# EpicDuckPotato/stereo_vo

Measured on AMD Instinct MI355X. Metric: stereo frames/sec on 1241x376 KITTI pairs, higher is better.
Workload: dtype u8/f32/f64; 1 GPU; kitti_1241x376_1500corners_5kf_window (BASELINE configs[1]); streams_per_gpu=96, max_corners=1500, window=5, pipeline_groups=3, hardware_queues=4

## Files before the change

include/svo.h:

```cpp
#ifndef SVO_H_
#define SVO_H_

#include <stddef.h>
#include <stdint.h>

#ifdef __cplusplus
extern "C" {
#endif

typedef enum svo_status {
  SVO_OK = 0,
  SVO_ERR_INVALID = -1,
  SVO_ERR_HIP = -2,
  SVO_ERR_CAPACITY = -3,
  SVO_ERR_NO_DEVICE = -4,
  SVO_ERR_NUMERIC = -5
} svo_status;

typedef struct svo_camera_info {
  double focal, cx, cy;
  double k1, k2, p1, p2;
  double baseline;
} svo_camera_info;

// ... 224 lines not shown

typedef struct svo_ba_options {
  int max_iterations;
  double max_time_s;
  double function_tolerance, gradient_tolerance, parameter_tolerance;
  double initial_radius;
  int max_features;
  int accumulation;
} svo_ba_options;

enum { SVO_BA_ACC_AUTO = 0, SVO_BA_ACC_DETERMINISTIC = 1, SVO_BA_ACC_ATOMICS = 2, SVO_BA_ACC_MFMA = 3 };

typedef struct svo_ba_summary {
  int iterations, successful_steps, termination;
  double initial_cost, final_cost;
  double solve_ms;
} svo_ba_summary;

typedef int (*svo_allreduce_fn)(void* dev_ptr, size_t n_doubles, void* user);

typedef struct svo_lm_step_ctl {
  double cost, mcc, decrease_factor;
  double spec_radius;
  int chain;
} svo_lm_step_ctl;
typedef struct svo_lm_ops {
  void* user;
  int (*linearize)(void* user, double radius, int first, double* payload1);
  int (*step)(void* user, const double* dc, const double* cand_poses7, double radius, const svo_lm_step_ctl* ctl,
              double* payload2, double* payload1_next, double* next_radius, int* next_at_candidate);
  int (*accept)(void* user);
} svo_lm_ops;
typedef struct svo_lm_stats {
  int linearize_calls;
  int step_calls;
  int speculations;
  int speculation_hits;
  int single_exchange;
  int collectives;
  int device_control;
  int fallbacks;
  double host_us;
} svo_lm_stats;

void svo_ba_default_options(svo_ba_options* o);
int svo_lm_solve(int n_poses, double* poses7, const svo_lm_ops* ops, const svo_ba_options* opt,
                 svo_ba_summary* summary, svo_lm_stats* stats);
int svo_lm_decide_step(double cost, double mcc, double radius, double decrease_factor, double cost_new,
                       double model_change_points, int* accept, double* next_radius);
int svo_ba_create(svo_ctx* ctx, svo_ba** out, int window_size, const svo_camera_info* cam,
                  const svo_ba_options* opt, int max_landmarks, int max_observations);
void svo_ba_destroy(svo_ba* ba);
int svo_ba_reset(svo_ba* ba);
int svo_ba_add_keyframe(svo_ba* ba, const double* pose7, const int64_t* tracked_ids,
                        const float* tracked_xy, int n_tracked, const float* new_xy,
                        const float* new_xyz, int n_new, int64_t* new_ids, int* n_new_out);
int svo_ba_solve(svo_ba* ba, svo_ba_summary* summary);
int svo_cholesky_solve(double* A, double* b, int n);
int svo_cholesky_solve_dev(svo_ctx* ctx, double* A, double* b, int n);
int svo_ba_get_pose(svo_ba* ba, int k, double* pose7);
int svo_ba_window_count(svo_ba* ba);
int svo_ba_get_points(svo_ba* ba, const int64_t* ids, int n, float* xyz);

int svo_ba_load_problem(svo_ba* ba, int n_poses, const double* poses7, int n_points,
                        const double* points3, int n_obs, const int32_t* obs_pose,
                        const int32_t* obs_point, const double* obs_uv);
int svo_ba_set_allreduce(svo_ba* ba, svo_allreduce_fn fn, void* user);
int svo_ba_set_comm(svo_ba* ba, void* nccl_comm);
int svo_rccl_unique_id(void* id128);
int svo_rccl_comm_create(void** nccl_comm, int n_ranks, int rank, const void* id128, int device);
int svo_rccl_comm_destroy(void* nccl_comm);
int svo_ba_set_device_lm(svo_ba* ba, int mode);
int svo_ba_set_solve_form(svo_ba* ba, int form);
int svo_ba_set_bulk_control(svo_ba* ba, int mode);
int svo_ba_last_stats(svo_ba* ba, svo_lm_stats* stats);
int svo_ba_wave_chunks_limit(void);
int svo_ba_set_wave_chunks(svo_ba* ba, int k);
int svo_ba_solve_forms(svo_ba* ba, long* counts, int n, long* gave_up);
int svo_ba_set_yield_iterations(svo_ba* ba, int n);
int svo_ba_solve_problem(svo_ba* ba, svo_ba_summary* summary);
int svo_ba_solve_problems(svo_ba** bas, int n, svo_ba_summary* summaries);
int svo_ba_read_problem(svo_ba* ba, double* poses7, double* points3);

typedef struct svo_pipeline svo_pipeline;
typedef struct svo_pipeline_params {
  svo_camera_info cam;
  int width, height;
  int max_corners;
  double quality;
  float min_feature_distance;
  float parallax_thresh;
  int window_size;
  int max_features;
  int ba_max_iterations;
  double ba_max_time_s;
} svo_pipeline_params;

typedef struct svo_frame_result {
  int n_detected, n_tracked, n_inliers, n_new;
  int is_keyframe;
  float av_parallax, percent_lost;
  double pose7[7];
  int ba_iterations;
} svo_frame_result;

void svo_pipeline_default_params(svo_pipeline_params* p);
int svo_pipeline_create(svo_ctx* ctx, svo_pipeline** out, const svo_pipeline_params* p);
void svo_pipeline_destroy(svo_pipeline* p);
int svo_pipeline_reset(svo_pipeline* p);
int svo_pipeline_process_batch_dev(svo_pipeline* p, const uint8_t* left, const uint8_t* right,
                                   int batch, svo_frame_result* results);
int svo_pipeline_process_batch(svo_pipeline* p, const uint8_t* left, const uint8_t* right,
                               int batch, svo_frame_result* results);
int svo_pipeline_set_rectification(svo_pipeline* p, const svo_rectify_eye* left, const svo_rectify_eye* right);
int svo_pipeline_set_keyframe_clouds(svo_pipeline* p, const svo_cloud_params* params, int max_keyframes_per_call);
int svo_pipeline_set_keyframe_speckle_filter(svo_pipeline* p, const svo_speckle_params* params);
int svo_pipeline_set_keyframe_lr_check(svo_pipeline* p, const svo_lr_check_params* params);
int svo_pipeline_set_keyframe_sgm(svo_pipeline* p, const svo_sgm_params* params);
typedef struct svo_keyframe_cloud {
  int frame;
  int lane;
  int n_total, n_stored;
  const svo_cloud_point* dev;
} svo_keyframe_cloud;
int svo_pipeline_keyframe_clouds(svo_pipeline* p, int* n, const svo_keyframe_cloud** table);
int svo_pipeline_copy_keyframe_cloud(svo_pipeline* p, int i, svo_cloud_point* host, int capacity);
int svo_pipeline_keyframe_disparity(svo_pipeline* p, int i, const int16_t** dev);
int svo_pipeline_copy_keyframe_disparity(svo_pipeline* p, int i, int16_t* host);
int svo_pipeline_get_tracked(svo_pipeline* p, int64_t* ids, float* xy, int capacity, int* n);

typedef struct svo_pipeline_group svo_pipeline_group;
int svo_pipeline_group_create(svo_ctx* ctx, svo_pipeline_group** out, const svo_pipeline_params* p, int n_lanes);
void svo_pipeline_group_destroy(svo_pipeline_group* g);
int svo_pipeline_group_reset(svo_pipeline_group* g);
int svo_pipeline_group_lanes(const svo_pipeline_group* g);
int svo_pipeline_group_process_batch_dev(svo_pipeline_group* g, const uint8_t* left, const uint8_t* right, size_t lane_stride,
                                         int batch, svo_frame_result* results);
int svo_pipeline_group_staging(svo_pipeline_group* g, int slot, uint8_t** left, uint8_t** right, size_t* lane_stride);
int svo_pipeline_group_upload(svo_pipeline_group* g, int slot, int batch);
int svo_pipeline_group_process_uploaded(svo_pipeline_group* g, int slot, svo_frame_result* results);
int svo_pipeline_group_process_batch(svo_pipeline_group* g, const uint8_t* left, const uint8_t* right, size_t lane_stride,
                                     int batch, svo_frame_result* results);
int svo_pipeline_group_set_rectification(svo_pipeline_group* g, int lane, const svo_rectify_eye* left, const svo_rectify_eye* right);
int svo_pipeline_group_set_keyframe_clouds(svo_pipeline_group* g, int lane, const svo_cloud_params* params, int max_keyframes_per_call);
int svo_pipeline_group_set_keyframe_speckle_filter(svo_pipeline_group* g, const svo_speckle_params* params);
int svo_pipeline_group_set_keyframe_lr_check(svo_pipeline_group* g, const svo_lr_check_params* params);
int svo_pipeline_group_set_keyframe_sgm(svo_pipeline_group* g, const svo_sgm_params* params);
int svo_pipeline_group_keyframe_clouds(svo_pipeline_group* g, int* n, const svo_keyframe_cloud** table);
int svo_pipeline_group_copy_keyframe_cloud(svo_pipeline_group* g, int i, svo_cloud_point* host, int capacity);
int svo_pipeline_group_keyframe_disparity(svo_pipeline_group* g, int i, const int16_t** dev);
int svo_pipeline_group_copy_keyframe_disparity(svo_pipeline_group* g, int i, int16_t* host);
int svo_pipeline_group_get_tracked(svo_pipeline_group* g, int lane, int64_t* ids, float* xy, int capacity, int* n);
int svo_pipeline_group_last_stats(const svo_pipeline_group* g, long* launches6, long* lanes6);
int svo_pipeline_group_solve_work(svo_pipeline_group* g, double* out4, int reset);
int svo_pipeline_group_solve_forms(svo_pipeline_group* g, long* counts, int n, long* gave_up);
int svo_pipeline_group_set_solve_yield(svo_pipeline_group* g, int n);

int svo_draw_track(const uint8_t* gray, int width, int height, int row_stride, const float* from_xy,
                   const float* to_xy, int n, uint8_t* rgb);
int svo_pipeline_draw_track(svo_pipeline* p, const uint8_t* keyframe_gray, int row_stride, uint8_t* rgb);

typedef struct svo_synth_params {
  uint64_t seed;
  int width, height;
  double focal, cx, cy, baseline;
  double step_z, step_x, yaw_per_frame;
  int n_billboards;
} svo_synth_params;
void svo_synth_default_params(svo_synth_params* p, int width, int height);
int svo_synth_render(const svo_synth_params* p, int frame, uint8_t* left, uint8_t* right);
int svo_synth_pose(const svo_synth_params* p, int frame, double* rt12);

int svo_image_read_gray(const char* path, uint8_t* buf, size_t capacity, int* width, int* height);
int svo_kitti_read_poses(const char* poses_file, double* rt12, int capacity_frames, int* n_frames);
int svo_ate_rmse(const double* est_xyz, const double* gt_xyz, int n, int with_scale, double* rmse);
typedef struct svo_run_stats {
  int frames, keyframes;
  double ate_rmse;
  double seconds;
} svo_run_stats;
int svo_kitti_run(svo_ctx* ctx, const svo_pipeline_params* params, const char* data_path, int sequence,
                  int max_frames, double* traj_rt12, svo_run_stats* stats);

#ifdef __cplusplus
}
#endif
#endif
```

stereo_vo_amd/api.py:

```python
import ctypes as C
import os

import numpy as np

_HERE = os.path.dirname(os.path.abspath(__file__))
_LIB = None


class SvoError(RuntimeError):
    pass


def lib_path():
    return os.path.join(_HERE, "libsvo_hip.so")


class Limits(C.Structure):
    _fields_ = [("max_width", C.c_int), ("max_height", C.c_int), ("max_batch", C.c_int),
                ("max_corners", C.c_int), ("max_candidates", C.c_int), ("max_features", C.c_int)]


class CameraInfo(C.Structure):
    _fields_ = [(n, C.c_double) for n in ("focal", "cx", "cy", "k1", "k2", "p1", "p2", "baseline")]

# ... 199 lines not shown
SPECKLE_TILE = (64, 16)


def speckle_workspace_bytes(width, height, batch=1):
    return int(lib().svo_speckle_workspace_bytes(width, height, batch))


CLOUD_POINT_DTYPE = np.dtype([("x", np.float32), ("y", np.float32), ("z", np.float32), ("tag", np.uint32)])


class KeyframeCloud(C.Structure):
    _fields_ = [("frame", C.c_int), ("lane", C.c_int), ("n_total", C.c_int), ("n_stored", C.c_int), ("dev", C.c_void_p)]


def cloud_default_params(width, height):
    p = CloudParams()
    if lib().svo_cloud_default_params(C.byref(p), width, height) != 0:
        raise SvoError("svo_cloud_default_params failed")
    return p


def _cloud_params(width, height, step, min_disparity, max_points):
    return CloudParams(int(step), float(min_disparity), int(width * height if max_points is None else max_points))


def _keyframe_disparity(ctx, h, fn, i):
    dev = C.c_void_p()
    ctx._chk(fn(h, int(i), C.byref(dev)), fn.__name__)
    return dev.value


def _keyframe_disparity_host(ctx, h, fn, i, width, height):
    d = np.empty((height, width), np.int16)
    ctx._chk(fn(h, int(i), _p(d)), fn.__name__)
    return d


def _keyframe_clouds(ctx, L, h, table_fn, copy_fn):
    n, tab = C.c_int(0), C.POINTER(KeyframeCloud)()
    ctx._chk(table_fn(h, C.byref(n), C.byref(tab)), table_fn.__name__)
    out = []
    for i in range(n.value):
        e = tab[i]
        pts = np.empty(e.n_stored, CLOUD_POINT_DTYPE)
        ctx._chk(copy_fn(h, i, _p(pts), e.n_stored), copy_fn.__name__)
        out.append({"frame": e.frame, "lane": e.lane, "n_total": e.n_total, "n_stored": e.n_stored, "dev": e.dev, "points": pts})
    return out


class SynthParams(C.Structure):
    _fields_ = [("seed", C.c_uint64), ("width", C.c_int), ("height", C.c_int), ("focal", C.c_double),
                ("cx", C.c_double), ("cy", C.c_double), ("baseline", C.c_double), ("step_z", C.c_double),
                ("step_x", C.c_double), ("yaw_per_frame", C.c_double), ("n_billboards", C.c_int)]


REFERENCE_CONSTANT_NAMES = (
    "gftt_max_corners", "gftt_quality", "min_detected", "keyframe_percent_lost", "pnp_iterations", "pnp_reproj_error",
    "pnp_confidence", "stereo_num_disparities", "stereo_block_size", "stereo_disparity_scale",
    "triangulate_min_disparity_exclusive", "lk_win_w", "lk_win_h", "lk_max_level", "lk_max_iterations", "lk_epsilon",
    "lk_min_eig_threshold", "fb_max_distance", "max_parallax", "draw_thickness", "parallax_thresh", "min_feature_distance",
    "sliding_window_size", "max_features", "ba_max_solver_time_s", "ba_num_threads")


class ReferenceConstants(C.Structure):
    _fields_ = [(n, C.c_double) for n in REFERENCE_CONSTANT_NAMES]


def reference_constants():
    c = ReferenceConstants()
    if lib().svo_reference_constants(C.byref(c)) != 0:
        raise SvoError("svo_reference_constants failed")
    return {n: getattr(c, n) for n in REFERENCE_CONSTANT_NAMES}


class LmStats(C.Structure):
    _fields_ = [("linearize_calls", C.c_int), ("step_calls", C.c_int), ("speculations", C.c_int), ("speculation_hits", C.c_int),
                ("single_exchange", C.c_int), ("collectives", C.c_int), ("device_control", C.c_int), ("fallbacks", C.c_int),
                ("host_us", C.c_double)]


class LmStepCtl(C.Structure):
    _fields_ = [("cost", C.c_double), ("mcc", C.c_double), ("decrease_factor", C.c_double), ("spec_radius", C.c_double),
                ("chain", C.c_int)]


LM_LINEARIZE_FN = C.CFUNCTYPE(C.c_int, C.c_void_p, C.c_double, C.c_int, C.POINTER(C.c_double))
LM_STEP_FN = C.CFUNCTYPE(C.c_int, C.c_void_p, C.POINTER(C.c_double), C.POINTER(C.c_double), C.c_double, C.POINTER(LmStepCtl),
                         C.POINTER(C.c_double), C.POINTER(C.c_double), C.POINTER(C.c_double), C.POINTER(C.c_int))
LM_ACCEPT_FN = C.CFUNCTYPE(C.c_int, C.c_void_p)


class LmOps(C.Structure):
    _fields_ = [("user", C.c_void_p), ("linearize", LM_LINEARIZE_FN), ("step", LM_STEP_FN), ("accept", LM_ACCEPT_FN)]


def lm_decide_step(cost, mcc, radius, decrease_factor, cost_new, model_change_points):
    acc, rad = C.c_int(0), C.c_double(0.0)
    lib().svo_lm_decide_step(C.c_double(cost), C.c_double(mcc), C.c_double(radius), C.c_double(decrease_factor), C.c_double(cost_new),
                             C.c_double(model_change_points), C.byref(acc), C.byref(rad))
    return bool(acc.value), rad.value


def lm_solve(poses7, linearize, step, accept, max_iterations=50, max_time_s=0.0):
    poses = np.ascontiguousarray(poses7, np.float64).copy()
    K = poses.shape[0]
    n = 6 * (K - 1)
    pay1 = n * n + 3 * n + 2

    def _lin(user, radius, first, out):
        np.ctypeslib.as_array(out, shape=(pay1,))[:] = linearize(radius, first)
        return 0

    def _step(user, dc, cand, radius, ctl, out2, out1, out_radius, out_at_cand):
        d = np.ctypeslib.as_array(dc, shape=(max(n, 1),))[:n].copy()
        c = np.ctypeslib.as_array(cand, shape=(K, 7)).copy()
        p2, p1, nr, at_cand = step(d, c, radius, ctl.contents)
        np.ctypeslib.as_array(out2, shape=(4,))[:] = p2
        if p1 is not None:
            np.ctypeslib.as_array(out1, shape=(pay1,))[:] = p1
        out_radius[0] = nr if p1 is not None else 0.0
        out_at_cand[0] = int(bool(at_cand))
        return 0

    def _acc(user):
        accept()
        return 0
    ops = LmOps(None, LM_LINEARIZE_FN(_lin), LM_STEP_FN(_step), LM_ACCEPT_FN(_acc))
    opt = ba_default_options()
    opt.max_iterations, opt.max_time_s = max_iterations, max_time_s
    s, st = BASummary(), LmStats()
    rc = lib().svo_lm_solve(K, _p(poses), C.byref(ops), C.byref(opt), C.byref(s), C.byref(st))
    if rc:
        raise SvoError(f"svo_lm_solve failed ({rc})")
    return poses, s, st


ALLREDUCE_FN = C.CFUNCTYPE(C.c_int, C.c_void_p, C.c_size_t, C.c_void_p)

SYMBOLS = [
    "svo_create", "svo_destroy", "svo_last_error", "svo_stream", "svo_sync", "svo_version", "svo_reference_constants",
    "svo_profile_select", "svo_profile_read", "svo_measure_peak",
    "svo_reproj_eval", "svo_reproj_eval_dev",
    "svo_corner_detect", "svo_corner_detect_batch_dev", "svo_corner_response",
    "svo_stereo_bm", "svo_stereo_disparity_at", "svo_stereo_disparity_at_dev",
    "svo_triangulate", "svo_lk_track", "svo_build_pyramid", "svo_track_features", "svo_dedup",
    "svo_pnp_ransac",
    "svo_ba_default_options", "svo_ba_create", "svo_ba_destroy", "svo_ba_reset", "svo_ba_add_keyframe", "svo_ba_solve",
    "svo_ba_get_pose", "svo_ba_window_count", "svo_ba_get_points", "svo_ba_load_problem",
    "svo_ba_set_allreduce", "svo_ba_set_device_lm", "svo_ba_set_bulk_control", "svo_ba_set_solve_form", "svo_ba_wave_chunks_limit", "svo_ba_set_wave_chunks", "svo_ba_set_yield_iterations", "svo_ba_solve_forms", "svo_ba_solve_problem", "svo_ba_solve_problems", "svo_ba_read_problem", "svo_ba_set_comm", "svo_ba_last_stats", "svo_lm_solve", "svo_lm_decide_step",
    "svo_rccl_unique_id", "svo_rccl_comm_create", "svo_rccl_comm_destroy",
    "svo_pipeline_default_params", "svo_pipeline_create", "svo_pipeline_destroy", "svo_pipeline_reset",
    "svo_pipeline_process_batch_dev", "svo_pipeline_process_batch", "svo_pipeline_get_tracked",
    "svo_pipeline_group_create", "svo_pipeline_group_destroy", "svo_pipeline_group_reset", "svo_pipeline_group_lanes",
    "svo_pipeline_group_process_batch_dev", "svo_pipeline_group_get_tracked", "svo_pipeline_group_last_stats",
    "svo_pipeline_group_solve_work", "svo_pipeline_group_solve_forms", "svo_pipeline_group_set_solve_yield", "svo_pipeline_group_staging", "svo_pipeline_group_upload", "svo_pipeline_group_process_uploaded", "svo_pipeline_group_process_batch",
    "svo_synth_default_params", "svo_synth_render", "svo_synth_pose",
    "svo_image_read_gray", "svo_kitti_read_poses", "svo_ate_rmse", "svo_kitti_run", "svo_cholesky_solve", "svo_cholesky_solve_dev", "svo_draw_track", "svo_pipeline_draw_track",
    "svo_rectify_eye_from_camera_info", "svo_rectify_build_map", "svo_rectify_remap", "svo_rectify_remap_batch_dev",
    "svo_pipeline_set_rectification", "svo_pipeline_group_set_rectification",
    "svo_stereo_bm_batch_dev", "svo_cloud_default_params", "svo_disparity_cloud_batch_dev", "svo_stereo_cloud",
    "svo_pipeline_set_keyframe_clouds", "svo_pipeline_keyframe_clouds", "svo_pipeline_copy_keyframe_cloud",
    "svo_pipeline_group_set_keyframe_clouds", "svo_pipeline_group_keyframe_clouds", "svo_pipeline_group_copy_keyframe_cloud",
    "svo_speckle_workspace_bytes", "svo_disparity_speckle_filter_batch_dev", "svo_disparity_speckle_filter",
    "svo_pipeline_set_keyframe_speckle_filter", "svo_pipeline_group_set_keyframe_speckle_filter",
    "svo_stereo_bm_cost_batch_dev", "svo_disparity_lr_check_batch_dev", "svo_disparity_lr_check",
    "svo_pipeline_set_keyframe_lr_check", "svo_pipeline_group_set_keyframe_lr_check",
    "svo_sgm_default_params", "svo_sgm_workspace_bytes", "svo_stereo_sgm_batch_dev", "svo_stereo_sgm",
    "svo_pipeline_set_keyframe_sgm", "svo_pipeline_group_set_keyframe_sgm",
    "svo_voxel_map_default_params", "svo_voxel_map_bytes", "svo_voxel_map_create", "svo_voxel_map_destroy", "svo_voxel_map_clear",
    "svo_voxel_map_insert_dev", "svo_pose7_to_cam_to_world", "svo_voxel_map_insert_pose7_dev", "svo_voxel_map_stats",
    "svo_voxel_map_extract_dev", "svo_voxel_map_extract", "svo_voxel_map_download",
    "svo_voxel_carve_default_params", "svo_voxel_map_carve_dev", "svo_pose7_to_world_to_cam", "svo_voxel_map_carve_pose7_dev",
    "svo_voxel_map_carve", "svo_voxel_map_copy_live_dev", "svo_pipeline_keyframe_disparity", "svo_pipeline_group_keyframe_disparity",
    "svo_pipeline_copy_keyframe_disparity", "svo_pipeline_group_copy_keyframe_disparity",
    "svo_voxel_render_default_params", "svo_voxel_render_workspace_bytes", "svo_voxel_map_render_dev", "svo_voxel_map_render_pose7_dev",
    "svo_voxel_map_render", "svo_voxel_render_set_mode",
    "svo_voxel_map_remove_dev", "svo_voxel_map_remove_pose7_dev", "svo_voxel_map_remove_sync", "svo_voxel_map_move_dev", "svo_voxel_map_move_pose7_dev",
    "svo_voxel_ledger_bytes", "svo_voxel_ledger_create", "svo_voxel_ledger_destroy", "svo_voxel_ledger_insert_pose7_dev",
    "svo_voxel_ledger_update_pose7", "svo_voxel_ledger_retire", "svo_voxel_ledger_remove", "svo_voxel_ledger_ids", "svo_voxel_ledger_get",
]


def lib():
    global _LIB
    if _LIB is None:
        p = lib_path()
        if not os.path.exists(p):
            raise SvoError(f"{p} not built — run `python -c 'import __graft_entry__ as g; g.build()'`")
        L = C.CDLL(p)
        L.svo_version.restype = C.c_char_p
        L.svo_last_error.restype = C.c_char_p
        L.svo_last_error.argtypes = [C.c_void_p]
        L.svo_stream.restype = C.c_void_p
        L.svo_stream.argtypes = [C.c_void_p]
        L.svo_destroy.argtypes = [C.c_void_p]
        L.svo_destroy.restype = None
        vp, ci, sz = C.c_void_p, C.c_int, C.c_size_t
        L.svo_cloud_default_params.argtypes = [vp, ci, ci]
        L.svo_stereo_bm_batch_dev.argtypes = [vp, vp, vp, ci, ci, ci, ci, sz, ci, ci, vp]
        L.svo_disparity_cloud_batch_dev.argtypes = [vp, vp, vp, ci, ci, ci, ci, sz, vp, vp, vp, vp, vp]
        L.svo_stereo_cloud.argtypes = [vp, vp, vp, ci, ci, ci, ci, ci, vp, vp, vp, vp, vp, vp]
        L.svo_pipeline_set_keyframe_clouds.argtypes = [vp, vp, ci]
        L.svo_pipeline_keyframe_clouds.argtypes = [vp, vp, vp]
        L.svo_pipeline_copy_keyframe_cloud.argtypes = [vp, ci, vp, ci]
        L.svo_pipeline_group_set_keyframe_clouds.argtypes = [vp, ci, vp, ci]
        L.svo_pipeline_group_keyframe_clouds.argtypes = [vp, vp, vp]
        L.svo_pipeline_group_copy_keyframe_cloud.argtypes = [vp, ci, vp, ci]
        for f in ("svo_cloud_default_params", "svo_stereo_bm_batch_dev", "svo_disparity_cloud_batch_dev", "svo_stereo_cloud",
                  "svo_pipeline_set_keyframe_clouds", "svo_pipeline_keyframe_clouds", "svo_pipeline_copy_keyframe_cloud",
                  "svo_pipeline_group_set_keyframe_clouds", "svo_pipeline_group_keyframe_clouds", "svo_pipeline_group_copy_keyframe_cloud"):
            getattr(L, f).restype = ci
        L.svo_speckle_workspace_bytes.argtypes = [ci, ci, ci]
        L.svo_speckle_workspace_bytes.restype = sz
        L.svo_disparity_speckle_filter_batch_dev.argtypes = [vp, vp, ci, ci, ci, vp, vp, sz, vp]
        L.svo_disparity_speckle_filter.argtypes = [vp, vp, ci, ci, vp, vp]
        L.svo_pipeline_set_keyframe_speckle_filter.argtypes = [vp, vp]
        L.svo_pipeline_group_set_keyframe_speckle_filter.argtypes = [vp, vp]
        for f in ("svo_disparity_speckle_filter_batch_dev", "svo_disparity_speckle_filter", "svo_pipeline_set_keyframe_speckle_filter",
                  "svo_pipeline_group_set_keyframe_speckle_filter"):
            getattr(L, f).restype = ci
        L.svo_stereo_bm_cost_batch_dev.argtypes = [vp, vp, vp, ci, ci, ci, ci, sz, ci, ci, vp, vp]
        L.svo_disparity_lr_check_batch_dev.argtypes = [vp, vp, vp, ci, ci, ci, vp, vp]
        L.svo_disparity_lr_check.argtypes = [vp, vp, vp, ci, ci, vp, vp]
        L.svo_pipeline_set_keyframe_lr_check.argtypes = [vp, vp]
        L.svo_pipeline_group_set_keyframe_lr_check.argtypes = [vp, vp]
        for f in ("svo_stereo_bm_cost_batch_dev", "svo_disparity_lr_check_batch_dev", "svo_disparity_lr_check",
                  "svo_pipeline_set_keyframe_lr_check", "svo_pipeline_group_set_keyframe_lr_check"):
            getattr(L, f).restype = ci
        L.svo_sgm_default_params.argtypes = [vp, ci]
        L.svo_sgm_workspace_bytes.argtypes = [ci, ci, ci, ci, ci]
        L.svo_sgm_workspace_bytes.restype = sz
        L.svo_stereo_sgm_batch_dev.argtypes = [vp, vp, vp, ci, ci, ci, ci, sz, ci, ci, vp, vp, sz, vp, vp]
        L.svo_stereo_sgm.argtypes = [vp, vp, vp, ci, ci, ci, ci, ci, vp, vp, vp]
        L.svo_pipeline_set_keyframe_sgm.argtypes = [vp, vp]
        L.svo_pipeline_group_set_keyframe_sgm.argtypes = [vp, vp]
        for f in ("svo_sgm_default_params", "svo_stereo_sgm_batch_dev", "svo_stereo_sgm", "svo_pipeline_set_keyframe_sgm",
                  "svo_pipeline_group_set_keyframe_sgm"):
            getattr(L, f).restype = ci
        L.svo_voxel_map_default_params.argtypes = [vp]
        L.svo_voxel_map_bytes.argtypes = [vp, vp]
        L.svo_voxel_map_create.argtypes = [vp, vp, vp]
        L.svo_voxel_map_destroy.argtypes = [vp]
        L.svo_voxel_map_destroy.restype = None
        L.svo_voxel_map_clear.argtypes = [vp]
        L.svo_voxel_map_insert_dev.argtypes = [vp, vp, ci, vp]
        L.svo_pose7_to_cam_to_world.argtypes = [vp, vp]
        L.svo_voxel_map_insert_pose7_dev.argtypes = [vp, vp, ci, vp]
        L.svo_voxel_map_stats.argtypes = [vp, vp]
        L.svo_voxel_map_extract_dev.argtypes = [vp, ci, vp, ci, vp]
        L.svo_voxel_map_extract.argtypes = [vp, ci, vp, ci, vp, vp]
        L.svo_voxel_map_download.argtypes = [vp, vp, sz]
        for f in ("svo_voxel_map_default_params", "svo_voxel_map_bytes", "svo_voxel_map_create", "svo_voxel_map_clear",
                  "svo_voxel_map_insert_dev", "svo_pose7_to_cam_to_world", "svo_voxel_map_insert_pose7_dev", "svo_voxel_map_stats",
                  "svo_voxel_map_extract_dev", "svo_voxel_map_extract", "svo_voxel_map_download"):
            getattr(L, f).restype = ci
        L.svo_voxel_carve_default_params.argtypes = [vp]
        L.svo_voxel_map_carve_dev.argtypes = [vp, vp, ci, ci, vp, vp, vp, vp]
        L.svo_pose7_to_world_to_cam.argtypes = [vp, vp]
        L.svo_voxel_map_carve_pose7_dev.argtypes = [vp, vp, ci, ci, vp, vp, vp, vp]
        L.svo_voxel_map_carve.argtypes = [vp, vp, ci, ci, vp, vp, vp, vp]
        L.svo_voxel_map_copy_live_dev.argtypes = [vp, vp, ci, vp]
        L.svo_pipeline_keyframe_disparity.argtypes = [vp, ci, vp]
        L.svo_pipeline_group_keyframe_disparity.argtypes = [vp, ci, vp]
        L.svo_pipeline_copy_keyframe_disparity.argtypes = [vp, ci, vp]
        L.svo_pipeline_group_copy_keyframe_disparity.argtypes = [vp, ci, vp]
        for f in ("svo_voxel_carve_default_params", "svo_voxel_map_carve_dev", "svo_pose7_to_world_to_cam", "svo_voxel_map_carve_pose7_dev",
                  "svo_voxel_map_carve", "svo_voxel_map_copy_live_dev", "svo_pipeline_keyframe_disparity",
                  "svo_pipeline_group_keyframe_disparity", "svo_pipeline_copy_keyframe_disparity",
                  "svo_pipeline_group_copy_keyframe_disparity"):
            getattr(L, f).restype = ci
        L.svo_voxel_render_default_params.argtypes = [vp]
        L.svo_voxel_render_workspace_bytes.argtypes = [ci, ci]
        L.svo_voxel_render_workspace_bytes.restype = sz
        L.svo_voxel_map_render_dev.argtypes = [vp, ci, ci, vp, vp, vp, vp, vp, vp, vp]
        L.svo_voxel_map_render_pose7_dev.argtypes = [vp, ci, ci, vp, vp, vp, vp, vp, vp, vp]
        L.svo_voxel_map_render.argtypes = [vp, ci, ci, vp, vp, vp, vp, vp, vp]
        L.svo_voxel_render_set_mode.argtypes = [vp, ci, ci]
        for f in ("svo_voxel_render_default_params", "svo_voxel_map_render_dev", "svo_voxel_map_render_pose7_dev", "svo_voxel_map_render",
                  "svo_voxel_render_set_mode"):
            getattr(L, f).restype = ci
        i64 = C.c_int64
        L.svo_voxel_map_remove_dev.argtypes = [vp, vp, ci, vp, vp]
        L.svo_voxel_map_remove_pose7_dev.argtypes = [vp, vp, ci, vp, vp]
        L.svo_voxel_map_remove_sync.argtypes = [vp, vp, ci, vp, vp]
        L.svo_voxel_map_move_dev.argtypes = [vp, vp, ci, vp, vp, vp]
        L.svo_voxel_map_move_pose7_dev.argtypes = [vp, vp, ci, vp, vp, vp]
        L.svo_voxel_ledger_bytes.argtypes = [vp, vp]
        L.svo_voxel_ledger_create.argtypes = [vp, vp, vp]
        L.svo_voxel_ledger_destroy.argtypes = [vp]
        L.svo_voxel_ledger_destroy.restype = None
        L.svo_voxel_ledger_insert_pose7_dev.argtypes = [vp, i64, vp, ci, vp]
        L.svo_voxel_ledger_update_pose7.argtypes = [vp, i64, vp, vp]
        L.svo_voxel_ledger_retire.argtypes = [vp, i64]
        L.svo_voxel_ledger_remove.argtypes = [vp, i64, vp]
        L.svo_voxel_ledger_ids.argtypes = [vp, vp, ci, vp]
        L.svo_voxel_ledger_get.argtypes = [vp, i64, vp, vp, vp]
        for f in ("svo_voxel_map_remove_dev", "svo_voxel_map_remove_pose7_dev", "svo_voxel_map_remove_sync", "svo_voxel_map_move_dev", "svo_voxel_map_move_pose7_dev",
                  "svo_voxel_ledger_bytes", "svo_voxel_ledger_create", "svo_voxel_ledger_insert_pose7_dev", "svo_voxel_ledger_update_pose7",
                  "svo_voxel_ledger_retire", "svo_voxel_ledger_remove", "svo_voxel_ledger_ids", "svo_voxel_ledger_get"):
            getattr(L, f).restype = ci
        _LIB = L
    return _LIB


def _p(a, t=None):
    if a is None:
        return None
# ... 685 lines not shown

    def close(self):
        if self.h:
            self.L.svo_pipeline_destroy(self.h)
            self.h = C.c_void_p()

    def __del__(self):
        try:
            self.close()
        except Exception:
            pass

    def reset(self):
        self.ctx._chk(self.L.svo_pipeline_reset(self.h), "svo_pipeline_reset")

    def set_rectification(self, left=None, right=None):
        self.L.svo_pipeline_set_rectification.argtypes = [C.c_void_p, C.c_void_p, C.c_void_p]
        self.ctx._chk(self.L.svo_pipeline_set_rectification(self.h, _ref(left), _ref(right)), "svo_pipeline_set_rectification")

    def set_keyframe_clouds(self, params=None, max_keyframes_per_call=0):
        if params is True:
            params = cloud_default_params(self.prm.width, self.prm.height)
        self.ctx._chk(self.L.svo_pipeline_set_keyframe_clouds(self.h, _ref(params), max_keyframes_per_call),
                      "svo_pipeline_set_keyframe_clouds")

    def process_batch(self, left, right):
        left, right = _u8(left), _u8(right)
        b = left.shape[0]
        res = (FrameResult * b)()
        self.ctx._chk(self.L.svo_pipeline_process_batch(self.h, _p(left), _p(right), b, res), "svo_pipeline_process_batch")
        return list(res)

    def process_batch_dev(self, left_ptr, right_ptr, batch):
        res = (FrameResult * batch)()
        self.ctx._chk(self.L.svo_pipeline_process_batch_dev(self.h, C.c_void_p(left_ptr), C.c_void_p(right_ptr), batch, res),
                      "svo_pipeline_process_batch_dev")
        return list(res)

    def draw_track(self, keyframe_gray):
        g = np.ascontiguousarray(keyframe_gray, np.uint8)
        out = np.empty(g.shape + (3,), np.uint8)
        self.ctx._chk(self.L.svo_pipeline_draw_track(self.h, _p(g), g.shape[1], _p(out)), "svo_pipeline_draw_track")
        return out

    def tracked(self, capacity=8192):
        ids = np.empty(capacity, np.int64)
        xy = np.empty((capacity, 2), np.float32)
        n = C.c_int(0)
        self.ctx._chk(self.L.svo_pipeline_get_tracked(self.h, _p(ids), _p(xy), capacity, C.byref(n)), "svo_pipeline_get_tracked")
        return ids[:n.value].copy(), xy[:n.value].copy()


class PipelineGroup(_KeyframeCloudMethods):

    _ENTRY = "svo_pipeline_group"
    STAGES = ("track", "pnp_ransac", "host_thread_busy_us_of_call_us", "dedup_stereo_triangulate", "bundle_adjust", "corners_pyramids")

    def __init__(self, ctx, params, n_lanes):
        self.ctx, self.L, self.prm, self.n_lanes = ctx, ctx.L, params, n_lanes
        self.h = C.c_void_p()
        self.L.svo_pipeline_group_destroy.argtypes = [C.c_void_p]
        self.L.svo_pipeline_group_destroy.restype = None
        self.L.svo_pipeline_group_process_batch_dev.argtypes = [C.c_void_p, C.c_void_p, C.c_void_p, C.c_size_t, C.c_int, C.c_void_p]
        ctx._chk(self.L.svo_pipeline_group_create(ctx.h, C.byref(self.h), C.byref(params), n_lanes), "svo_pipeline_group_create")

    def close(self):
        if self.h:
            self.L.svo_pipeline_group_destroy(self.h)
            self.h = C.c_void_p()

    def __del__(self):
        try:
            self.close()
        except Exception:
            pass

    def reset(self):
        self.ctx._chk(self.L.svo_pipeline_group_reset(self.h), "svo_pipeline_group_reset")

    def set_rectification(self, lane, left=None, right=None):
        self.L.svo_pipeline_group_set_rectification.argtypes = [C.c_void_p, C.c_int, C.c_void_p, C.c_void_p]
        self.ctx._chk(self.L.svo_pipeline_group_set_rectification(self.h, lane, _ref(left), _ref(right)), "svo_pipeline_group_set_rectification")

    def set_keyframe_clouds(self, lane=-1, params=None, max_keyframes_per_call=0):
        if params is True:
            params = cloud_default_params(self.prm.width, self.prm.height)
        self.ctx._chk(self.L.svo_pipeline_group_set_keyframe_clouds(self.h, lane, _ref(params), max_keyframes_per_call),
                      "svo_pipeline_group_set_keyframe_clouds")

    def process_batch_dev(self, left_ptr, right_ptr, lane_stride, batch):
        res = (FrameResult * (self.n_lanes * batch))()
        self.ctx._chk(self.L.svo_pipeline_group_process_batch_dev(self.h, C.c_void_p(left_ptr), C.c_void_p(right_ptr), C.c_size_t(lane_stride),
                                                                  batch, res), "svo_pipeline_group_process_batch_dev")
        self.last_raw = bytes(res)
        return [list(res[l * batch:(l + 1) * batch]) for l in range(self.n_lanes)]

    def staging(self, slot):
        lp, rp, stride = C.POINTER(C.c_uint8)(), C.POINTER(C.c_uint8)(), C.c_size_t(0)
        self.L.svo_pipeline_group_staging.argtypes = [C.c_void_p, C.c_int, C.c_void_p, C.c_void_p, C.c_void_p]
        self.ctx._chk(self.L.svo_pipeline_group_staging(self.h, slot, C.byref(lp), C.byref(rp), C.byref(stride)), "svo_pipeline_group_staging")
        h, w = self.prm.height, self.prm.width
        mb = stride.value // (h * w)
        shape = (self.n_lanes, mb, h, w)
        n = self.n_lanes * mb * h * w
        return (np.ctypeslib.as_array(lp, shape=(n,)).reshape(shape), np.ctypeslib.as_array(rp, shape=(n,)).reshape(shape))

    def upload(self, slot, batch):
        self.ctx._chk(self.L.svo_pipeline_group_upload(self.h, slot, batch), "svo_pipeline_group_upload")

    def process_uploaded(self, slot, batch):
        res = (FrameResult * (self.n_lanes * batch))()
        self.L.svo_pipeline_group_process_uploaded.argtypes = [C.c_void_p, C.c_int, C.c_void_p]
        self.ctx._chk(self.L.svo_pipeline_group_process_uploaded(self.h, slot, res), "svo_pipeline_group_process_uploaded")
        self.last_raw = bytes(res)
        return [list(res[l * batch:(l + 1) * batch]) for l in range(self.n_lanes)]

    def process_batch(self, left, right):
        left, right = _u8(left), _u8(right)
        batch = left.shape[1]
        res = (FrameResult * (self.n_lanes * batch))()
        self.L.svo_pipeline_group_process_batch.argtypes = [C.c_void_p, C.c_void_p, C.c_void_p, C.c_size_t, C.c_int, C.c_void_p]
        self.ctx._chk(self.L.svo_pipeline_group_process_batch(self.h, _p(left), _p(right), C.c_size_t(batch * left.shape[2] * left.shape[3]), batch, res),
                      "svo_pipeline_group_process_batch")
        self.last_raw = bytes(res)
        return [list(res[l * batch:(l + 1) * batch]) for l in range(self.n_lanes)]

    def get_tracked(self, lane, capacity=8192):
        ids = np.empty(capacity, np.int64)
        xy = np.empty((capacity, 2), np.float32)
        n = C.c_int(0)
        self.ctx._chk(self.L.svo_pipeline_group_get_tracked(self.h, lane, _p(ids), _p(xy), capacity, C.byref(n)), "svo_pipeline_group_get_tracked")
        return ids[:n.value].copy(), xy[:n.value].copy()

    def solve_work(self, reset=False):
        out = (C.c_double * 4)()
        self.ctx._chk(self.L.svo_pipeline_group_solve_work(self.h, out, int(reset)), "svo_pipeline_group_solve_work")
        return list(out)

    def solve_forms(self):
        n = self.L.svo_ba_wave_chunks_limit() + 1
        out, gu = (C.c_long * n)(), C.c_long(0)
        self.ctx._chk(self.L.svo_pipeline_group_solve_forms(self.h, out, n, C.byref(gu)), "svo_pipeline_group_solve_forms")
        return list(out), gu.value

    def set_solve_yield(self, n):
        self.ctx._chk(self.L.svo_pipeline_group_set_solve_yield(self.h, int(n)), "svo_pipeline_group_set_solve_yield")

    def solve_resumes(self):
        n = self.L.svo_ba_wave_chunks_limit() + 2
        out = (C.c_long * n)()
        self.ctx._chk(self.L.svo_pipeline_group_solve_forms(self.h, out, n, None), "svo_pipeline_group_solve_forms")
        return out[n - 1]

    def last_stats(self):
        a, b = (C.c_long * 6)(), (C.c_long * 6)()
        self.ctx._chk(self.L.svo_pipeline_group_last_stats(self.h, a, b), "svo_pipeline_group_last_stats")
        return {s: (a[i], b[i]) for i, s in enumerate(self.STAGES) if s != "unused"}


class RunStats(C.Structure):
    _fields_ = [("frames", C.c_int), ("keyframes", C.c_int), ("ate_rmse", C.c_double), ("seconds", C.c_double)]


def image_read_gray(path, max_pixels=1 << 24):
    buf = np.empty(max_pixels, np.uint8)
    w, h = C.c_int(0), C.c_int(0)
    rc = lib().svo_image_read_gray(path.encode(), _p(buf), C.c_size_t(max_pixels), C.byref(w), C.byref(h))
    if rc:
        raise SvoError(f"svo_image_read_gray({path}) rc={rc}")
    return buf[:w.value * h.value].reshape(h.value, w.value).copy()


def kitti_read_poses(path, max_frames=100000):
    rt = np.empty((max_frames, 12))
    n = C.c_int(0)
    rc = lib().svo_kitti_read_poses(path.encode(), _p(rt), max_frames, C.byref(n))
    if rc:
        raise SvoError(f"svo_kitti_read_poses({path}) rc={rc}")
    return rt[:n.value].reshape(-1, 3, 4).copy()


def ate_rmse(est_xyz, gt_xyz, with_scale=False):
    est_xyz, gt_xyz = _f64(est_xyz), _f64(gt_xyz)
    out = C.c_double(0)
    rc = lib().svo_ate_rmse(_p(est_xyz), _p(gt_xyz), est_xyz.shape[0], int(with_scale), C.byref(out))
    if rc:
        raise SvoError(f"svo_ate_rmse rc={rc}")
    return out.value


def kitti_run(ctx, params, data_path, sequence, max_frames):
    traj = np.zeros((max_frames, 12))
    st = RunStats()
    ctx._chk(lib().svo_kitti_run(ctx.h, C.byref(params), data_path.encode(), sequence, max_frames, _p(traj), C.byref(st)),
             "svo_kitti_run")
    return traj[:st.frames].reshape(-1, 3, 4).copy(), st


def cholesky_solve(A, b):
    A = np.array(A, np.float64, order="C")
    b = np.array(b, np.float64)
    rc = lib().svo_cholesky_solve(_p(A), _p(b), b.shape[0])
    if rc != 0:
        raise SvoError(f"svo_cholesky_solve rc={rc}")
    return b


def draw_track(gray, from_xy, to_xy):
    g = np.ascontiguousarray(gray, np.uint8)
    a = np.ascontiguousarray(from_xy, np.float32).reshape(-1, 2)
    b = np.ascontiguousarray(to_xy, np.float32).reshape(-1, 2)
    out = np.empty(g.shape + (3,), np.uint8)
    rc = lib().svo_draw_track(_p(g), g.shape[1], g.shape[0], g.shape[1], _p(a), _p(b), a.shape[0], _p(out))
    if rc:
        raise SvoError(f"svo_draw_track rc={rc}")
    return out
```

stereo_vo_amd/csrc/ba.hip:

```cpp
#include <math.h>
#include <stdlib.h>

#include <algorithm>
#include <atomic>
#include <mutex>
#include <sched.h>
#include <chrono>
#include <memory>
#include <vector>

#include "ba_admission.h"
#include "ba_graph.h"
#include "ba_layout.h"
#include "ba_plan.h"
#include "kernels.h"
#include "group_kernels.h"
#include "lm_decide.h"
#include "lm_device.h"
#include "lm_lds.h"
#include "lm_turns.h"
#include "ref_constants.h"
#include "reproj_device.h"

int svo_rccl_allreduce_f64(void* buf, size_t count, void* comm, hipStream_t stream, const char** err);
bool svo_throughput_mode();

namespace {
int g_ba_cu_share = 32;
constexpr int SVO_MAX_DEVICES = 16;
int ba_fused_budget(int device);
BaLedger& ba_ledger(int dev) {
  static std::mutex mu;
  static BaLedger* ledger[SVO_MAX_DEVICES];
  dev = dev >= 0 && dev < SVO_MAX_DEVICES ? dev : 0;
  std::lock_guard<std::mutex> g(mu);
  if (ledger[dev]) return *ledger[dev];
  char bus[64] = {0}, path[128] = {0};
  const char* e = getenv("SVO_BA_XPROC");
  if (!(e && *e && atoi(e) == 0) && hipDeviceGetPCIBusId(bus, sizeof(bus) - 1, dev) == hipSuccess) {
    for (char* c = bus; *c; ++c) if (*c == ':' || *c == '.') *c = '_';
    snprintf(path, sizeof(path), "/dev/shm/svo_admit_%s", bus);
  }
  return *(ledger[dev] = new BaLedger(path[0] ? path : nullptr, dev));
}
constexpr double MIN_DIAG = 1e-6, MAX_DIAG = 1e32, LM_MIN_RADIUS_BULK = 1e-32;
constexpr int BULK_RING = 8;
constexpr int PAY2_SLOTS = 8;

struct BaDev {
  int K = 0, n = 0, M = 0, L = 0, C = 0;
  const double* poses = nullptr;
  double* cand_poses = nullptr;
  const double* points = nullptr;
  double* cand_points = nullptr;
  const int4* rec = nullptr;
  const double* obs_uv = nullptr;
  double* sp = nullptr;
  double* pay1 = nullptr;
  double* pay2 = nullptr;
  double f = 0, cx = 0, cy = 0;
  int det = 0;
  int G = 1, NG = 0, Epad = 0, E = 0;
  int CPW = 1, GS = 1;
  const uint16_t* tab = nullptr;
  const uint32_t* tab_off = nullptr;
  int tab_lds_words = 0;
  const unsigned* lm_key = nullptr;
  double* part1 = nullptr;
  double* part2 = nullptr;
  double* pay1_out = nullptr;
  double* pay2_out = nullptr;
  const double* step_in = nullptr;
  int* flag = nullptr;
  unsigned* arrive = nullptr;
  unsigned arrive_target = 0;
  int seq = 0;
  double* ctl_dev = nullptr;
  unsigned long long pay_tag = 0;
  int pay_parity = 0;
};

struct LmCtl { double cost, mcc, radius, decrease_factor; int chain; };

typedef double svo_d2 __attribute__((ext_vector_type(2)));
template <bool WT>
__device__ __forceinline__ void slot_store2(double* p, double x, double y) {
  if constexpr (WT) {
    const svo_d2 v = {x, y};
    asm volatile("global_store_dwordx4 %0, %1, off sc1\n\ts_nop 1" : : "v"(p), "v"(v) : "memory");
  } else {
    p[0] = x; p[1] = y;
  }
}
__device__ __forceinline__ double slot_load(const double* p) { return __hip_atomic_load(p, __ATOMIC_RELAXED, __HIP_MEMORY_SCOPE_AGENT); }

__device__ __forceinline__ void pay_store(double* p, double v) { __hip_atomic_store(p, v, __ATOMIC_RELAXED, __HIP_MEMORY_SCOPE_SYSTEM); }
__device__ __forceinline__ void granule_store(double* g, double v, unsigned long long tag) { slot_store2<true>(g, v, __longlong_as_double((long long)tag)); }
__device__ __forceinline__ unsigned granule_load8(const double* base, const int (&idx)[8], unsigned long long tag, double (&out)[8]) {
  svo_d2 v0, v1, v2, v3, v4, v5, v6, v7;
  const double* p0 = base + 2 * (idx[0] < 0 ? 0 : idx[0]); const double* p1 = base + 2 * (idx[1] < 0 ? 0 : idx[1]);
  const double* p2 = base + 2 * (idx[2] < 0 ? 0 : idx[2]); const double* p3 = base + 2 * (idx[3] < 0 ? 0 : idx[3]);
  const double* p4 = base + 2 * (idx[4] < 0 ? 0 : idx[4]); const double* p5 = base + 2 * (idx[5] < 0 ? 0 : idx[5]);
  const double* p6 = base + 2 * (idx[6] < 0 ? 0 : idx[6]); const double* p7 = base + 2 * (idx[7] < 0 ? 0 : idx[7]);
  asm volatile(
      "global_load_dwordx4 %0, %8, off sc1\n\tglobal_load_dwordx4 %1, %9, off sc1\n\tglobal_load_dwordx4 %2, %10, off sc1\n\t"
      "global_load_dwordx4 %3, %11, off sc1\n\tglobal_load_dwordx4 %4, %12, off sc1\n\tglobal_load_dwordx4 %5, %13, off sc1\n\t"
      "global_load_dwordx4 %6, %14, off sc1\n\tglobal_load_dwordx4 %7, %15, off sc1\n\ts_waitcnt vmcnt(0)"
      : "=&v"(v0), "=&v"(v1), "=&v"(v2), "=&v"(v3), "=&v"(v4), "=&v"(v5), "=&v"(v6), "=&v"(v7)
      : "v"(p0), "v"(p1), "v"(p2), "v"(p3), "v"(p4), "v"(p5), "v"(p6), "v"(p7)
      : "memory");
  const svo_d2 v[8] = {v0, v1, v2, v3, v4, v5, v6, v7};
  unsigned ok = 0;
#pragma unroll
  for (int u = 0; u < 8; ++u) {
    out[u] = v[u].x;
    if (idx[u] < 0 || (unsigned long long)__double_as_longlong(v[u].y) == tag) ok |= 1u << u;
  }
  return ok;
}
__device__ __forceinline__ bool granule_wait(const double* base, int idx, unsigned long long tag, double& out) {
  const int only[8] = {idx, -1, -1, -1, -1, -1, -1, -1};
  double v[8];
  long long t0 = 0;
  for (unsigned spins = 0;; ++spins) {
    if (granule_load8(base, only, tag, v) & 1u) { out = v[0]; return true; }
    __builtin_amdgcn_s_sleep(2);
    if ((spins & 255u) == 255u) {
      const long long tn = (long long)wall_clock64();
      if (!t0) t0 = tn;
      else if (tn - t0 > 300000000ll) return false;
    }
  }
}

__device__ __forceinline__ bool wait_sentinels(const double* base, int first, int stride, int count, unsigned long long tag, int* s_flag) {
  if (threadIdx.x == 0) *s_flag = 1;
  __syncthreads();
  for (int i = threadIdx.x; i < count; i += (int)blockDim.x) {
    const double* p = base + 2 * ((size_t)first + (size_t)i * stride);
    long long t0 = 0;
    for (unsigned spins = 0;; ++spins) {
      svo_d2 v;
      asm volatile("global_load_dwordx4 %0, %1, off sc1\n\ts_waitcnt vmcnt(0)" : "=&v"(v) : "v"(p) : "memory");
      if ((unsigned long long)__double_as_longlong(v.y) == tag) break;
      __builtin_amdgcn_s_sleep(4);
      if ((spins & 255u) == 255u) {
        const long long tn = (long long)wall_clock64();
        if (!t0) t0 = tn;
        else if (tn - t0 > 300000000ll) { *s_flag = 0; break; }
      }
    }
  }
  __syncthreads();
  return *s_flag != 0;
}

__device__ __forceinline__ void decide_device(const LmCtl& c, double cost_new, double mc_points, double* ctl_dev, double* pay2buf) {
  const SvoLmDecision d = svo_lm_decide(c.cost, c.mcc, c.radius, c.decrease_factor, cost_new, mc_points);
  ctl_dev[0] = (double)d.accept; ctl_dev[1] = d.next_radius;
  pay_store(&pay2buf[4], (double)d.accept); pay_store(&pay2buf[5], d.next_radius);
}

__device__ __forceinline__ void apply_ctl(BaDev& P, double& radius, const double* __restrict__ ctl) {
  if (!ctl) return;
  const double acc = __hip_atomic_load(&ctl[0], __ATOMIC_RELAXED, __HIP_MEMORY_SCOPE_AGENT);
  radius = __hip_atomic_load(&ctl[1], __ATOMIC_RELAXED, __HIP_MEMORY_SCOPE_AGENT);
  if (acc != 0.0) { P.points = P.cand_points; P.poses = P.cand_poses; }
}

enum { BC_DONE = 0, BC_MODE, BC_SEL, BC_RADIUS, BC_DF, BC_COST, BC_INITIAL_COST, BC_MCC, BC_ITER, BC_SUCC, BC_TERM, BC_NEED_LIN,
       BC_LIN_CALLS, BC_STEP_CALLS, BC_NEXT_USED, BC_T0, BC_WORDS = 24 };
enum { BCM_FIRST = 0, BCM_STEP, BCM_RELIN };
struct BulkSel { const double* bctl; double* pts[2]; double* pos[2]; };

__device__ __forceinline__ void bulk_select(BaDev& P, const BulkSel& bs) {
  const int sel = (int)bs.bctl[BC_SEL] & 1;
  P.points = bs.pts[sel]; P.cand_points = bs.pts[sel ^ 1]; P.poses = bs.pos[sel]; P.cand_poses = bs.pos[sel ^ 1];
}
__device__ __forceinline__ bool bulk_apply(BaDev& P, double& radius, int& first_pass, const BulkSel& bs) {
  if (!bs.bctl) return true;
  const double* c = bs.bctl;
  if (c[BC_DONE] != 0.0) return false;
  const int mode = (int)c[BC_MODE];
  bulk_select(P, bs);
  first_pass = mode == BCM_FIRST;
  radius = c[BC_RADIUS];
  if (mode == BCM_STEP) {
    const SvoLmDecision d = svo_lm_decide(c[BC_COST], c[BC_MCC], c[BC_RADIUS], c[BC_DF], P.pay2[0], P.pay2[1]);
    radius = d.next_radius;
    if (d.accept) { P.points = P.cand_points; P.poses = P.cand_poses; }
  }
  return true;
}

__device__ __forceinline__ bool inv3_sym(const double* V, double* Vi) {
  const double a = V[0], b = V[1], c = V[2], d = V[4], e = V[5], f = V[8];
  const double c00 = d * f - e * e, c01 = c * e - b * f, c02 = b * e - c * d;
  const double det = a * c00 + b * c01 + c * c02;
  if (!(fabs(det) > 0)) { for (int i = 0; i < 9; ++i) Vi[i] = 0.0; return false; }
  const double id = 1.0 / det;
  Vi[0] = c00 * id; Vi[1] = c01 * id; Vi[2] = c02 * id;
  Vi[3] = Vi[1]; Vi[4] = (a * f - c * c) * id; Vi[5] = (b * c - a * e) * id;
  Vi[6] = Vi[2]; Vi[7] = Vi[5]; Vi[8] = (a * d - b * b) * id;
  return true;
}

__device__ __forceinline__ double shfl_d(double v, int src) { return __shfl(v, src); }

template <int NV>
__device__ __forceinline__ void segment_totals(double (&v)[NV], int lane, int first, int last, int maxlen) {
  for (int off = 1; off < maxlen; off <<= 1) {
    const bool take = lane - off >= first;
#pragma unroll
    for (int i = 0; i < NV; ++i) {
      const double u = __shfl_up(v[i], off);
      v[i] += take ? u : 0.0;
    }
  }
#pragma unroll
  for (int i = 0; i < NV; ++i) v[i] = shfl_d(v[i], last);
}

__device__ __forceinline__ void eval_obs(const double* __restrict__ pose, D3 p, double u, double v, double f, double cx,
                                         double cy, bool want_jc, double* r, double* Jc, double* Jp) {
  double Jq[14];
  reproj_full(pose, p, u, v, f, cx, cy, r, want_jc ? Jq : nullptr, Jp);
  if (want_jc) {
    const double w = pose[0], x = pose[1], y = pose[2], z = pose[3];
    const double T[4][3] = {{-x, -y, -z}, {w, z, -y}, {-z, w, x}, {y, -x, w}};
#pragma unroll
    for (int row = 0; row < 2; ++row) {
#pragma unroll
      for (int c = 0; c < 3; ++c) {
        double s = 0;
#pragma unroll
        for (int k = 0; k < 4; ++k) s += Jq[7 * row + k] * T[k][c];
        Jc[6 * row + c] = s;
      }
#pragma unroll
      for (int c = 0; c < 3; ++c) Jc[6 * row + 3 + c] = Jq[7 * row + 4 + c];
    }
  }
}
#pragma clang fp contract(fast)
__device__ __forceinline__ void eval_obs_contract(const double* __restrict__ pose, D3 p, double u, double v, double f, double cx,
                                         double cy, bool want_jc, double* r, double* Jc, double* Jp) {
  double Jq[14];
  reproj_full_c(pose, p, u, v, f, cx, cy, r, want_jc ? Jq : nullptr, Jp);
  if (want_jc) {
    const double w = pose[0], x = pose[1], y = pose[2], z = pose[3];
    const double T[4][3] = {{-x, -y, -z}, {w, z, -y}, {-z, w, x}, {y, -x, w}};
#pragma unroll
    for (int row = 0; row < 2; ++row) {
#pragma unroll
      for (int c = 0; c < 3; ++c) {
        double s = 0;
#pragma unroll
        for (int k = 0; k < 4; ++k) s += Jq[7 * row + k] * T[k][c];
        Jc[6 * row + c] = s;
      }
#pragma unroll
      for (int c = 0; c < 3; ++c) Jc[6 * row + 3 + c] = Jq[7 * row + 4 + c];
    }
  }
}
#pragma clang fp contract(off)
}

struct ObsRec { bool active; int o, k, j, first, len; D3 p; double u, v; };

__device__ __forceinline__ ObsRec load_obs(const BaDev& P, int chunk, int lane, const double* __restrict__ points) {
  ObsRec R{false, 0, 0, 0, lane, 0, D3{0, 0, 1}, 0.0, 0.0};
  R.o = chunk * 64 + lane;
  const int4 rc = P.rec[R.o];
  R.u = P.obs_uv[2 * R.o]; R.v = P.obs_uv[2 * R.o + 1];
  R.active = rc.x >= 0;
  if (R.active) {
    R.k = rc.x; R.j = rc.y; R.first = rc.z; R.len = rc.w;
    R.p = D3{points[3 * R.j], points[3 * R.j + 1], points[3 * R.j + 2]};
  }
  return R;
}

struct ObsNext { int4 rc; double u, v; };
__device__ __forceinline__ ObsNext obs_request(const BaDev& P, int chunk, int lane) {
  const int o = chunk * 64 + lane;
  return ObsNext{P.rec[o], P.obs_uv[2 * o], P.obs_uv[2 * o + 1]};
}

struct LinPre { double r[2], Jc[12], Jp[6], V[9], gp[3], cost_l; int maxlen; };
struct ChunkRegs { double s[3]; };

__device__ __forceinline__ ObsRec obs_complete(const ObsNext& x, int chunk, int lane, const double* __restrict__ points, const double* sp, ChunkRegs& c) {
  ObsRec R{false, 0, 0, 0, lane, 0, D3{0, 0, 1}, 0.0, 0.0};
  R.o = chunk * 64 + lane;
  R.u = x.u; R.v = x.v;
// ... 3824 lines not shown
```

stereo_vo_amd/csrc/group_kernels.h:

```cpp
#ifndef SVO_GROUP_KERNELS_H_
#define SVO_GROUP_KERNELS_H_
#include "kernels.h"

#include "chain_math.h"
#include "xcd_map.h"

struct SvoLkLane {
  const uint8_t* pyr_prev; const uint8_t* pyr_next;
  const uint8_t* l0_prev; const uint8_t* l0_next;
  const float* xy; const float* init_xy; const long long* ids;
  int n;
  float* fwd; uint8_t* keep; float* parallax;
  float* kept_xy; float* init_dst; long long* ids_dst;
  float* host_xy; long long* host_ids; int* host_n; float* host_av;
  unsigned* arrive; unsigned arrive_target;
  int* word; int seq;
};
struct SvoLkLanes { int w, h; SvoXcdMap map; SvoLkLane lane[SVO_MAX_LANES]; };
int svo_kg_track(svo_ctx* ctx, hipStream_t st, const SvoLkLanes& lanes, int n_lanes, int grid_x);

struct SvoPnpLane {
  const long long* ids; const float4* store; unsigned store_mask;
  const float* xy; int n; double f, cx, cy; double q0[4], t0[3]; double thr2, confidence; int iterations;
  int launched;
  double* hyp_pose; int* hyp_count; unsigned long long* hyp_mask; int mask_words;
  double* out_pose; int* inliers; int* n_inliers; float* inlier_xy;
  double* host_pose; int* host_inliers; int* host_nin; int* host_best; int* host_bad;
  unsigned* arrive; unsigned arrive_target;
  int* word; int seq;
  SvoChainRec* chain; float prev_rvec[3], prev_tvec[3]; float cam_f, cam_cx, cam_cy, cam_b;
};
struct SvoPnpLanes { SvoPnpLane lane[SVO_MAX_LANES]; };
int svo_kg_pnp(svo_ctx* ctx, hipStream_t st, const SvoPnpLanes& lanes, int n_lanes);
int svo_kg_pnp_workgroups(int launched);
int svo_kg_pnp_first(int iterations);
int svo_pnp_update_num_iters(double p, double ep, int model_points, int max_iters);
int svo_pnp_model_points();

struct SvoStereoTriLane {
  const uint8_t* left; const uint8_t* right; const float* xy; const int* n_dev; int n_max; float* disp; SvoMat4 M;
  const float* trk; int n_trk; float min_d;
  float* kept_xy; float* xyz; int* n_kept; SvoPublish pub;
  const SvoChainRec* chain;
};
struct SvoStereoTriLanes { int w, h, stride, ndisp, block; SvoXcdMap map; SvoStereoTriLane lane[SVO_MAX_LANES]; };
int svo_kg_stereo_triangulate(svo_ctx* ctx, hipStream_t st, const SvoStereoTriLanes& lanes, int n_lanes, int grid_x);

int svo_ba_solve_prepare(svo_ba* ba);
int svo_ba_solve_launch(svo_ba** bas, int n, void* stream, unsigned long long* launched_mask);
int svo_ba_solve_poll(svo_ba* ba);
int svo_ba_solve_continues(svo_ba* ba);
int svo_ba_solve_yielded(svo_ba* ba);
int svo_ba_solve_holds_budget(svo_ba* ba);
int svo_ba_solve_finish(svo_ba* ba, svo_ba_summary* summary);
void svo_ba_work(svo_ba* ba, double* out4, int reset);
int svo_ba_use_stream(svo_ba* ba, void* stream);
int svo_ba_attach_store(svo_ba* ba, float4* store, unsigned mask);

#endif
```

stereo_vo_amd/csrc/lk.hip:

```cpp
#include "kernels.h"
#include "group_kernels.h"
#include "tail_device.h"

namespace {
#include "ref_constants.h"
#ifndef SVO_LK_MAX_ITER
#define SVO_LK_MAX_ITER svo_ref::LK_MAX_ITERATIONS
#endif
constexpr int WIN = svo_ref::LK_WIN, HALF = WIN / 2, LEVELS = svo_ref::LK_MAX_LEVEL + 1, MAX_ITER = SVO_LK_MAX_ITER;
static_assert(WIN == 21 && LEVELS == 4, "the LDS layout and the exact-sum bounds below are derived for a 21x21 window, 4 levels");
constexpr int G = WIN + 1;
constexpr int RP = WIN + 3;
constexpr float MIN_EIG = svo_ref::LK_MIN_EIG_THRESHOLD;
constexpr double LK_EPS = svo_ref::LK_EPSILON;
constexpr float FLT_SCALE = 1.0f / (float)(1 << 20);
constexpr float FLT_EPS = 1.1920928955078125e-7f;

struct Pyr {
  const uint8_t* base;
  const uint8_t* l0;
  int w0, h0;
};

__device__ __forceinline__ Pyr make_pyr(const uint8_t* base, int w, int h, const uint8_t* l0 = nullptr) { return Pyr{base, l0 ? l0 : base, w, h}; }

__device__ __forceinline__ void pyr_level(const Pyr& P, int level, const uint8_t*& p, int& w, int& h) {
  if (level == 0) { p = P.l0; w = P.w0; h = P.h0; return; }
  size_t off = 0;
  w = P.w0; h = P.h0;
  for (int l = 0; l < level; ++l) {
    off += (size_t)w * h;
    w = (w + 1) / 2; h = (h + 1) / 2;
  }
  p = P.base + off;
}

__device__ __forceinline__ int descale(int v, int n) { return (v + (1 << (n - 1))) >> n; }

__device__ __forceinline__ long long wave_sum_i64(int v) {
  v += __builtin_amdgcn_mov_dpp(v, 0xB1, 0xf, 0xf, true);
  v += __builtin_amdgcn_mov_dpp(v, 0x4E, 0xf, 0xf, true);
  v += __builtin_amdgcn_mov_dpp(v, 0x141, 0xf, 0xf, true);
  int lo = v & 0xFFFF, hi = v >> 16;
  lo += __builtin_amdgcn_mov_dpp(lo, 0x140, 0xf, 0xf, true);
  hi += __builtin_amdgcn_mov_dpp(hi, 0x140, 0xf, 0xf, true);
  lo += __builtin_amdgcn_update_dpp(0, lo, 0x142, 0xa, 0xf, false);
  hi += __builtin_amdgcn_update_dpp(0, hi, 0x142, 0xa, 0xf, false);
  lo += __builtin_amdgcn_update_dpp(0, lo, 0x143, 0xc, 0xf, false);
  hi += __builtin_amdgcn_update_dpp(0, hi, 0x143, 0xc, 0xf, false);
  const long long l = __builtin_amdgcn_readlane(lo, 63), h = __builtin_amdgcn_readlane(hi, 63);
  return h * 65536 + l;
}

__device__ __forceinline__ float wave_sum_f32(int v) {
  v += __builtin_amdgcn_mov_dpp(v, 0xB1, 0xf, 0xf, true);
  v += __builtin_amdgcn_mov_dpp(v, 0x4E, 0xf, 0xf, true);
  v += __builtin_amdgcn_mov_dpp(v, 0x141, 0xf, 0xf, true);
  int lo = v & 0xFFFF, hi = v >> 16;
  lo += __builtin_amdgcn_mov_dpp(lo, 0x140, 0xf, 0xf, true);
  hi += __builtin_amdgcn_mov_dpp(hi, 0x140, 0xf, 0xf, true);
  lo += __builtin_amdgcn_update_dpp(0, lo, 0x142, 0xa, 0xf, false);
  hi += __builtin_amdgcn_update_dpp(0, hi, 0x142, 0xa, 0xf, false);
  lo += __builtin_amdgcn_update_dpp(0, lo, 0x143, 0xc, 0xf, false);
  hi += __builtin_amdgcn_update_dpp(0, hi, 0x143, 0xc, 0xf, false);
  const int l = __builtin_amdgcn_readlane(lo, 63), h = __builtin_amdgcn_readlane(hi, 63);
  return (float)h * 65536.0f + (float)l;
}

#ifndef SVO_LK_THREADS
#define SVO_LK_THREADS 64
#endif
typedef short lk_s2 __attribute__((ext_vector_type(2)));
__device__ __forceinline__ lk_s2 pack_s2(int lo, int hi) { return __builtin_bit_cast(lk_s2, __builtin_amdgcn_perm((unsigned)hi, (unsigned)lo, 0x05040100u)); }

constexpr int LKT = SVO_LK_THREADS;
constexpr int NW = LKT / 64;
constexpr int FPB = LKT == 64 ? 1 : 256 / LKT;
constexpr int PPT = (21 * 21 + LKT - 1) / LKT;
static_assert(LKT == 64 || LKT == 128 || LKT == 256, "threads per feature");
static_assert(PPT * 8 * 33292800ll < 2147483647ll, "half-row sums must stay exact in int32");
constexpr int RM = 5;
constexpr int RS = G + 2 * RM;

struct LkShared {
  alignas(4) uint8_t raw[RP * RP];
  alignas(4) uint8_t jreg[RS * RS + 8];
  short Iw[LKT == 64 ? 2 : WIN * WIN], dIx[LKT == 64 ? 2 : WIN * WIN], dIy[LKT == 64 ? 2 : WIN * WIN];
  short gx[LKT == 64 ? 2 : G * G], gy[LKT == 64 ? 2 : G * G];
  long long red[2][3][NW];
};

__device__ __forceinline__ void lk_sync() {
  if (NW == 1) {
    __builtin_amdgcn_fence(__ATOMIC_RELEASE, "workgroup");
    __builtin_amdgcn_wave_barrier();
    __builtin_amdgcn_fence(__ATOMIC_ACQUIRE, "workgroup");
  } else {
    __syncthreads();
  }
}

template <int NV>
__device__ __forceinline__ void block_sum_split(const int* v, long long* out, LkShared& S, int& phase) {
  if (NW == 1) {
#pragma unroll
    for (int k = 0; k < NV; ++k) out[k] = wave_sum_i64(v[k]);
    lk_sync();
    return;
  }
  const int wave = (threadIdx.x % LKT) >> 6, lane = threadIdx.x & 63;
#pragma unroll
  for (int k = 0; k < NV; ++k) {
    const long long t = wave_sum_i64(v[k]);
    if (lane == 0) S.red[phase][k][wave] = t;
  }
  __syncthreads();
#pragma unroll
  for (int k = 0; k < NV; ++k) {
    long long t = S.red[phase][k][0];
#pragma unroll
    for (int w = 1; w < NW; ++w) t += S.red[phase][k][w];
    out[k] = t;
  }
  phase ^= 1;
}

__device__ uint8_t lk_point_wave(const Pyr& A, const Pyr& B, float px0, float py0, float* ox, float* oy, LkShared& S);

__device__ uint8_t lk_point(const Pyr& A, const Pyr& B, float px0, float py0, float* ox, float* oy, LkShared& S) {
  if (NW == 1) return lk_point_wave(A, B, px0, py0, ox, oy, S);
  const int lane = threadIdx.x % LKT;
  int phase = 0;
  uint8_t status = 1;
  float nx = 0.f, ny = 0.f;
  for (int level = LEVELS - 1; level >= 0; --level) {
    const uint8_t *Ip, *Jp;
    int Iw_, Ih_, Jw_, Jh_;
    pyr_level(A, level, Ip, Iw_, Ih_);
    pyr_level(B, level, Jp, Jw_, Jh_);
    const float sc = (float)(1.0 / (double)(1 << level));
    float pxl = px0 * sc, pyl = py0 * sc;
    if (level == LEVELS - 1) { nx = pxl; ny = pyl; } else { nx = nx * 2.0f; ny = ny * 2.0f; }
    pxl -= (float)HALF; pyl -= (float)HALF;
    const int ipx = (int)floorf(pxl), ipy = (int)floorf(pyl);
    if (ipx < -WIN || ipx >= Iw_ || ipy < -WIN || ipy >= Ih_) {
      if (level == 0) status = 0;
      continue;
    }
    float a = pxl - (float)ipx, b = pyl - (float)ipy;
    int iw00 = __float2int_rn((1.f - a) * (1.f - b) * (float)(1 << 14));
    int iw01 = __float2int_rn(a * (1.f - b) * (float)(1 << 14));
    int iw10 = __float2int_rn((1.f - a) * b * (float)(1 << 14));
    int iw11 = (1 << 14) - iw00 - iw01 - iw10;
    lk_sync();
    for (int i = lane; i < RP * RP; i += LKT) {
      const int r = i / RP, c = i % RP;
      S.raw[i] = Ip[__mul24(reflect101(ipy - 1 + r, Ih_), Iw_) + reflect101(ipx - 1 + c, Iw_)];
    }
    lk_sync();
    for (int i = lane; i < G * G; i += LKT) {
      const int r = i / G, c = i % G;
      const int X = ipx + c, Y = ipy + r;
      int vx = 0, vy = 0;
      if (X >= 0 && X < Iw_ && Y >= 0 && Y < Ih_) {
        const uint8_t* t = &S.raw[r * RP + c];
        const int t00 = t[0], t01 = t[1], t02 = t[2];
        const int t10 = t[RP], t11 = t[RP + 1], t12 = t[RP + 2];
        const int t20 = t[2 * RP], t21 = t[2 * RP + 1], t22 = t[2 * RP + 2];
        const int s0 = (t00 + t20) * 3 + t10 * 10, s2 = (t02 + t22) * 3 + t12 * 10;
        const int d0 = t20 - t00, d1 = t21 - t01, d2 = t22 - t02;
        vx = (short)(s2 - s0);
        vy = (short)((d2 + d0) * 3 + d1 * 10);
        (void)t11;
      }
      S.gx[i] = (short)vx; S.gy[i] = (short)vy;
    }
    lk_sync();
    int pA[3] = {0, 0, 0};
    for (int i = lane; i < WIN * WIN; i += LKT) {
      const int r = i / WIN, c = i % WIN;
      const int o = r * G + c, o1 = o + G;
      const int rr = (r + 1) * RP + (c + 1);
      const int ival = descale(__mul24(S.raw[rr], iw00) + __mul24(S.raw[rr + 1], iw01) + __mul24(S.raw[rr + RP], iw10) + __mul24(S.raw[rr + RP + 1], iw11), 9);
      const int ixv = descale(__mul24(S.gx[o], iw00) + __mul24(S.gx[o + 1], iw01) + __mul24(S.gx[o1], iw10) + __mul24(S.gx[o1 + 1], iw11), 14);
      const int iyv = descale(__mul24(S.gy[o], iw00) + __mul24(S.gy[o + 1], iw01) + __mul24(S.gy[o1], iw10) + __mul24(S.gy[o1 + 1], iw11), 14);
      S.Iw[i] = (short)ival; S.dIx[i] = (short)ixv; S.dIy[i] = (short)iyv;
      pA[0] += __mul24(ixv, ixv);
      pA[1] += __mul24(ixv, iyv);
      pA[2] += __mul24(iyv, iyv);
    }
    long long sA[3];
    block_sum_split<3>(pA, sA, S, phase);
    const long long sA11 = sA[0], sA12 = sA[1], sA22 = sA[2];
    const float A11 = (float)(double)sA11 * FLT_SCALE;
    const float A12 = (float)(double)sA12 * FLT_SCALE;
    const float A22 = (float)(double)sA22 * FLT_SCALE;
    float D = A11 * A22 - A12 * A12;
    const float dif = A11 - A22;
    const float minEig = (A22 + A11 - sqrtf(dif * dif + 4.f * A12 * A12)) / (float)(2 * WIN * WIN);
    if (minEig < MIN_EIG || D < FLT_EPS) {
      if (level == 0) status = 0;
      continue;
    }
    D = 1.f / D;
    float outx = nx, outy = ny;
    nx -= (float)HALF; ny -= (float)HALF;
    float pdx = 0.f, pdy = 0.f;
    int woff[PPT], wi[PPT];
#pragma unroll
    for (int u = 0; u < PPT; ++u) {
      const int i = lane + LKT * u;
      wi[u] = i < WIN * WIN ? i : -1;
      woff[u] = i < WIN * WIN ? (i / WIN) * RS + (i % WIN) : 0;
    }
    int rx0 = 0, ry0 = 0;
    bool staged = false;
    for (int j = 0; j < MAX_ITER; ++j) {
      const int inx = (int)floorf(nx), iny = (int)floorf(ny);
      if (inx < -WIN || inx >= Jw_ || iny < -WIN || iny >= Jh_) {
        if (level == 0) status = 0;
        break;
      }
      a = nx - (float)inx; b = ny - (float)iny;
      iw00 = __float2int_rn((1.f - a) * (1.f - b) * (float)(1 << 14));
      iw01 = __float2int_rn(a * (1.f - b) * (float)(1 << 14));
      iw10 = __float2int_rn((1.f - a) * b * (float)(1 << 14));
      iw11 = (1 << 14) - iw00 - iw01 - iw10;
      if (!staged || inx < rx0 || inx > rx0 + 2 * RM || iny < ry0 || iny > ry0 + 2 * RM) {
        rx0 = inx - RM; ry0 = iny - RM;
        lk_sync();
        if (rx0 >= 0 && ry0 >= 0 && rx0 + RS <= Jw_ && ry0 + RS <= Jh_) {
          for (int i = lane; i < RS * RS; i += LKT) S.jreg[i] = Jp[__mul24(ry0 + i / RS, Jw_) + rx0 + i % RS];
        } else {
          for (int i = lane; i < RS * RS; i += LKT)
            S.jreg[i] = Jp[__mul24(reflect101(ry0 + i / RS, Jh_), Jw_) + reflect101(rx0 + i % RS, Jw_)];
        }
        lk_sync();
        staged = true;
      }
      const int ob = (iny - ry0) * RS + (inx - rx0);
      int pb[2] = {0, 0};
#pragma unroll
      for (int u = 0; u < PPT; ++u) {
        if (wi[u] >= 0) {
          const int o = ob + woff[u];
          const int diff = descale(__mul24(S.jreg[o], iw00) + __mul24(S.jreg[o + 1], iw01) + __mul24(S.jreg[o + RS], iw10) + __mul24(S.jreg[o + RS + 1], iw11), 9) - S.Iw[wi[u]];
          pb[0] += __mul24(diff, S.dIx[wi[u]]);
          pb[1] += __mul24(diff, S.dIy[wi[u]]);
        }
      }
      long long sb[2];
      block_sum_split<2>(pb, sb, S, phase);
      const long long sb1 = sb[0], sb2 = sb[1];
      const float b1 = (float)(double)sb1 * FLT_SCALE;
      const float b2 = (float)(double)sb2 * FLT_SCALE;
      const float dx = (A12 * b2 - A22 * b1) * D;
      const float dy = (A12 * b1 - A11 * b2) * D;
      nx += dx; ny += dy;
      outx = nx + (float)HALF; outy = ny + (float)HALF;
      if ((double)dx * (double)dx + (double)dy * (double)dy <= LK_EPS * LK_EPS) break;
      if (j > 0 && (double)fabsf(dx + pdx) < LK_EPS && (double)fabsf(dy + pdy) < LK_EPS) {
        outx -= dx * 0.5f; outy -= dy * 0.5f;
        break;
      }
      pdx = dx; pdy = dy;
    }
    nx = outx; ny = outy;
    if (status && level == 0) {
      const float fx = nx - (float)HALF, fy = ny - (float)HALF;
      const int ix = (int)floorf(fx), iy = (int)floorf(fy);
      if (ix < -WIN || ix >= Jw_ || iy < -WIN || iy >= Jh_) status = 0;
    }
  }
  *ox = nx; *oy = ny;
  return status;
}

__device__ __forceinline__ bool below_eps(float x) {
  static_assert(LK_EPS == 0.01, "the float threshold below is derived for epsilon = 0.01");
  return fabsf(x) <= 0.01f;
}
__device__ __forceinline__ bool step_below_eps(float dx, float dy) {
  const float s = dx * dx + dy * dy;
  if (s < 0.9999e-4f) return true;
  if (s > 1.0001e-4f) return false;
  return (double)dx * (double)dx + (double)dy * (double)dy <= LK_EPS * LK_EPS;
}

template <int N, int CAP>
__device__ __forceinline__ void stage_tile(uint8_t* dst, const uint8_t* __restrict__ img, int w, int h, int x0, int y0, int lane) {
  static_assert(N % 4 == 0 && N * N <= CAP, "tile rows are whole dwords");
  constexpr int DW = N / 4, NDW = DW * N, PER = (NDW + 63) / 64;
  if (x0 >= 0 && y0 >= 0 && x0 + N <= w && y0 + N <= h) {
    uint32_t v[PER];
#pragma unroll
    for (int k = 0; k < PER; ++k) {
      const int i = lane + 64 * k;
      v[k] = 0;
      if (NDW % 64 == 0 || i < NDW) __builtin_memcpy(&v[k], img + __mul24(y0 + i / DW, w) + x0 + 4 * (i % DW), 4);
    }
    uint32_t* d32 = reinterpret_cast<uint32_t*>(dst);
#pragma unroll
    for (int k = 0; k < PER; ++k) {
      const int i = lane + 64 * k;
      if (NDW % 64 == 0 || i < NDW) d32[i] = v[k];
    }
  } else {
    constexpr int NB = N * N, PERB = (NB + 63) / 64;
    uint8_t v[PERB];
#pragma unroll
    for (int k = 0; k < PERB; ++k) {
      const int i = lane + 64 * k;
      v[k] = 0;
      if (NB % 64 == 0 || i < NB) v[k] = img[__mul24(reflect101(y0 + i / N, h), w) + reflect101(x0 + i % N, w)];
    }
#pragma unroll
    for (int k = 0; k < PERB; ++k) {
      const int i = lane + 64 * k;
      if (NB % 64 == 0 || i < NB) dst[i] = v[k];
    }
  }
}

__device__ uint8_t lk_point_wave(const Pyr& A, const Pyr& B, float px0, float py0, float* ox, float* oy, LkShared& S) {
  const int lane = threadIdx.x & 63;
  const bool act = lane < 63;
  const int r = act ? lane / 3 : 0, c0 = act ? 7 * (lane - 3 * (lane / 3)) : 0;
  int phase = 0;
  uint8_t status = 1;
  float nx = 0.f, ny = 0.f;
  for (int level = LEVELS - 1; level >= 0; --level) {
    const uint8_t *Ip, *Jp;
    int Iw_, Ih_, Jw_, Jh_;
    pyr_level(A, level, Ip, Iw_, Ih_);
    pyr_level(B, level, Jp, Jw_, Jh_);
    const float sc = (float)(1.0 / (double)(1 << level));
    float pxl = px0 * sc, pyl = py0 * sc;
    if (level == LEVELS - 1) { nx = pxl; ny = pyl; } else { nx = nx * 2.0f; ny = ny * 2.0f; }
    pxl -= (float)HALF; pyl -= (float)HALF;
    const int ipx = (int)floorf(pxl), ipy = (int)floorf(pyl);
    if (ipx < -WIN || ipx >= Iw_ || ipy < -WIN || ipy >= Ih_) {
      if (level == 0) status = 0;
      continue;
    }
    float a = pxl - (float)ipx, b = pyl - (float)ipy;
    int iw00 = __float2int_rn((1.f - a) * (1.f - b) * (float)(1 << 14));
    int iw01 = __float2int_rn(a * (1.f - b) * (float)(1 << 14));
    int iw10 = __float2int_rn((1.f - a) * b * (float)(1 << 14));
    int iw11 = (1 << 14) - iw00 - iw01 - iw10;
    lk_sync();
    stage_tile<RP, sizeof(S.raw)>(S.raw, Ip, Iw_, Ih_, ipx - 1, ipy - 1, lane);
    lk_sync();
    int tI[7], tX[7], tY[7];
    int pA[3] = {0, 0, 0};
    {
      int t[4][10];
#pragma unroll
      for (int j = 0; j < 4; ++j)
#pragma unroll
        for (int i = 0; i < 10; ++i) t[j][i] = S.raw[(r + j) * RP + c0 + i];
      int gx[2][8], gy[2][8];
#pragma unroll
      for (int j = 0; j < 2; ++j)
#pragma unroll
        for (int i = 0; i < 8; ++i) {
          const int X = ipx + c0 + i, Y = ipy + r + j;
          const int s0 = (t[j][i] + t[j + 2][i]) * 3 + t[j + 1][i] * 10, s2 = (t[j][i + 2] + t[j + 2][i + 2]) * 3 + t[j + 1][i + 2] * 10;
          const int d0 = t[j + 2][i] - t[j][i], d1 = t[j + 2][i + 1] - t[j][i + 1], d2 = t[j + 2][i + 2] - t[j][i + 2];
          const bool in = X >= 0 && X < Iw_ && Y >= 0 && Y < Ih_;
          gx[j][i] = in ? (int)(short)(s2 - s0) : 0;
          gy[j][i] = in ? (int)(short)((d2 + d0) * 3 + d1 * 10) : 0;
        }
#pragma unroll
      for (int p = 0; p < 7; ++p) {
        const int ival = descale(__mul24(t[1][p + 1], iw00) + __mul24(t[1][p + 2], iw01) + __mul24(t[2][p + 1], iw10) + __mul24(t[2][p + 2], iw11), 9);
        const int ixv = descale(__mul24(gx[0][p], iw00) + __mul24(gx[0][p + 1], iw01) + __mul24(gx[1][p], iw10) + __mul24(gx[1][p + 1], iw11), 14);
        const int iyv = descale(__mul24(gy[0][p], iw00) + __mul24(gy[0][p + 1], iw01) + __mul24(gy[1][p], iw10) + __mul24(gy[1][p + 1], iw11), 14);
        tI[p] = (1 << 8) - ((int)(short)ival << 9); tX[p] = (int)(short)ixv; tY[p] = (int)(short)iyv;
        if (act) {
          pA[0] += __mul24(tX[p], tX[p]);
          pA[1] += __mul24(tX[p], tY[p]);
          pA[2] += __mul24(tY[p], tY[p]);
        }
      }
    }
    lk_s2 tXp[4], tYp[4];
#pragma unroll
    for (int q = 0; q < 4; ++q) {
      tXp[q] = pack_s2(act ? tX[2 * q] : 0, act && 2 * q + 1 < 7 ? tX[2 * q + 1] : 0);
      tYp[q] = pack_s2(act ? tY[2 * q] : 0, act && 2 * q + 1 < 7 ? tY[2 * q + 1] : 0);
    }
    long long sA[3];
    block_sum_split<3>(pA, sA, S, phase);
    const float A11 = (float)(double)sA[0] * FLT_SCALE;
    const float A12 = (float)(double)sA[1] * FLT_SCALE;
    const float A22 = (float)(double)sA[2] * FLT_SCALE;
    float D = A11 * A22 - A12 * A12;
    const float dif = A11 - A22;
    const float minEig = (A22 + A11 - sqrtf(dif * dif + 4.f * A12 * A12)) / (float)(2 * WIN * WIN);
    if (minEig < MIN_EIG || D < FLT_EPS) {
      if (level == 0) status = 0;
      continue;
    }
    D = 1.f / D;
    float outx = nx, outy = ny;
    nx -= (float)HALF; ny -= (float)HALF;
    float pdx = 0.f, pdy = 0.f;
    int rx0 = 0, ry0 = 0;
    bool staged = false;
    const uint32_t* jw = reinterpret_cast<const uint32_t*>(S.jreg);
    for (int j = 0; j < MAX_ITER; ++j) {
      const int inx = __builtin_amdgcn_readfirstlane((int)floorf(nx)), iny = __builtin_amdgcn_readfirstlane((int)floorf(ny));
      if (inx < -WIN || inx >= Jw_ || iny < -WIN || iny >= Jh_) {
        if (level == 0) status = 0;
        break;
      }
      a = nx - (float)inx; b = ny - (float)iny;
      iw00 = __float2int_rn((1.f - a) * (1.f - b) * (float)(1 << 14));
      iw01 = __float2int_rn(a * (1.f - b) * (float)(1 << 14));
      iw10 = __float2int_rn((1.f - a) * b * (float)(1 << 14));
      iw11 = (1 << 14) - iw00 - iw01 - iw10;
      if (!staged || inx < rx0 || inx > rx0 + 2 * RM || iny < ry0 || iny > ry0 + 2 * RM) {
        rx0 = inx - RM; ry0 = iny - RM;
        lk_sync();
        stage_tile<RS, RS * RS>(S.jreg, Jp, Jw_, Jh_, rx0, ry0, lane);
        lk_sync();
        staged = true;
      }
      const int base = (iny - ry0 + r) * RS + (inx - rx0) + c0;
      const int wi = base >> 2, sh = base & 3;
      const uint32_t u0 = jw[wi], u1 = jw[wi + 1], u2 = jw[wi + 2];
      const uint32_t v0 = jw[wi + RS / 4], v1 = jw[wi + RS / 4 + 1], v2 = jw[wi + RS / 4 + 2];
      const uint32_t tl = __builtin_amdgcn_alignbyte(u1, u0, sh), th = __builtin_amdgcn_alignbyte(u2, u1, sh);
      const uint32_t bl = __builtin_amdgcn_alignbyte(v1, v0, sh), bh = __builtin_amdgcn_alignbyte(v2, v1, sh);
      const lk_s2 wtop = pack_s2(iw00, iw01), wbot = pack_s2(iw10, iw11);
      int diff[8];
#pragma unroll
      for (int p = 0; p < 7; ++p) {
        const uint32_t sel = 0x0c000c00u | ((uint32_t)(p + 1) << 16) | (uint32_t)p;
        const lk_s2 tp = __builtin_bit_cast(lk_s2, __builtin_amdgcn_perm(th, tl, sel)), bp = __builtin_bit_cast(lk_s2, __builtin_amdgcn_perm(bh, bl, sel));
        diff[p] = __builtin_amdgcn_sdot2(tp, wtop, __builtin_amdgcn_sdot2(bp, wbot, tI[p], false), false) >> 9;
      }
      diff[7] = 0;
      int pb[2] = {0, 0};
#pragma unroll
      for (int q = 3; q >= 0; --q) {
        const lk_s2 d = pack_s2(diff[2 * q], diff[2 * q + 1]);
        pb[0] = __builtin_amdgcn_sdot2(d, tXp[q], pb[0], false);
        pb[1] = __builtin_amdgcn_sdot2(d, tYp[q], pb[1], false);
      }
      const float b1 = wave_sum_f32(pb[0]) * FLT_SCALE;
      const float b2 = wave_sum_f32(pb[1]) * FLT_SCALE;
      const float dx = (A12 * b2 - A22 * b1) * D;
      const float dy = (A12 * b1 - A11 * b2) * D;
      nx += dx; ny += dy;
      outx = nx + (float)HALF; outy = ny + (float)HALF;
      if (step_below_eps(dx, dy)) break;
      if (j > 0 && ((int)below_eps(dx + pdx) & (int)below_eps(dy + pdy))) {
        outx -= dx * 0.5f; outy -= dy * 0.5f;
        break;
      }
      pdx = dx; pdy = dy;
    }
    nx = outx; ny = outy;
    if (status && level == 0) {
      const float fx = nx - (float)HALF, fy = ny - (float)HALF;
      const int ix = (int)floorf(fx), iy = (int)floorf(fy);
      if (ix < -WIN || ix >= Jw_ || iy < -WIN || iy >= Jh_) status = 0;
    }
  }
  *ox = nx; *oy = ny;
  return status;
}
}

__global__ __launch_bounds__(256) void pyr_copy_kernel(const uint8_t* __restrict__ imgs, int w, int h, int row_stride,
                                                       size_t image_stride, uint8_t* __restrict__ pyr, size_t pyr_stride) {
  const int x = blockIdx.x * 64 + (threadIdx.x & 63), y = blockIdx.y * 4 + (threadIdx.x >> 6);
  if (x >= w || y >= h) return;
  pyr[(size_t)blockIdx.z * pyr_stride + (size_t)y * w + x] = imgs[(size_t)blockIdx.z * image_stride + (size_t)y * row_stride + x];
}

__global__ __launch_bounds__(256) void pyr_down_kernel(uint8_t* __restrict__ pyr, size_t pyr_stride, size_t src_off, int sw,
                                                       int sh, size_t dst_off, int dw, int dh, const uint8_t* __restrict__ src_imgs,
                                                       size_t src_image_stride, int src_row_stride) {
  const int x = blockIdx.x * 64 + (threadIdx.x & 63), y = blockIdx.y * 4 + (threadIdx.x >> 6);
  if (x >= dw || y >= dh) return;
  const uint8_t* src = src_imgs ? src_imgs + (size_t)blockIdx.z * src_image_stride : pyr + (size_t)blockIdx.z * pyr_stride + src_off;
  const int k[5] = {1, 4, 6, 4, 1};
  int s = 0;
#pragma unroll
  for (int j = 0; j < 5; ++j) {
    const uint8_t* row = src + (size_t)reflect101(2 * y + j - 2, sh) * (src_imgs ? src_row_stride : sw);
    int r = 0;
#pragma unroll
    for (int i = 0; i < 5; ++i) r += k[i] * row[reflect101(2 * x + i - 2, sw)];
    s += k[j] * r;
  }
  pyr[(size_t)blockIdx.z * pyr_stride + dst_off + (size_t)y * dw + x] = (uint8_t)((s + 128) >> 8);
}

constexpr int PB_T1W = 128, PB_T1H = 64;
constexpr int PB_R0W = 2 * PB_T1W + 21, PB_R0H = 2 * PB_T1H + 21;
constexpr int PB_R1W = PB_T1W + 9, PB_R1H = PB_T1H + 9;
constexpr int PB_R2W = PB_T1W / 2 + 3, PB_R2H = PB_T1H / 2 + 3;
constexpr int PB_P0 = 280, PB_P1 = 140, PB_P2 = 68;
__global__ __launch_bounds__(256) void pyr_build_kernel(const uint8_t* __restrict__ imgs, size_t image_stride, int row_stride, int w0, int h0,
                                                        uint8_t* __restrict__ pyr, size_t pyr_stride, int tiles_x, int tiles_y, int n_images) {
  __shared__ __align__(16) uint8_t s0[PB_R0H * PB_P0];
  __shared__ __align__(16) uint8_t s1[PB_R1H * PB_P1];
  __shared__ __align__(16) uint8_t s2[PB_R2H * PB_P2];
  const int per_img = tiles_x * tiles_y, total = per_img * n_images;
  const int per_xcd = (total + 7) >> 3, v = ((int)blockIdx.x & 7) * per_xcd + ((int)blockIdx.x >> 3);
  if (v >= total) return;
  const int img = v / per_img, t = v - img * per_img, ty = t / tiles_x, tx = t - ty * tiles_x;
  const int w1 = (w0 + 1) >> 1, h1 = (h0 + 1) >> 1, w2 = (w1 + 1) >> 1, h2 = (h1 + 1) >> 1, w3 = (w2 + 1) >> 1, h3 = (h2 + 1) >> 1;
  const int x0lo = max(0, 2 * PB_T1W * tx - 14), x0hi = min(w0 - 1, 2 * PB_T1W * tx + 2 * PB_T1W + 6);
  const int y0lo = max(0, 2 * PB_T1H * ty - 14), y0hi = min(h0 - 1, 2 * PB_T1H * ty + 2 * PB_T1H + 6);
  const int x1lo = max(0, PB_T1W * tx - 6), x1hi = min(w1 - 1, PB_T1W * tx + PB_T1W + 2);
  const int y1lo = max(0, PB_T1H * ty - 6), y1hi = min(h1 - 1, PB_T1H * ty + PB_T1H + 2);
  const int x2lo = max(0, PB_T1W / 2 * tx - 2), x2hi = min(w2 - 1, PB_T1W / 2 * tx + PB_T1W / 2);
  const int y2lo = max(0, PB_T1H / 2 * ty - 2), y2hi = min(h2 - 1, PB_T1H / 2 * ty + PB_T1H / 2);
  const uint8_t* src = imgs + (size_t)img * image_stride;
  uint8_t* dst = pyr + (size_t)img * pyr_stride;
  const size_t off1 = (size_t)w0 * h0, off2 = off1 + (size_t)w1 * h1, off3 = off2 + (size_t)w2 * h2;
  {
    const int rw = x0hi - x0lo + 1, rh = y0hi - y0lo + 1, dw = rw >> 2;
    for (int i = threadIdx.x; i < rh * dw; i += 256) {
      const int r = i / dw, c = i - r * dw;
      uint32_t val;
      __builtin_memcpy(&val, src + (size_t)(y0lo + r) * row_stride + x0lo + 4 * c, 4);
      *reinterpret_cast<uint32_t*>(&s0[r * PB_P0 + 4 * c]) = val;
    }
    const int tail = rw - 4 * dw;
    for (int i = threadIdx.x; i < rh * tail; i += 256) {
      const int r = i / tail, c = 4 * dw + (i - r * tail);
      s0[r * PB_P0 + c] = src[(size_t)(y0lo + r) * row_stride + x0lo + c];
    }
  }
  __syncthreads();
  const int k5[5] = {1, 4, 6, 4, 1};
  {
    const int rw = x1hi - x1lo + 1, rh = y1hi - y1lo + 1;
    for (int i = threadIdx.x; i < rw * rh; i += 256) {
      const int ry = i / rw, rx = i - ry * rw, x = x1lo + rx, y = y1lo + ry;
      int sum = 0;
#pragma unroll
      for (int j = 0; j < 5; ++j) {
        const uint8_t* row = &s0[(reflect101(2 * y + j - 2, h0) - y0lo) * PB_P0];
        int r = 0;
#pragma unroll
        for (int q = 0; q < 5; ++q) r += k5[q] * row[reflect101(2 * x + q - 2, w0) - x0lo];
        sum += k5[j] * r;
      }
      const uint8_t o = (uint8_t)((sum + 128) >> 8);
      s1[ry * PB_P1 + rx] = o;
      if (x >= PB_T1W * tx && x < PB_T1W * tx + PB_T1W && y >= PB_T1H * ty && y < PB_T1H * ty + PB_T1H) dst[off1 + (size_t)y * w1 + x] = o;
    }
  }
  __syncthreads();
  {
    const int rw = x2hi - x2lo + 1, rh = y2hi - y2lo + 1;
    for (int i = threadIdx.x; i < rw * rh; i += 256) {
      const int ry = i / rw, rx = i - ry * rw, x = x2lo + rx, y = y2lo + ry;
      int sum = 0;
#pragma unroll
      for (int j = 0; j < 5; ++j) {
        const uint8_t* row = &s1[(reflect101(2 * y + j - 2, h1) - y1lo) * PB_P1];
        int r = 0;
#pragma unroll
        for (int q = 0; q < 5; ++q) r += k5[q] * row[reflect101(2 * x + q - 2, w1) - x1lo];
        sum += k5[j] * r;
      }
      const uint8_t o = (uint8_t)((sum + 128) >> 8);
      s2[ry * PB_P2 + rx] = o;
      if (x >= PB_T1W / 2 * tx && x < PB_T1W / 2 * tx + PB_T1W / 2 && y >= PB_T1H / 2 * ty && y < PB_T1H / 2 * ty + PB_T1H / 2) dst[off2 + (size_t)y * w2 + x] = o;
    }
  }
  __syncthreads();
  {
    const int x3lo = PB_T1W / 4 * tx, y3lo = PB_T1H / 4 * ty, rw = min(w3, x3lo + PB_T1W / 4) - x3lo, rh = min(h3, y3lo + PB_T1H / 4) - y3lo;
    for (int i = threadIdx.x; i < rw * rh; i += 256) {
      const int ry = i / rw, rx = i - ry * rw, x = x3lo + rx, y = y3lo + ry;
      int sum = 0;
#pragma unroll
      for (int j = 0; j < 5; ++j) {
        const uint8_t* row = &s2[(reflect101(2 * y + j - 2, h2) - y2lo) * PB_P2];
        int r = 0;
#pragma unroll
        for (int q = 0; q < 5; ++q) r += k5[q] * row[reflect101(2 * x + q - 2, w2) - x2lo];
        sum += k5[j] * r;
      }
      dst[off3 + (size_t)y * w3 + x] = (uint8_t)((sum + 128) >> 8);
    }
  }
}

__global__ __launch_bounds__(LKT * FPB) void lk_kernel(const uint8_t* __restrict__ pyrA, const uint8_t* __restrict__ pyrB, int w,
                                                      int h, const float* __restrict__ xy, int n, float* __restrict__ out,
                                                      uint8_t* __restrict__ status) {
  __shared__ LkShared SS[FPB];
  LkShared& S = SS[threadIdx.x / LKT];
  const int f = blockIdx.x * FPB + threadIdx.x / LKT;
  if (f >= n) return;
  const Pyr A = make_pyr(pyrA, w, h), B = make_pyr(pyrB, w, h);
  float ox, oy;
  const uint8_t s = lk_point(A, B, xy[2 * f], xy[2 * f + 1], &ox, &oy, S);
  if (threadIdx.x % LKT == 0) { out[2 * f] = ox; out[2 * f + 1] = oy; status[f] = s; }
}

__global__ __launch_bounds__(LKT * FPB) void lk_fb_kernel(const uint8_t* __restrict__ pyrA, const uint8_t* __restrict__ pyrB, int w,
                                                         int h, const float* __restrict__ xy, const float* __restrict__ init_xy,
                                                         const int* __restrict__ n_dev, int n_host, float* __restrict__ fwd,
                                                         uint8_t* __restrict__ keep, float* __restrict__ parallax) {
  __shared__ LkShared SS[FPB];
  LkShared& S = SS[threadIdx.x / LKT];
  const int n = n_dev ? *n_dev : n_host;
  const int f = blockIdx.x * FPB + threadIdx.x / LKT;
  if (f >= n) return;
  const Pyr A = make_pyr(pyrA, w, h), B = make_pyr(pyrB, w, h);
  const float x0 = xy[2 * f], y0 = xy[2 * f + 1];
  float fx, fy, bx = 0.f, by = 0.f;
  const uint8_t s1 = lk_point(A, B, x0, y0, &fx, &fy, S);
  uint8_t s2 = 0;
  if (s1) s2 = lk_point(B, A, fx, fy, &bx, &by, S);
  if (threadIdx.x % LKT == 0) {
    uint8_t k = 0;
    float par = 0.f;
    if (s1 && s2) {
      const float ex = x0 - bx, ey = y0 - by;
      if ((double)ex * (double)ex + (double)ey * (double)ey < svo_ref::FB_MAX_DISTANCE * svo_ref::FB_MAX_DISTANCE) {
        const float dx = fx - init_xy[2 * f], dy = fy - init_xy[2 * f + 1];
        par = sqrtf(dx * dx + dy * dy);
        k = !(par > svo_ref::MAX_PARALLAX);
      }
    }
    fwd[2 * f] = fx; fwd[2 * f + 1] = fy; keep[f] = k; parallax[f] = par;
  }
}

__global__ __launch_bounds__(64) __attribute__((amdgpu_waves_per_eu(4))) void lk_fb_group_kernel(SvoLkLanes g) {
  static_assert(LKT == 64 && FPB == 1, "the stream-batched tracker is written for one wavefront per feature");
  __shared__ LkShared S;
  __shared__ int sLast;
  int li, f;
  if (!svo_xcd_map_item(g.map, li, f)) return;
  const SvoLkLane& a = g.lane[li];
  const int n = a.n, lane = threadIdx.x;
  if (f < n) {
    const Pyr A = make_pyr(a.pyr_prev, g.w, g.h, a.l0_prev), B = make_pyr(a.pyr_next, g.w, g.h, a.l0_next);
    const float x0 = a.xy[2 * f], y0 = a.xy[2 * f + 1];
    float fx = 0.f, fy = 0.f, bx = 0.f, by = 0.f, px = x0, py = y0;
    uint8_t s1 = 0, s2 = 0;
#pragma nounroll
    for (int dir = 0; dir < 2; ++dir) {
      const Pyr P0 = dir ? B : A, P1 = dir ? A : B;
      float ox, oy;
      const uint8_t st = lk_point(P0, P1, px, py, &ox, &oy, S);
      if (dir == 0) { s1 = st; fx = ox; fy = oy; px = ox; py = oy; if (!st) break; }
      else { s2 = st; bx = ox; by = oy; }
    }
    if (lane == 0) {
      uint8_t k = 0;
      float par = 0.f;
      if (s1 && s2) {
        const float ex = x0 - bx, ey = y0 - by;
        if ((double)ex * (double)ex + (double)ey * (double)ey < svo_ref::FB_MAX_DISTANCE * svo_ref::FB_MAX_DISTANCE) {
          const float dx = fx - a.init_xy[2 * f], dy = fy - a.init_xy[2 * f + 1];
          par = sqrtf(dx * dx + dy * dy);
          k = !(par > svo_ref::MAX_PARALLAX);
        }
      }
      svo_wt_store(&a.fwd[2 * f], fx); svo_wt_store(&a.fwd[2 * f + 1], fy);
      svo_wt_store(&a.keep[f], k); svo_wt_store(&a.parallax[f], par);
    }
  }
  if (!svo_last_arrival(a.arrive, a.arrive_target, &sLast)) return;
  svo_latency_critical();
  int base = 0;
  float sum = 0.f;
  for (int c0 = 0; c0 < n; c0 += 64) {
    const int i = c0 + lane;
    const bool k = i < n && svo_coherent_load(&a.keep[i]) != 0;
    const float par = k ? svo_coherent_load(&a.parallax[i]) : 0.0f;
    const unsigned long long mask = __ballot(k);
    if (k) {
      const int slot = base + __popcll(mask & ((1ull << lane) - 1ull));
      const float fx = svo_coherent_load(&a.fwd[2 * i]), fy = svo_coherent_load(&a.fwd[2 * i + 1]);
      a.kept_xy[2 * slot] = fx; a.kept_xy[2 * slot + 1] = fy;
      a.init_dst[2 * slot] = a.init_xy[2 * i]; a.init_dst[2 * slot + 1] = a.init_xy[2 * i + 1];
      const long long id = a.ids[i];
      a.ids_dst[slot] = id;
      a.host_xy[2 * slot] = fx; a.host_xy[2 * slot + 1] = fy;
      a.host_ids[slot] = id;
    }
    base += __popcll(mask);
#pragma unroll
    for (int t = 0; t < 64; ++t) sum += __int_as_float(__builtin_amdgcn_readlane(__float_as_int(par), t));
  }
  if (lane == 0) {
    *a.host_n = base;
    *a.host_av = n > 0 ? sum / (float)n : 0.f;
  }
  __builtin_amdgcn_fence(__ATOMIC_RELEASE, "");
  if (lane == 0) __hip_atomic_store(a.word, a.seq, __ATOMIC_RELAXED, __HIP_MEMORY_SCOPE_SYSTEM);
}

__global__ __launch_bounds__(1024) void track_compact_kernel(const float* __restrict__ fwd, const uint8_t* __restrict__ keep,
                                                             const float* __restrict__ parallax, const int* __restrict__ n_dev,
                                                             int n_host, float* __restrict__ kept_xy, int* __restrict__ kept_index,
                                                             int* __restrict__ n_kept, float* __restrict__ av_parallax,
                                                             SvoTrackCarry carry) {
  svo_latency_critical();
  __shared__ int sWave[16];
  __shared__ __align__(16) float sPar[4096];
  const int n = n_dev ? *n_dev : n_host;
  const int lane = threadIdx.x & 63, wave = threadIdx.x >> 6;
  int base = 0;
  for (int c0 = 0; c0 < n; c0 += 1024) {
    const int i = c0 + threadIdx.x;
    const bool k = i < n && keep[i];
    if (i < 4096) sPar[i] = k ? parallax[i] : 0.0f;
    const unsigned long long mask = __ballot(k);
    if (lane == 0) sWave[wave] = __popcll(mask);
    __syncthreads();
    int off = 0, total = 0;
    for (int w = 0; w < 16; ++w) { const int c = sWave[w]; if (w < wave) off += c; total += c; }
    if (k) {
      const int slot = base + off + __popcll(mask & ((1ull << lane) - 1ull));
      kept_xy[2 * slot] = fwd[2 * i]; kept_xy[2 * slot + 1] = fwd[2 * i + 1];
      kept_index[slot] = i;
      if (carry.init_src) {
        carry.init_dst[2 * slot] = carry.init_src[2 * i]; carry.init_dst[2 * slot + 1] = carry.init_src[2 * i + 1];
        const long long id = carry.ids_src[i];
        carry.ids_dst[slot] = id;
        if (carry.host_xy) { carry.host_xy[2 * slot] = fwd[2 * i]; carry.host_xy[2 * slot + 1] = fwd[2 * i + 1]; carry.host_ids[slot] = id; }
      }
    }
    base += total;
    __syncthreads();
  }
  float sum = 0.f;
  for (int c0 = 0; c0 < n; c0 += 4096) {
    if (c0 > 0) {
      __syncthreads();
      for (int i = threadIdx.x; i < 4096 && c0 + i < n; i += 1024) sPar[i] = keep[c0 + i] ? parallax[c0 + i] : 0.0f;
      __syncthreads();
    }
    if (threadIdx.x == 0) {
      const int m = n - c0 < 4096 ? n - c0 : 4096;
      int i = 0;
      for (; i + 32 <= m; i += 32) {
        float4 q[8];
#pragma unroll
        for (int u = 0; u < 8; ++u) q[u] = *reinterpret_cast<const float4*>(&sPar[i + 4 * u]);
#pragma unroll
        for (int u = 0; u < 8; ++u) { sum += q[u].x; sum += q[u].y; sum += q[u].z; sum += q[u].w; }
      }
      for (; i < m; ++i) sum += sPar[i];
    }
  }
  if (threadIdx.x == 0) {
    const float av = n > 0 ? sum / (float)n : 0.f;
    *n_kept = base;
    *av_parallax = av;
    if (carry.host_n) {
      *carry.host_n = base;
      *carry.host_av = av;
    }
  }
  svo_publish_block(carry.pub);
}

size_t svo_k_pyramid_bytes(int w, int h) {
  size_t s = 0;
  for (int l = 0; l < LEVELS; ++l) { s += (size_t)w * h; w = (w + 1) / 2; h = (h + 1) / 2; }
  return s;
}

int svo_k_build_pyramid(svo_ctx* ctx, const uint8_t* imgs, int batch, int w, int h, int row_stride, size_t image_stride,
                        uint8_t* pyr, size_t pyr_stride, bool level0_in_place) {
  hipStream_t st = ctx->stream;
  if (!level0_in_place)
    hipLaunchKernelGGL(pyr_copy_kernel, dim3(svo_div_up(w, 64), svo_div_up(h, 4), batch), dim3(256), 0, st, imgs, w, h,
                       row_stride, image_stride, pyr, pyr_stride);
  static const bool per_level = [] { const char* e = getenv("SVO_PYR_PER_LEVEL"); return e && *e && atoi(e) != 0; }();
  if (LEVELS == 4 && !per_level && w >= 64 && h >= 64) {
    const int w1 = (w + 1) / 2, h1 = (h + 1) / 2, tiles_x = svo_div_up(w1, PB_T1W), tiles_y = svo_div_up(h1, PB_T1H);
    const long long total = (long long)tiles_x * tiles_y * batch;
    if (total > 0 && total < (1ll << 30)) {
      SvoProfScope prof(ctx, SVO_PROF_PYR_DOWN);
      hipLaunchKernelGGL(pyr_build_kernel, dim3((unsigned)(8 * ((total + 7) / 8))), dim3(256), 0, st, imgs, image_stride, row_stride, w, h, pyr, pyr_stride,
                         tiles_x, tiles_y, batch);
      SVO_HIP_CHECK(ctx, hipGetLastError());
      return SVO_OK;
    }
  }
  size_t src_off = 0;
  int sw = w, sh = h;
  for (int l = 1; l < LEVELS; ++l) {
    const size_t dst_off = src_off + (size_t)sw * sh;
    const int dw = (sw + 1) / 2, dh = (sh + 1) / 2;
    SvoProfScope prof(ctx, SVO_PROF_PYR_DOWN);
    const bool from_images = level0_in_place && l == 1;
    hipLaunchKernelGGL(pyr_down_kernel, dim3(svo_div_up(dw, 64), svo_div_up(dh, 4), batch), dim3(256), 0, st, pyr, pyr_stride,
                       src_off, sw, sh, dst_off, dw, dh, from_images ? imgs : (const uint8_t*)nullptr, image_stride, row_stride);
    src_off = dst_off; sw = dw; sh = dh;
  }
  SVO_HIP_CHECK(ctx, hipGetLastError());
  return SVO_OK;
}

int svo_k_pyramid_level0(svo_ctx* ctx, const uint8_t* imgs, int batch, int w, int h, int row_stride, size_t image_stride, uint8_t* pyr,
                         size_t pyr_stride, hipStream_t st) {
  hipLaunchKernelGGL(pyr_copy_kernel, dim3(svo_div_up(w, 64), svo_div_up(h, 4), batch), dim3(256), 0, st, imgs, w, h, row_stride, image_stride,
                     pyr, pyr_stride);
  SVO_HIP_CHECK(ctx, hipGetLastError());
  return SVO_OK;
}

int svo_k_lk(svo_ctx* ctx, const uint8_t* pyr_prev, const uint8_t* pyr_next, int w, int h, const float* xy, int n,
             float* out_xy, uint8_t* status) {
  if (n <= 0) return SVO_OK;
  hipLaunchKernelGGL(lk_kernel, dim3(svo_div_up(n, FPB)), dim3(LKT * FPB), 0, ctx->stream, pyr_prev, pyr_next, w, h, xy, n, out_xy, status);
  SVO_HIP_CHECK(ctx, hipGetLastError());
  return SVO_OK;
}

int svo_k_track(svo_ctx* ctx, const uint8_t* pyr_prev, const uint8_t* pyr_next, int w, int h, const float* xy,
                const float* initial_xy, const int* n_dev, int n_max, float* fwd_xy, uint8_t* keep_flag, float* parallax,
                float* kept_xy, int* kept_index, int* n_kept, float* av_parallax, const SvoTrackCarry* carry) {
  if (n_max > 0) {
    SvoProfScope prof(ctx, SVO_PROF_LK_FB);
    hipLaunchKernelGGL(lk_fb_kernel, dim3(svo_div_up(n_max, FPB)), dim3(LKT * FPB), 0, ctx->stream, pyr_prev, pyr_next, w, h, xy, initial_xy, n_dev,
                       n_max, fwd_xy, keep_flag, parallax);
  }
  hipLaunchKernelGGL(track_compact_kernel, dim3(1), dim3(1024), 0, ctx->stream, fwd_xy, keep_flag, parallax, n_dev, n_max,
                     kept_xy, kept_index, n_kept, av_parallax, carry ? *carry : SvoTrackCarry{});
  SVO_HIP_CHECK(ctx, hipGetLastError());
  return SVO_OK;
}

int svo_kg_track(svo_ctx* ctx, hipStream_t st, const SvoLkLanes& lanes, int n_lanes, int grid_x) {
  SvoProfScope prof(ctx, SVO_PROF_LK_FB, st);
  if (lanes.map.per_chunk > 0) hipLaunchKernelGGL(lk_fb_group_kernel, dim3(lanes.map.grid()), dim3(64), 0, st, lanes);
  else hipLaunchKernelGGL(lk_fb_group_kernel, dim3(grid_x, n_lanes), dim3(64), 0, st, lanes);
  SVO_HIP_CHECK(ctx, hipGetLastError());
// ... 112 lines not shown
```

stereo_vo_amd/host/group.cpp:

```cpp
#include <math.h>
#include <stdio.h>
#include <stdlib.h>
#include <string.h>

#include <sched.h>

#include <algorithm>
#include <atomic>
#include <chrono>
#include <condition_variable>
#include <deque>
#include <mutex>
#include <thread>
#include <vector>

#include "chain_math.h"
#include "dense_args.h"
#include "det_trig.h"
#include "group_kernels.h"
#include "group_lines.h"
#include "ref_constants.h"
#include "svo.h"

namespace {

constexpr int GROUP_SOLVE_YIELD_DEFAULT = 8;
int group_solve_yield_default() {
  const char* e = getenv("SVO_BA_YIELD_ITERS");
  return e && *e ? std::max(0, atoi(e)) : GROUP_SOLVE_YIELD_DEFAULT;
}

enum LaneState { L_IDLE = 0, L_TRACK_WAIT, L_NEED_SOLVE, L_PNP_WAIT, L_TRI_WAIT, L_DONE };
enum BaState { BA_NONE = 0, BA_ASSEMBLING, BA_READY, BA_INFLIGHT, BA_HOST_SOLVING, BA_HOST_DONE };
enum Word { W_TRACK = 0, W_PNP, W_TRI, W_COUNT };
enum Counter { C_LK = 0, C_PNP, C_TRI, C_COUNT };
enum Stat { ST_TRACK = 0, ST_PNP, ST_HOST_US, ST_TRI, ST_SOLVE, ST_FRONT_END, ST_COUNT };

struct Lane {
  int lk_line = 0, chain_line = 0;
  float* d_xy[2] = {nullptr, nullptr}; float* d_init[2] = {nullptr, nullptr}; long long* d_ids[2] = {nullptr, nullptr};
  float* d_fwd = nullptr; float* d_par = nullptr; uint8_t* d_keep = nullptr;
  float* h_xy[2] = {nullptr, nullptr}; long long* h_ids[2] = {nullptr, nullptr};
  float* h_kf_xy = nullptr; long long* h_kf_ids = nullptr;
  int* h_n = nullptr; float* h_av = nullptr;
  int cur = 0, n = 0, n_initial = 0;
  bool from_host = false;
  const uint8_t* last_pyr = nullptr;
  const uint8_t* last_l0 = nullptr;
  uint8_t* d_own_pyr = nullptr;
  float4* d_store = nullptr; unsigned store_mask = 0;
  double* d_hyp_pose = nullptr; int* d_hyp_count = nullptr; unsigned long long* d_hyp_mask = nullptr;
  double* d_out = nullptr; int* d_nin = nullptr; int* d_inl = nullptr; float* d_trk_xy = nullptr;
  bool pnp_all = false;
  int* h_best = nullptr; int* h_bad = nullptr; double* h_out = nullptr; int* h_nin = nullptr; int* h_inl = nullptr;
  float* d_disp = nullptr;
  int* h_tri_cnt = nullptr; float* h_tri_xy = nullptr; float* h_tri_xyz = nullptr;
  int* words = nullptr;
  int seq[W_COUNT] = {};
  unsigned* d_arrive = nullptr;
  unsigned arrive_total[C_COUNT] = {0, 0, 0};
  svo_ba* ba = nullptr;
  std::atomic<int> ba_state{BA_NONE};
  svo_ba_summary ba_summary{};
  int ba_rc = 0;
  int ba_launch = 0, ba_line = 0;
  unsigned long long ba_ready_seq = 0;
  bool ba_yielded = false;
  bool has_keyframe = false;
  double solved_pose[7] = {1, 0, 0, 0, 0, 0, 0};
  int last_iterations = 0;
  float rvec[3] = {0, 0, 0}, tvec[3] = {0, 0, 0};
  int state = L_IDLE;
  bool queued = false;
  int frame = 0;
  int pending_from = -1;
  bool first_keyframe = false;
  SvoChainRec* d_chain = nullptr;
  double t_q = 0.0;
  bool fused = false;
  int m_tracked = 0, num_inliers = 0, best = -1;
  float rmat[9], quat[4];
  std::vector<long long> kf_tracked_ids; std::vector<float> kf_tracked_xy;
  std::vector<long long> ids64; std::vector<int64_t> new_ids;
};

struct Pool {
  std::vector<std::thread> th;
  std::mutex mu;
  std::condition_variable cv;
  std::deque<std::pair<Lane*, int>> jobs;
  bool quit = false;
  int device = 0;
  void start(int n, int dev) {
    device = dev;
    for (int i = 0; i < n; ++i) th.emplace_back([this] { run(); });
  }
  void post(Lane* l, int what) {
    { std::lock_guard<std::mutex> g(mu); jobs.emplace_back(l, what); }
    cv.notify_one();
  }
  void run() {
    (void)hipSetDevice(device);
    for (;;) {
      std::pair<Lane*, int> j;
      {
        std::unique_lock<std::mutex> lk(mu);
        cv.wait(lk, [this] { return quit || !jobs.empty(); });
        if (quit && jobs.empty()) return;
        j = jobs.front(); jobs.pop_front();
      }
      Lane* l = j.first;
      if (j.second == 0) {
        l->ba_rc = svo_ba_solve_prepare(l->ba);
        l->ba_state.store(BA_READY, std::memory_order_release);
      } else {
        l->ba_rc = svo_ba_solve_finish(l->ba, &l->ba_summary);
        l->ba_state.store(BA_HOST_DONE, std::memory_order_release);
      }
    }
  }
  void stop() {
    { std::lock_guard<std::mutex> g(mu); quit = true; }
    cv.notify_all();
    for (auto& t : th) t.join();
    th.clear();
  }
};

}

struct svo_pipeline_group {
  svo_ctx* ctx = nullptr;
  svo_pipeline_params prm{};
  int n_lanes = 0, max_batch = 0;
  float K[9];
  std::vector<Lane*> lanes;
  std::vector<void*> dev_allocs, pin_allocs;
  static constexpr int MAX_LINES = 8;
  int n_lk = 1, n_chain = 1, n_ba = 2;
  int n_cmp = 0;
  int xcd_chunks = SVO_XCD_CHUNKS;
  bool xcd_map = true, xcd_map_tri = true;
  double t_get_points = 0, t_add_keyframe = 0, t_finish = 0, t_loop = 0; long n_kf = 0; bool timing = false;
  double gather_us = 0.0;
  hipStream_t st_lk[MAX_LINES] = {}, st_chain[MAX_LINES] = {}, st_ba[MAX_LINES] = {};
  int ba_launch_id = 0;
  unsigned long long ba_ready_counter = 0;
  float* d_corners = nullptr; int* d_ncorners = nullptr; uint8_t* d_pyr[2] = {nullptr, nullptr}; int pyr_cur = 0;
  size_t pyr_stride = 0;
  int* h_counts = nullptr;
  Pool pool;
  int pnp_iterations = 0, mask_words_cap = 0;
  long launches[ST_COUNT] = {}, lanes_carried[ST_COUNT] = {};
  uint8_t* h_stage[2][2] = {{nullptr, nullptr}, {nullptr, nullptr}};
  uint8_t* d_stage[2][2] = {{nullptr, nullptr}, {nullptr, nullptr}};
  hipStream_t st_copy = nullptr;
  hipEvent_t ev_up[2] = {nullptr, nullptr};
  int up_batch[2] = {0, 0};
  std::vector<SvoRectModel*> rect_models;
  SvoRectModel* lane_rect[SVO_MAX_LANES] = {};
  uint8_t* d_rect[2] = {nullptr, nullptr};
  SvoKfClouds* kfc = nullptr;
  bool lane_cloud[SVO_MAX_LANES] = {};
};

namespace {

int fail(svo_pipeline_group* g, const char* what, hipError_t e) {
  g->ctx->err = std::string("pipeline group: ") + what + ": " + hipGetErrorString(e);
  return SVO_ERR_HIP;
}

template <typename T>
int dev_alloc(svo_pipeline_group* g, T** p, size_t count) {
  const hipError_t e = hipMalloc((void**)p, sizeof(T) * (count ? count : 1));
  if (e != hipSuccess) return fail(g, "hipMalloc", e);
  g->dev_allocs.push_back(*p);
  return SVO_OK;
}

int word_ready(const Lane* l, int w) { return __atomic_load_n(&l->words[16 * w], __ATOMIC_ACQUIRE) == l->seq[w]; }

SvoPublish make_pub(Lane* l, int w, int counter, int nblocks) {
  SvoPublish p;
  p.word = &l->words[16 * w];
  p.seq = ++l->seq[w];
  if (counter >= 0) {
    l->arrive_total[counter] += (unsigned)nblocks;
    p.arrive = l->d_arrive + 16 * counter;
    p.target = l->arrive_total[counter];
  }
  return p;
}

void fill_pending(Lane* l, svo_frame_result* res, int upto) {
  if (l->pending_from < 0) return;
  for (int j = l->pending_from; j < upto; ++j) {
    memcpy(res[j].pose7, l->solved_pose, sizeof(res[j].pose7));
    if (j == l->pending_from && res[j].is_keyframe) res[j].ba_iterations = l->last_iterations;
  }
  l->pending_from = -1;
}

int finish_solve(svo_pipeline_group* g, Lane* l) {
  const int st = l->ba_state.load(std::memory_order_acquire);
  l->ba_ready_seq = 0;
  l->ba_yielded = false;
  if (st == BA_NONE) return SVO_OK;
  int rc = SVO_OK;
  const auto tf0 = std::chrono::steady_clock::now();
  if (st == BA_INFLIGHT) rc = svo_ba_solve_finish(l->ba, &l->ba_summary);
  else rc = l->ba_rc;
  if (g->timing) g->t_finish += std::chrono::duration<double, std::nano>(std::chrono::steady_clock::now() - tf0).count();
  l->ba_state.store(BA_NONE, std::memory_order_release);
  if (rc) return rc;
  l->last_iterations = l->ba_summary.iterations;
  double p[7];
  if ((rc = svo_ba_get_pose(l->ba, -1, p))) return rc;
  for (int i = 0; i < 7; ++i) l->solved_pose[i] = (double)(float)p[i];
  (void)g;
  return SVO_OK;
}

void quiesce_after_error(svo_pipeline_group* g) {
  for (int i = 0; i < svo_pipeline_group::MAX_LINES; ++i) {
    if (g->st_lk[i]) (void)hipStreamSynchronize(g->st_lk[i]);
    if (g->st_chain[i]) (void)hipStreamSynchronize(g->st_chain[i]);
    if (g->st_ba[i]) (void)hipStreamSynchronize(g->st_ba[i]);
  }
  for (Lane* l : g->lanes) {
    (void)hipMemset(l->d_arrive, 0, sizeof(unsigned) * 16 * C_COUNT);
    for (int c = 0; c < C_COUNT; ++c) l->arrive_total[c] = 0;
    for (int w = 0; w < W_COUNT; ++w) { l->seq[w] = 0; l->words[16 * w] = 0; }
    if (l->h_bad) *l->h_bad = 0;
    l->fused = false; l->pnp_all = false;
    l->queued = false;
  }
  (void)hipDeviceSynchronize();
}

}

extern "C" void svo_pipeline_group_destroy(svo_pipeline_group* g) {
  if (!g) return;
  (void)hipSetDevice(g->ctx->device);
  g->pool.stop();
  for (Lane* l : g->lanes) {
    if (l->ba_state.load() == BA_INFLIGHT) { svo_ba_summary s; (void)svo_ba_solve_finish(l->ba, &s); }
  }
  if (g->timing && g->n_kf)
    fprintf(stderr, "[svo group] %d lanes, %ld keyframes; group thread per keyframe (us): get_world_points %.1f, add_keyframe %.1f, join + write-back of the solve %.1f\n",
            g->n_lanes, g->n_kf, 1e-3 * g->t_get_points / g->n_kf, 1e-3 * g->t_add_keyframe / g->n_kf, 1e-3 * g->t_finish / g->n_kf);
  (void)hipStreamSynchronize(g->ctx->stream);
  for (Lane* l : g->lanes) { if (l->ba) { svo_ba_destroy(l->ba); l->ba = nullptr; } }
  for (int i = 0; i < svo_pipeline_group::MAX_LINES; ++i) {
    if (g->st_lk[i] && g->st_lk[i] != g->ctx->stream) { (void)hipStreamSynchronize(g->st_lk[i]); (void)hipStreamDestroy(g->st_lk[i]); }
    if (g->st_chain[i]) { (void)hipStreamSynchronize(g->st_chain[i]); (void)hipStreamDestroy(g->st_chain[i]); }
    if (g->st_ba[i]) { (void)hipStreamSynchronize(g->st_ba[i]); (void)hipStreamDestroy(g->st_ba[i]); }
  }
  if (g->st_copy) { (void)hipStreamSynchronize(g->st_copy); (void)hipStreamDestroy(g->st_copy); }
  for (int sl = 0; sl < 2; ++sl) {
    if (g->ev_up[sl]) (void)hipEventDestroy(g->ev_up[sl]);
    for (int e = 0; e < 2; ++e) { if (g->h_stage[sl][e]) (void)hipHostFree(g->h_stage[sl][e]); if (g->d_stage[sl][e]) (void)hipFree(g->d_stage[sl][e]); }
  }
  for (Lane* l : g->lanes) { if (l->ba) svo_ba_destroy(l->ba); delete l; }
  svo_kfc_destroy(g->kfc);
  for (SvoRectModel* m : g->rect_models) svo_rect_model_destroy(m);
  for (int e = 0; e < 2; ++e) if (g->d_rect[e]) (void)hipFree(g->d_rect[e]);
  for (void* p : g->dev_allocs) (void)hipFree(p);
  for (void* p : g->pin_allocs) (void)hipHostFree(p);
  delete g;
}

extern "C" int svo_pipeline_group_create(svo_ctx* ctx, svo_pipeline_group** out, const svo_pipeline_params* p, int n_lanes) {
  if (!ctx || !out || !p) return SVO_ERR_INVALID;
  *out = nullptr;
  SVO_HIP_CHECK(ctx, hipSetDevice(ctx->device));
  SVO_REQUIRE(ctx, n_lanes >= 1 && n_lanes <= SVO_MAX_LANES, "pipeline_group_create: 1..64 lanes");
  SVO_REQUIRE(ctx, p->width >= 32 && p->height >= 32 && p->width <= ctx->lim.max_width && p->height <= ctx->lim.max_height,
              "pipeline_group_create: image size outside the context limits");
  SVO_REQUIRE(ctx, p->max_corners >= 4 && p->max_corners <= ctx->lim.max_corners && p->max_features >= 4 &&
                       p->max_features <= ctx->lim.max_features, "pipeline_group_create: feature counts outside the context limits");
  SVO_REQUIRE(ctx, p->window_size >= 1 && p->window_size <= 63, "pipeline_group_create: window size must be 1..63");
  SVO_REQUIRE(ctx, ctx->lim.max_batch >= n_lanes, "pipeline_group_create: svo_limits.max_batch must hold lanes x frames per call");
  {
    static std::atomic<bool> warned{false};
    const char* q = getenv("GPU_MAX_HW_QUEUES");
    const int nq = q && *q ? atoi(q) : 4;
    if (n_lanes > 4 && nq < 8 && !warned.exchange(true))
      fprintf(stderr, "[svo] pipeline group of %d lanes with GPU_MAX_HW_QUEUES=%d: its launches will share hardware queues and serialise; "
                      "export GPU_MAX_HW_QUEUES=16 before the first HIP call (INTEGRATION.md)\n", n_lanes, nq);
  }
  svo_pipeline_group* g = new svo_pipeline_group();
  g->ctx = ctx; g->prm = *p; g->n_lanes = n_lanes;
  g->max_batch = ctx->lim.max_batch / n_lanes;
  const float K[9] = {(float)p->cam.focal, 0.f, (float)p->cam.cx, 0.f, (float)p->cam.focal, (float)p->cam.cy, 0.f, 0.f, 1.f};
  memcpy(g->K, K, sizeof(K));
  g->pnp_iterations = svo_ref::PNP_ITERATIONS;
  const size_t mc = (size_t)p->max_corners, mf = (size_t)ctx->lim.max_features, B = (size_t)g->max_batch, S = (size_t)n_lanes;
  const int words = (int)((mf + 63) / 64);
  g->mask_words_cap = words;
  int rc = SVO_OK;
  auto chk = [&](hipError_t e, const char* what) { if (rc == SVO_OK && e != hipSuccess) rc = fail(g, what, e); };
  {
    auto knob = [](const char* name, int dflt, int hi) { const char* e = getenv(name); int v = e && *e ? atoi(e) : dflt; return v < 1 ? 1 : (v > hi ? hi : v); };
    g->n_lk = knob("SVO_GROUP_LK_LINES", 1, svo_pipeline_group::MAX_LINES);
    g->timing = getenv("SVO_TIMING") != nullptr;
    { const char* e = getenv("SVO_GROUP_GATHER_US"); g->gather_us = e && *e ? std::max(0.0, atof(e)) : 0.0; }
    g->n_chain = knob("SVO_GROUP_CHAIN_LINES", 2, svo_pipeline_group::MAX_LINES);
    { const char* e = getenv("SVO_GROUP_LK_XCD"); g->xcd_map = !(e && *e && atoi(e) == 0); }
    { const char* e = getenv("SVO_GROUP_TRI_XCD"); g->xcd_map_tri = !(e && *e && atoi(e) == 0); }
    { const char* e = getenv("SVO_GROUP_XCD_CHUNKS"); if (e && *e) g->xcd_chunks = std::max(8, std::min(64, atoi(e) / 8 * 8)); }
    g->n_ba = knob("SVO_GROUP_BA_LINES", 4, svo_pipeline_group::MAX_LINES);
    { const char* e = getenv("SVO_GROUP_COMPACT_LINES"); g->n_cmp = e && *e ? std::max(0, std::min(atoi(e), svo_pipeline_group::MAX_LINES - g->n_ba)) : 0; }
    g->st_lk[0] = ctx->stream;
    for (int i = 1; i < g->n_lk; ++i) chk(hipStreamCreateWithFlags(&g->st_lk[i], hipStreamNonBlocking), "stream");
    for (int i = 0; i < g->n_chain; ++i) chk(hipStreamCreateWithFlags(&g->st_chain[i], hipStreamNonBlocking), "stream");
    for (int i = 0; i < g->n_ba + g->n_cmp; ++i) chk(hipStreamCreateWithFlags(&g->st_ba[i], hipStreamNonBlocking), "stream");
  }
  g->pyr_stride = svo_k_pyramid_bytes(p->width, p->height);
  if (!rc) rc = dev_alloc(g, &g->d_corners, 2 * mc * S * B);
  if (!rc) {
    const char* e = getenv("SVO_GROUP_TOUCH");
    if (!(e && *e && atoi(e) == 0)) {
      hipStream_t order[3 * svo_pipeline_group::MAX_LINES];
      int no = 0;
      for (int i = 0; i < g->n_ba + g->n_cmp; ++i) order[no++] = g->st_ba[i];
      for (int i = 0; i < g->n_chain; ++i) order[no++] = g->st_chain[i];
      for (int i = 0; i < g->n_lk; ++i) order[no++] = g->st_lk[i];
      for (int i = 0; i < no && !rc; ++i) {
        chk(hipMemsetAsync(g->d_corners, 0, 16, order[i]), "hipMemsetAsync");
        chk(hipStreamSynchronize(order[i]), "hipStreamSynchronize");
      }
    }
  }
  if (!rc) rc = dev_alloc(g, &g->d_ncorners, S * B);
  if (!rc) rc = dev_alloc(g, &g->d_pyr[0], g->pyr_stride * S * B);
  if (!rc) rc = dev_alloc(g, &g->d_pyr[1], g->pyr_stride * S * B);
  if (!rc) {
    void* hp = nullptr;
    chk(hipHostMalloc(&hp, sizeof(int) * (S * B + 16), hipHostMallocDefault), "hipHostMalloc");
    if (hp) { g->pin_allocs.push_back(hp); g->h_counts = (int*)hp; memset(hp, 0, sizeof(int) * (S * B + 16)); }
  }
  for (int li = 0; li < n_lanes && !rc; ++li) {
    Lane* l = new Lane();
    g->lanes.push_back(l);
    for (int b = 0; b < 2 && !rc; ++b) {
      rc = dev_alloc(g, &l->d_xy[b], 2 * mf);
      if (!rc) rc = dev_alloc(g, &l->d_init[b], 2 * mf);
      if (!rc) rc = dev_alloc(g, &l->d_ids[b], mf);
    }
    if (!rc) rc = dev_alloc(g, &l->d_fwd, 2 * mf);
    if (!rc) rc = dev_alloc(g, &l->d_par, mf);
    if (!rc) rc = dev_alloc(g, &l->d_keep, mf);
    {
      size_t cap = 1, keyframes = 256;
      if (const char* e = getenv("SVO_GROUP_STORE_KEYFRAMES")) keyframes = (size_t)std::max(1, atoi(e));
      while (cap < keyframes * mf) cap <<= 1;
      l->store_mask = (unsigned)(cap - 1);
      if (!rc) rc = dev_alloc(g, &l->d_store, cap);
      if (!rc) chk(hipMemset(l->d_store, 0xFF, sizeof(float4) * cap), "hipMemset");
    }
    if (!rc) rc = dev_alloc(g, &l->d_hyp_pose, 7 * (size_t)g->pnp_iterations);
    if (!rc) rc = dev_alloc(g, &l->d_hyp_count, (size_t)g->pnp_iterations);
    if (!rc) rc = dev_alloc(g, &l->d_hyp_mask, (size_t)g->pnp_iterations * words);
    if (!rc) rc = dev_alloc(g, &l->d_out, 8);
    if (!rc) rc = dev_alloc(g, &l->d_nin, 16);
    if (!rc) rc = dev_alloc(g, &l->d_inl, mf);
    if (!rc) rc = dev_alloc(g, &l->d_trk_xy, 2 * mf);
    if (!rc) rc = dev_alloc(g, &l->d_chain, 1);
    if (!rc) rc = dev_alloc(g, &l->d_disp, mc);
    if (!rc) rc = dev_alloc(g, &l->d_own_pyr, g->pyr_stride);
    if (!rc) rc = dev_alloc(g, &l->d_arrive, 16 * C_COUNT);
    if (!rc) chk(hipMemset(l->d_arrive, 0, sizeof(unsigned) * 16 * C_COUNT), "hipMemset");
    if (rc) break;
    const size_t f2 = sizeof(float) * 2 * mf, i8 = sizeof(long long) * mf;
    size_t off = 0;
    auto take = [&](size_t bytes) { const size_t o = off; off = (off + bytes + 127) & ~(size_t)127; return o; };
    const size_t o_xy0 = take(f2), o_xy1 = take(f2), o_id0 = take(i8), o_id1 = take(i8), o_kxy = take(f2), o_kid = take(i8), o_n = take(64),
                 o_cnt = take(64), o_out = take(64), o_nin = take(64),
                 o_inl = take(sizeof(int) * mf), o_tc = take(64), o_txy = take(sizeof(float) * 2 * mc), o_txyz = take(sizeof(float) * 3 * mc),
                 o_words = take(64 * W_COUNT);
    void* hp = nullptr;
    chk(hipHostMalloc(&hp, off, hipHostMallocDefault), "hipHostMalloc");
    if (rc) break;
    g->pin_allocs.push_back(hp);
    memset(hp, 0, off);
    char* h = (char*)hp;
    l->h_xy[0] = (float*)(h + o_xy0); l->h_xy[1] = (float*)(h + o_xy1); l->h_ids[0] = (long long*)(h + o_id0); l->h_ids[1] = (long long*)(h + o_id1);
    l->h_kf_xy = (float*)(h + o_kxy); l->h_kf_ids = (long long*)(h + o_kid);
    l->h_n = (int*)(h + o_n); l->h_av = (float*)(h + o_n + 16);
    l->h_best = (int*)(h + o_cnt); l->h_bad = (int*)(h + o_cnt) + 1; l->h_out = (double*)(h + o_out); l->h_nin = (int*)(h + o_nin);
    l->h_inl = (int*)(h + o_inl); l->h_tri_cnt = (int*)(h + o_tc); l->h_tri_xy = (float*)(h + o_txy); l->h_tri_xyz = (float*)(h + o_txyz);
    l->words = (int*)(h + o_words);
    svo_ba_options opt;
    svo_ba_default_options(&opt);
    opt.max_features = p->max_features;
    opt.max_iterations = p->ba_max_iterations;
    opt.max_time_s = p->ba_max_time_s;
    const int max_obs = (p->window_size + 1) * p->max_features + 64;
    rc = svo_ba_create(ctx, &l->ba, p->window_size, &p->cam, &opt, max_obs, max_obs);
    if (!rc) rc = svo_ba_attach_store(l->ba, l->d_store, l->store_mask);
    if (!rc) rc = svo_ba_use_stream(l->ba, g->st_ba[li % g->n_ba]);
    if (!rc) rc = svo_ba_set_yield_iterations(l->ba, group_solve_yield_default());
  }
  if (rc) { svo_pipeline_group_destroy(g); return rc; }
  {
    const char* e = getenv("SVO_GROUP_WORKERS");
    int nw = e ? atoi(e) : (n_lanes < 8 ? n_lanes : 8);
    if (nw < 1) nw = 1;
    if (nw > 8) nw = 8;
    g->pool.start(nw, ctx->device);
  }
  (void)hipDeviceSynchronize();
  *out = g;
  return SVO_OK;
}

extern "C" int svo_pipeline_group_reset(svo_pipeline_group* g) {
  if (!g) return SVO_ERR_INVALID;
  (void)hipSetDevice(g->ctx->device);
  int rc_join = SVO_OK;
  for (Lane* l : g->lanes) {
    const int rcf = finish_solve(g, l);
    if (rcf && !rc_join) rc_join = rcf;
    svo_ba_reset(l->ba);
    l->has_keyframe = false; l->n = l->n_initial = 0; l->from_host = false; l->last_pyr = nullptr; l->last_l0 = nullptr; l->cur = 0;
    l->rvec[0] = l->rvec[1] = l->rvec[2] = l->tvec[0] = l->tvec[1] = l->tvec[2] = 0.f;
    l->state = L_IDLE; l->queued = false; l->pending_from = -1; l->last_iterations = 0;
    const double id7[7] = {1, 0, 0, 0, 0, 0, 0};
    memcpy(l->solved_pose, id7, sizeof(id7));
    if (l->h_bad) *l->h_bad = 0;
    l->fused = false; l->pnp_all = false;
    if (l->d_store && hipMemsetAsync(l->d_store, 0xFF, sizeof(float4) * ((size_t)l->store_mask + 1), g->ctx->stream) != hipSuccess && !rc_join) rc_join = SVO_ERR_HIP;
  }
  if (hipStreamSynchronize(g->ctx->stream) != hipSuccess && !rc_join) rc_join = SVO_ERR_HIP;
  if (rc_join) { quiesce_after_error(g); return rc_join; }
  return SVO_OK;
}

extern "C" int svo_pipeline_group_lanes(const svo_pipeline_group* g) { return g ? g->n_lanes : 0; }

extern "C" int svo_pipeline_group_get_tracked(svo_pipeline_group* g, int lane, int64_t* ids, float* xy, int capacity, int* n) {
  if (!g || !n || lane < 0 || lane >= g->n_lanes) return SVO_ERR_INVALID;
  const Lane* l = g->lanes[lane];
  *n = l->n;
  const float* sx = l->from_host ? l->h_kf_xy : l->h_xy[l->cur];
  const long long* si = l->from_host ? l->h_kf_ids : l->h_ids[l->cur];
  for (int i = 0; i < l->n && i < capacity; ++i) {
    if (ids) ids[i] = (int64_t)si[i];
    if (xy) { xy[2 * i] = sx[2 * i]; xy[2 * i + 1] = sx[2 * i + 1]; }
  }
  return SVO_OK;
}

extern "C" int svo_pipeline_group_set_solve_yield(svo_pipeline_group* g, int n) {
  if (!g || n < 0) return SVO_ERR_INVALID;
  for (Lane* l : g->lanes) {
    const int rc = svo_ba_set_yield_iterations(l->ba, n);
    if (rc) return rc;
  }
  return SVO_OK;
}

extern "C" int svo_pipeline_group_solve_work(svo_pipeline_group* g, double* out4, int reset) {
  if (!g || !out4) return SVO_ERR_INVALID;
  out4[0] = out4[1] = out4[2] = out4[3] = 0.0;
  for (Lane* l : g->lanes) {
    double w[4];
    svo_ba_work(l->ba, w, reset);
    for (int i = 0; i < 4; ++i) out4[i] += w[i];
  }
  return SVO_OK;
}

extern "C" int svo_pipeline_group_solve_forms(svo_pipeline_group* g, long* counts, int n, long* gave_up) {
  if (!g || !counts || n < 1) return SVO_ERR_INVALID;
  std::vector<long> c((size_t)n);
  for (int i = 0; i < n; ++i) counts[i] = 0;
  if (gave_up) *gave_up = 0;
  for (Lane* l : g->lanes) {
    long gu = 0;
    const int rc = svo_ba_solve_forms(l->ba, c.data(), n, &gu);
    if (rc) return rc;
    for (int i = 0; i < n; ++i) counts[i] += c[(size_t)i];
    if (gave_up) *gave_up += gu;
  }
  return SVO_OK;
}

extern "C" int svo_pipeline_group_last_stats(const svo_pipeline_group* g, long* launches6, long* lanes6) {
  if (!g || !launches6 || !lanes6) return SVO_ERR_INVALID;
  static_assert(ST_COUNT == 6, "svo_pipeline_group_last_stats returns six slots");
  for (int i = 0; i < ST_COUNT; ++i) { launches6[i] = g->launches[i]; lanes6[i] = g->lanes_carried[i]; }
  return SVO_OK;
}

namespace {
bool trace_enabled() { static const bool on = getenv("SVO_GROUP_TRACE") != nullptr; return on; }
bool chain_fused_enabled() { static const bool on = [] { const char* e = getenv("SVO_GROUP_CHAIN_FUSED"); return !(e && *e && atoi(e) == 0); }(); return on; }
bool host_solves_only() { static const bool on = [] { const char* e = getenv("SVO_GROUP_HOST_SOLVES"); return e && *e && atoi(e) != 0; }(); return on; }

struct Batch {
  using Clock = std::chrono::steady_clock;
  struct Ev { double us; int lane; const char* what; int arg; };
  static constexpr int MAX_LINES = svo_pipeline_group::MAX_LINES;

  svo_pipeline_group* const g;
  svo_ctx* const ctx;
  const uint8_t* const* const lbase;
  const uint8_t* const* const rbase;
  const int batch;
  svo_frame_result* const results;
  const int W, H, S;
  const size_t istride;
  uint8_t* pyr = nullptr;
  int* hc = nullptr;
  std::vector<int> q_track, q_pnp, q_tri, q_ba;
  int error = SVO_OK;
  const int MODEL = svo_pnp_model_points();
  const bool trace_on = trace_enabled(), chain_fused = chain_fused_enabled();
  std::vector<Ev> evs;
  Clock::time_point t_begin, t_pass, last_progress;
  bool all_done = false, progressed = false;
  bool lk_busy[MAX_LINES] = {}, chain_busy[MAX_LINES] = {}, ba_line_busy[MAX_LINES] = {};
  double t_now_us = 0.0;
  unsigned idle_spins = 0;
  double busy_us = 0.0;

  Batch(svo_pipeline_group* g_, const uint8_t* const* lb, const uint8_t* const* rb, int batch_, svo_frame_result* res)
      : g(g_), ctx(g_->ctx), lbase(lb), rbase(rb), batch(batch_), results(res), W(g_->prm.width), H(g_->prm.height), S(g_->n_lanes),
        istride((size_t)g_->prm.width * g_->prm.height) {}

  svo_frame_result& RES(int lane, int f) const { return results[(size_t)lane * batch + f]; }
  const uint8_t* IMG(const uint8_t* const* base, int lane, int f) const { return base[lane] + (size_t)f * istride; }
  uint8_t* PYR(int lane, int f) const { return pyr + ((size_t)lane * batch + f) * g->pyr_stride; }
  const uint8_t* L0(int lane, int f) const { return f == batch - 1 ? PYR(lane, f) : IMG(lbase, lane, f); }
  float* DET(int lane, int f) const { return g->d_corners + ((size_t)lane * batch + f) * 2 * g->prm.max_corners; }
  double now_us() const { return std::chrono::duration<double, std::micro>(Clock::now() - t_begin).count(); }
  void EV(int lane, const char* what, int arg) { if (trace_on) evs.push_back({now_us(), lane, what, arg}); }
  void enqueue(std::vector<int>& q, int li, int state) {
    Lane* l = g->lanes[li];
    q.push_back(li); l->queued = true; l->t_q = now_us(); l->state = state;
  }
  void count(Stat s, int lanes) { g->launches[s]++; g->lanes_carried[s] += lanes; progressed = true; }

  void frame_done(int li) {
    Lane* l = g->lanes[li];
    svo_frame_result* res = &RES(li, 0);
    const int i = l->frame;
    if (l->has_keyframe && !(res[i].is_keyframe) && l->pending_from < 0) l->pending_from = i;
    l->frame = i + 1;
    l->state = l->frame < batch ? L_IDLE : L_DONE;
  }

  int keyframe_tail(int li) {
    Lane* l = g->lanes[li];
    svo_frame_result* res = &RES(li, 0);
    const int i = l->frame;
    const int m_new = *l->h_tri_cnt;
    double pose7[7];
    if (l->first_keyframe) {
      const double id7[7] = {1, 0, 0, 0, 0, 0, 0};
      memcpy(pose7, id7, sizeof(id7));
      l->kf_tracked_ids.clear(); l->kf_tracked_xy.clear();
    } else {
      pose7[0] = l->quat[0]; pose7[1] = l->quat[1]; pose7[2] = l->quat[2]; pose7[3] = l->quat[3];
      pose7[4] = l->tvec[0]; pose7[5] = l->tvec[1]; pose7[6] = l->tvec[2];
    }
    const int nt = (int)l->kf_tracked_ids.size();
    l->new_ids.assign((size_t)(m_new > 0 ? m_new : 1), 0);
    int kept = 0;
    std::vector<int64_t> tid(l->kf_tracked_ids.begin(), l->kf_tracked_ids.end());
    const auto ta0 = Clock::now();
    int rc2 = svo_ba_add_keyframe(l->ba, pose7, tid.data(), l->kf_tracked_xy.data(), nt, l->h_tri_xy, l->h_tri_xyz, m_new, l->new_ids.data(), &kept);
    if (g->timing) { g->t_add_keyframe += std::chrono::duration<double, std::nano>(Clock::now() - ta0).count(); g->n_kf++; }
    if (rc2) return rc2;
    fill_pending(l, res, i);
    l->pending_from = i;
    l->has_keyframe = true;
    l->ba_state.store(BA_ASSEMBLING, std::memory_order_release);
    g->pool.post(l, 0);
    EV(li, "assembly_posted", i);
    int n = nt + kept;
    if (n > ctx->lim.max_features) n = ctx->lim.max_features;
    for (int k = 0; k < nt && k < n; ++k) { l->h_kf_xy[2 * k] = l->kf_tracked_xy[2 * k]; l->h_kf_xy[2 * k + 1] = l->kf_tracked_xy[2 * k + 1]; l->h_kf_ids[k] = l->kf_tracked_ids[k]; }
    for (int k = nt; k < n; ++k) { l->h_kf_xy[2 * k] = l->h_tri_xy[2 * (k - nt)]; l->h_kf_xy[2 * k + 1] = l->h_tri_xy[2 * (k - nt) + 1]; l->h_kf_ids[k] = (long long)l->new_ids[k - nt]; }
    l->n = l->n_initial = n;
    l->from_host = true;
    l->last_pyr = PYR(li, i);
    l->last_l0 = L0(li, i);
    if (l->first_keyframe) { l->tvec[0] = l->tvec[1] = l->tvec[2] = 0.f; l->rvec[0] = l->rvec[1] = l->rvec[2] = 0.f; }
    res[i].is_keyframe = 1;
    res[i].n_new = kept;
    frame_done(li);
    return SVO_OK;
  }

  int consume_pnp(int li) {
    Lane* l = g->lanes[li];
    if (*l->h_bad) {
      ctx->err = "pipeline group: a tracked feature's entry of the landmark store belongs to another id (store capacity exceeded?)";
      error = SVO_ERR_CAPACITY;
      return -1;
    }
    l->best = *l->h_best;
    if (l->best == -2) {
      l->pnp_all = true;
      enqueue(q_pnp, li, L_PNP_WAIT);
      return -1;
    }
    if (l->best >= 0) {
      double rv[3];
      svo_det_rvec_from_quat(l->h_out, rv);
      for (int k = 0; k < 3; ++k) { l->rvec[k] = (float)rv[k]; l->tvec[k] = (float)l->h_out[4 + k]; }
      l->num_inliers = *l->h_nin;
    }
    return 0;
  }

  void after_pnp(int li, bool queue_tri = true) {
    Lane* l = g->lanes[li];
    svo_frame_result* res = &RES(li, 0);
    res[l->frame].n_inliers = l->num_inliers;
    svo_det_rodrigues_f(l->rvec, l->rmat);
    svo_det_quat_from_R(l->rmat, l->quat);
    const float* txy = l->h_xy[l->cur];
    const long long* tids = l->h_ids[l->cur];
    l->kf_tracked_ids.resize(l->num_inliers); l->kf_tracked_xy.resize(2 * (size_t)l->num_inliers);
    for (int k = 0; k < l->num_inliers; ++k) {
      const int idx = l->h_inl[k];
      l->kf_tracked_ids[k] = tids[idx];
      l->kf_tracked_xy[2 * k] = txy[2 * idx]; l->kf_tracked_xy[2 * k + 1] = txy[2 * idx + 1];
    }
    l->first_keyframe = false;
    if (queue_tri) enqueue(q_tri, li, L_TRI_WAIT);
  }

  int continue_keyframe(int li) {
    Lane* l = g->lanes[li];
    const int m = l->n;
    l->m_tracked = m;
    l->num_inliers = 0; l->best = -1;
    if (m >= MODEL) enqueue(q_pnp, li, L_PNP_WAIT);
    else after_pnp(li);
    return SVO_OK;
  }

  int after_track(int li) {
    Lane* l = g->lanes[li];
    svo_frame_result& r = RES(li, l->frame);
    const float av = *l->h_av;
    const float pl = (float)(1.0 - (double)((float)l->n / (float)l->n_initial));
    r.n_tracked = l->n; r.av_parallax = av; r.percent_lost = pl;
    if (av <= g->prm.parallax_thresh && (double)pl < svo_ref::KEYFRAME_PERCENT_LOST) { frame_done(li); return SVO_OK; }
    if (l->ba_state.load(std::memory_order_acquire) != BA_NONE) { l->state = L_NEED_SOLVE; EV(li, "need_solve", l->ba_state.load()); return SVO_OK; }
    return continue_keyframe(li);
  }

  int start_frame(int li) {
    Lane* l = g->lanes[li];
    const int i = l->frame;
    svo_frame_result& r = RES(li, i);
    const int n_det = hc[li * batch + i];
    r.n_detected = n_det;
    if (n_det < svo_ref::MIN_DETECTED) { frame_done(li); return SVO_OK; }
    if (!l->has_keyframe) {
      l->first_keyframe = true;
      l->num_inliers = 0;
      enqueue(q_tri, li, L_TRI_WAIT);
      return SVO_OK;
    }
    if (l->n <= 0) {
      l->n = 0; *l->h_av = 0.f;
      return after_track(li);
    }
    enqueue(q_track, li, L_TRACK_WAIT);
    return SVO_OK;
  }

  void advance_lane(int li) {
    Lane* l = g->lanes[li];
    for (bool again = true; again && !error;) {
      again = false;
      switch (l->state) {
        case L_IDLE:
          error = start_frame(li);
          progressed = true;
          again = l->state == L_IDLE;
          break;
        case L_TRACK_WAIT:
          if (l->queued || !word_ready(l, W_TRACK)) break;
          EV(li, "track_done", l->frame);
          l->cur ^= 1; l->from_host = false;
          l->n = *l->h_n;
          l->last_pyr = PYR(li, l->frame);
          l->last_l0 = L0(li, l->frame);
          error = after_track(li);
          progressed = true; again = l->state == L_IDLE;
          break;
        case L_NEED_SOLVE:
          if (!solve_came_back(l)) break;
          EV(li, "solve_joined_for_pnp", l->frame);
          error = finish_solve(g, l);
          if (!error) error = continue_keyframe(li);
          progressed = true; again = l->state == L_IDLE;
          break;
        case L_PNP_WAIT:
          if (l->queued || !word_ready(l, W_PNP)) break;
          EV(li, "pnp_done", l->frame);
          progressed = true;
          if (consume_pnp(li) < 0) break;
          after_pnp(li, true);
          break;
        case L_TRI_WAIT:
          if (l->queued || !word_ready(l, W_TRI)) break;
          EV(li, "tri_done", l->frame);
          progressed = true;
          if (l->fused) {
            l->fused = false;
            if (consume_pnp(li) < 0) break;
            after_pnp(li, false);
          }
          error = keyframe_tail(li);
          again = l->state == L_IDLE;
          break;
        default: break;
      }
    }
  }

  int front_end() {
    const int mc = g->prm.max_corners;
    hipStream_t st = ctx->stream;
    bool tight = true;
    for (int l = 1; l < S; ++l) tight = tight && lbase[l] == lbase[0] + (size_t)l * batch * istride;
    const uint8_t* const left = lbase[0];
    const size_t lane_stride = istride * (size_t)batch;
    for (int i = 0; i < ST_COUNT; ++i) { g->launches[i] = 0; g->lanes_carried[i] = 0; }
    g->pyr_cur ^= 1;
    pyr = g->d_pyr[g->pyr_cur];
    int rc = SVO_OK;
    const uint8_t* lo = pyr;
    const uint8_t* hi = pyr + g->pyr_stride * (size_t)g->n_lanes * (size_t)g->max_batch;
    for (Lane* l : g->lanes) {
      if (!l->last_pyr || l->last_pyr < lo || l->last_pyr >= hi) continue;
      SVO_HIP_CHECK(ctx, hipMemcpyAsync(l->d_own_pyr, l->last_pyr, g->pyr_stride, hipMemcpyDeviceToDevice, ctx->stream));
      l->last_pyr = l->d_own_pyr;
      l->last_l0 = l->d_own_pyr;
    }
    if (tight) {
      rc = svo_corner_detect_batch_dev(ctx, left, S * batch, W, H, W, istride, mc, g->prm.quality, (double)g->prm.min_feature_distance, g->d_corners, g->d_ncorners);
      if (!rc) rc = svo_k_build_pyramid(ctx, left, S * batch, W, H, W, istride, pyr, g->pyr_stride, true);
      if (!rc) rc = svo_k_pyramid_level0(ctx, left + (size_t)(batch - 1) * istride, S, W, H, W, lane_stride, pyr + (size_t)(batch - 1) * g->pyr_stride,
                                         (size_t)batch * g->pyr_stride, st);
    } else {
      for (int l = 0; l < S && !rc; ++l) {
        rc = svo_corner_detect_batch_dev(ctx, lbase[l], batch, W, H, W, istride, mc, g->prm.quality, (double)g->prm.min_feature_distance,
                                         g->d_corners + (size_t)l * batch * 2 * mc, g->d_ncorners + (size_t)l * batch);
        if (!rc) rc = svo_k_build_pyramid(ctx, lbase[l], batch, W, H, W, istride, pyr + (size_t)l * batch * g->pyr_stride, g->pyr_stride, true);
        if (!rc) rc = svo_k_pyramid_level0(ctx, lbase[l] + (size_t)(batch - 1) * istride, 1, W, H, W, istride,
                                           pyr + ((size_t)l * batch + (size_t)(batch - 1)) * g->pyr_stride, g->pyr_stride, st);
      }
    }
    if (rc) return rc;
    g->launches[ST_FRONT_END] += 7; g->lanes_carried[ST_FRONT_END] += 7 * S;
    hc = g->h_counts;
    SVO_HIP_CHECK(ctx, hipMemcpyAsync(hc, g->d_ncorners, sizeof(int) * S * batch, hipMemcpyDeviceToHost, st));
    SVO_HIP_CHECK(ctx, hipMemcpyAsync(hc + S * batch, ctx->d_status, sizeof(int), hipMemcpyDeviceToHost, st));
    SVO_HIP_CHECK(ctx, hipStreamSynchronize(st));
    if (hc[S * batch]) {
      (void)hipMemsetAsync(ctx->d_status, 0, sizeof(int), st);
      ctx->err = (hc[S * batch] & 8) ? "corner detection: more raw local maxima than the streaming pass's list holds (raw_cap: width x height / 4 per image under a 1 GiB budget)"
                           : "corner detection exceeded a workspace bound (svo_limits.max_candidates)";
      return SVO_ERR_CAPACITY;
    }
    return SVO_OK;
  }

  void advance_lanes() {
    all_done = true;
    for (int li = 0; li < S && !error; ++li) {
      advance_lane(li);
      if (g->lanes[li]->state != L_DONE) all_done = false;
    }
  }

  void scan_lines() {
    for (int i = 0; i < MAX_LINES; ++i) lk_busy[i] = chain_busy[i] = false;
    for (int li = 0; li < S; ++li) {
      const Lane* l = g->lanes[li];
      if (l->queued) continue;
      lk_busy[l->lk_line] |= l->state == L_TRACK_WAIT;
      chain_busy[l->chain_line] |= l->state == L_PNP_WAIT || l->state == L_TRI_WAIT;
    }
    t_now_us = now_us();
  }
  bool ripe(const std::vector<int>& q, int line, int n_lines, int near_state) const {
    return svo_line_ripe(q, S, line, n_lines, t_now_us, g->gather_us, [&](int li) { return g->lanes[li]->t_q; },
                         [&](int li) { return g->lanes[li]->state == near_state && !g->lanes[li]->queued; });
  }

  void fill_lk_lane(Lane* l, int li, SvoLkLane& x, int workgroups) {
    const int nxt = l->cur ^ 1;
    x.pyr_prev = l->last_pyr; x.pyr_next = PYR(li, l->frame);
    x.l0_prev = l->last_l0; x.l0_next = L0(li, l->frame);
    x.xy = l->from_host ? l->h_kf_xy : l->d_xy[l->cur];
    x.init_xy = l->from_host ? l->h_kf_xy : l->d_init[l->cur];
    x.ids = l->from_host ? l->h_kf_ids : l->d_ids[l->cur];
    x.n = l->n;
    x.fwd = l->d_fwd; x.keep = l->d_keep; x.parallax = l->d_par;
    x.kept_xy = l->d_xy[nxt]; x.init_dst = l->d_init[nxt]; x.ids_dst = l->d_ids[nxt];
    x.host_xy = l->h_xy[nxt]; x.host_ids = l->h_ids[nxt]; x.host_n = l->h_n; x.host_av = l->h_av;
    l->arrive_total[C_LK] += (unsigned)workgroups;
    x.arrive = l->d_arrive + 16 * C_LK; x.arrive_target = l->arrive_total[C_LK];
    x.word = &l->words[16 * W_TRACK]; x.seq = ++l->seq[W_TRACK];
    l->queued = false;
  }

  void launch_tracking() {
    scan_lines();
    for (int line = 0; line < g->n_lk && !error; ++line) {
      if (lk_busy[line] || !ripe(q_track, line, g->n_lk, L_TRI_WAIT)) continue;
      const std::vector<int> q_now = svo_line_take(q_track, line, g->n_lk);
      if (q_now.empty()) continue;
      for (int li : q_now) g->lanes[li]->lk_line = line;
      SvoLkLanes a;
      a.w = W; a.h = H;
      int gx = 1;
      for (int li : q_now) gx = std::max(gx, g->lanes[li]->n);
      a.map.per_chunk = 0; a.map.total = 0; a.map.chunks = 0;
      if (g->xcd_map) {
        int counts[SVO_MAX_LANES], j = 0;
        for (int li : q_now) counts[j++] = g->lanes[li]->n;
        svo_xcd_map_fill(a.map, counts, j, g->xcd_chunks);
      }
      int k = 0;
      for (int li : q_now) {
        Lane* l = g->lanes[li];
        fill_lk_lane(l, li, a.lane[k++], a.map.per_chunk > 0 ? std::max(1, l->n) : gx);
      }
      if ((error = svo_kg_track(ctx, g->st_lk[line], a, k, gx))) return;
      for (int li : q_now) EV(li, "track_launch", k);
      count(ST_TRACK, k);
    }
  }

  void fill_pnp_lane(Lane* l, int li, SvoPnpLane& x) {
    (void)li;
    const int m = l->m_tracked;
    x.ids = l->d_ids[l->cur]; x.store = l->d_store; x.store_mask = l->store_mask;
    x.xy = l->d_xy[l->cur]; x.n = m;
    x.f = (double)g->K[0]; x.cx = (double)g->K[2]; x.cy = (double)g->K[5];
    const double rv[3] = {l->rvec[0], l->rvec[1], l->rvec[2]};
    svo_det_quat_from_rvec(rv, x.q0);
    for (int c = 0; c < 3; ++c) x.t0[c] = (double)l->tvec[c];
    x.thr2 = (double)svo_ref::PNP_REPROJ_ERROR * (double)svo_ref::PNP_REPROJ_ERROR;
    x.confidence = svo_ref::PNP_CONFIDENCE; x.iterations = g->pnp_iterations;
    x.launched = l->pnp_all ? g->pnp_iterations : svo_kg_pnp_first(g->pnp_iterations);
    l->pnp_all = false;
    const int wgs = svo_kg_pnp_workgroups(x.launched);
    x.hyp_pose = l->d_hyp_pose; x.hyp_count = l->d_hyp_count; x.hyp_mask = l->d_hyp_mask; x.mask_words = svo_div_up(m, 64);
    x.out_pose = l->d_out; x.inliers = l->d_inl; x.n_inliers = l->d_nin; x.inlier_xy = l->d_trk_xy;
    x.host_pose = l->h_out; x.host_inliers = l->h_inl; x.host_nin = l->h_nin; x.host_best = l->h_best; x.host_bad = l->h_bad;
    const SvoPublish pb = make_pub(l, W_PNP, C_PNP, wgs);
    x.arrive = pb.arrive; x.arrive_target = pb.target; x.word = pb.word; x.seq = pb.seq;
    x.chain = chain_fused ? l->d_chain : nullptr;
    for (int c = 0; c < 3; ++c) { x.prev_rvec[c] = l->rvec[c]; x.prev_tvec[c] = l->tvec[c]; }
    x.cam_f = g->K[0]; x.cam_cx = g->K[2]; x.cam_cy = g->K[5]; x.cam_b = (float)g->prm.cam.baseline;
    l->queued = false;
  }

  void launch_pnp(int line, const std::vector<int>& h_now, std::vector<int>& t_now) {
    SvoPnpLanes a;
    int k = 0;
    for (int li : h_now) fill_pnp_lane(g->lanes[li], li, a.lane[k++]);
    if ((error = svo_kg_pnp(ctx, g->st_chain[line], a, k))) return;
    for (int li : h_now) EV(li, "pnp_launch", k);
    count(ST_PNP, k);
    if (chain_fused) for (int li : h_now) { g->lanes[li]->fused = true; t_now.push_back(li); }
  }

  void fill_tri_lane(Lane* l, int li, SvoStereoTriLane& x, int workgroups) {
    const int i = l->frame, n_det = hc[li * batch + i];
    x.xy = DET(li, i); x.n_dev = nullptr;
    x.trk = nullptr; x.n_trk = 0; x.min_d = 0.f;
    x.chain = nullptr;
    if (l->fused) {
      x.chain = l->d_chain; x.trk = l->d_trk_xy; x.min_d = g->prm.min_feature_distance;
    } else if (!l->first_keyframe) {
      x.trk = l->d_trk_xy; x.n_trk = l->num_inliers; x.min_d = g->prm.min_feature_distance;
      if (x.n_trk <= 0) x.trk = nullptr;
    }
    x.left = IMG(lbase, li, i); x.right = IMG(rbase, li, i);
    x.n_max = n_det; x.disp = l->d_disp;
    const float I9[9] = {1, 0, 0, 0, 1, 0, 0, 0, 1}, zero3[3] = {0, 0, 0};
    const bool posed = !l->fused && !l->first_keyframe;
    svo_chain_matrix_from_R(posed ? l->rmat : I9, posed ? l->tvec : zero3, g->K[0], g->K[2], g->K[5], (float)g->prm.cam.baseline, x.M.m);
    x.kept_xy = l->h_tri_xy; x.xyz = l->h_tri_xyz; x.n_kept = l->h_tri_cnt;
    x.pub = make_pub(l, W_TRI, C_TRI, workgroups);
    l->state = L_TRI_WAIT;
    l->queued = false;
  }

  void launch_tri(int line, const std::vector<int>& t_now) {
    SvoStereoTriLanes t;
    t.w = W; t.h = H; t.stride = W; t.ndisp = svo_ref::STEREO_NUM_DISPARITIES; t.block = svo_ref::STEREO_BLOCK_SIZE;
    int kt = 0, gxt = 1;
    t.map.per_chunk = 0; t.map.total = 0; t.map.chunks = 0;
    int counts[SVO_MAX_LANES], j = 0;
    for (int li : t_now) {
      const int n_det = hc[li * batch + g->lanes[li]->frame];
      gxt = std::max(gxt, n_det);
      counts[j++] = n_det;
    }
    if (g->xcd_map_tri) svo_xcd_map_fill(t.map, counts, j, g->xcd_chunks);
    for (int li : t_now) {
      Lane* l = g->lanes[li];
      fill_tri_lane(l, li, t.lane[kt++], t.map.per_chunk > 0 ? std::max(1, hc[li * batch + l->frame]) : gxt);
    }
    if ((error = svo_kg_stereo_triangulate(ctx, g->st_chain[line], t, kt, gxt))) return;
    for (int li : t_now) EV(li, "tri_launch", kt);
    count(ST_TRI, kt);
  }

  void launch_chains() {
    for (int line = 0; line < g->n_chain && !error; ++line) {
      if (chain_busy[line]) continue;
      const std::vector<int> h_now = ripe(q_pnp, line, g->n_chain, L_TRACK_WAIT) ? svo_line_take(q_pnp, line, g->n_chain) : std::vector<int>();
      std::vector<int> t_now = svo_line_take(q_tri, line, g->n_chain);
      for (int li : h_now) g->lanes[li]->chain_line = line;
      for (int li : t_now) g->lanes[li]->chain_line = line;
      if (!h_now.empty()) launch_pnp(line, h_now, t_now);
      if (!error && !t_now.empty()) launch_tri(line, t_now);
    }
  }

  bool solve_came_back(Lane* l) {
    const int bs = l->ba_state.load(std::memory_order_acquire);
    if (bs == BA_INFLIGHT && svo_ba_solve_poll(l->ba) && svo_ba_solve_continues(l->ba)) {
      l->ba_yielded = true;
      l->ba_state.store(BA_READY, std::memory_order_release);
      progressed = true;
      return false;
    }
    return (bs == BA_INFLIGHT && svo_ba_solve_poll(l->ba)) || bs == BA_HOST_DONE;
  }
  bool any_solve_in_flight(bool holding_budget) const {
    bool any = false;
    for (const Lane* l : g->lanes)
      any |= l->ba_state.load(std::memory_order_acquire) == BA_INFLIGHT && (!holding_budget || svo_ba_solve_holds_budget(l->ba));
    return any;
  }

  void join_finished_solves() {
    for (int li = 0; li < S && !error; ++li) {
      Lane* l = g->lanes[li];
      if (l->state == L_NEED_SOLVE || !solve_came_back(l)) continue;
      EV(li, "solve_joined", l->frame);
      error = finish_solve(g, l);
      progressed = true;
    }
  }

  void solves_departed(const int* lanes, int n, unsigned long long taken, int line, int carried, const char* what) {
    ++g->ba_launch_id;
// ... 427 lines not shown
```

Baseline: 15140 frames/s.

## Cache LK backward-pass templates for reuse as next frame's forward templates

Adds a per-lane, double-buffered device cache. The backward LK pass writes its per-level template (intensity, gradients, structure tensor) for each feature, and the next frame's forward pass on the same image reloads it instead of staging and recomputing the tile. A source-index map carries the cache slot through compaction and keyframe remapping, and tags plus position and id checks validate each entry. This trades extra memory (about 16.5 KB per feature slot, two buffers per lane) and write-through traffic for skipping tile staging, gradient computation and the block reduction on hits. It also adds counters and a stats API.

```diff
diff --git a/include/svo.h b/include/svo.h
--- a/include/svo.h
+++ b/include/svo.h
@@ -400,6 +400,7 @@
 int svo_pipeline_group_copy_keyframe_disparity(svo_pipeline_group* g, int i, int16_t* host);
 int svo_pipeline_group_get_tracked(svo_pipeline_group* g, int lane, int64_t* ids, float* xy, int capacity, int* n);
 int svo_pipeline_group_last_stats(const svo_pipeline_group* g, long* launches6, long* lanes6);
+int svo_pipeline_group_lk_cache_stats(svo_pipeline_group* g, int lane, long* out6, int reset);
 int svo_pipeline_group_solve_work(svo_pipeline_group* g, double* out4, int reset);
 int svo_pipeline_group_solve_forms(svo_pipeline_group* g, long* counts, int n, long* gave_up);
 int svo_pipeline_group_set_solve_yield(svo_pipeline_group* g, int n);
diff --git a/stereo_vo_amd/api.py b/stereo_vo_amd/api.py
--- a/stereo_vo_amd/api.py
+++ b/stereo_vo_amd/api.py
@@ -375,7 +375,7 @@
     "svo_pipeline_default_params", "svo_pipeline_create", "svo_pipeline_destroy", "svo_pipeline_reset",
     "svo_pipeline_process_batch_dev", "svo_pipeline_process_batch", "svo_pipeline_get_tracked",
     "svo_pipeline_group_create", "svo_pipeline_group_destroy", "svo_pipeline_group_reset", "svo_pipeline_group_lanes",
-    "svo_pipeline_group_process_batch_dev", "svo_pipeline_group_get_tracked", "svo_pipeline_group_last_stats",
+    "svo_pipeline_group_process_batch_dev", "svo_pipeline_group_get_tracked", "svo_pipeline_group_last_stats", "svo_pipeline_group_lk_cache_stats",
     "svo_pipeline_group_solve_work", "svo_pipeline_group_solve_forms", "svo_pipeline_group_set_solve_yield", "svo_pipeline_group_staging", "svo_pipeline_group_upload", "svo_pipeline_group_process_uploaded", "svo_pipeline_group_process_batch",
     "svo_synth_default_params", "svo_synth_render", "svo_synth_pose",
     "svo_image_read_gray", "svo_kitti_read_poses", "svo_ate_rmse", "svo_kitti_run", "svo_cholesky_solve", "svo_cholesky_solve_dev", "svo_draw_track", "svo_pipeline_draw_track",
@@ -1367,6 +1367,13 @@
         self.ctx._chk(self.L.svo_pipeline_group_solve_forms(self.h, out, n, None), "svo_pipeline_group_solve_forms")
         return out[n - 1]
 
+    LK_CACHE_STATS = ("launched", "mapped", "hits", "misses", "launches", "launches_all_mapped")
+
+    def lk_cache_stats(self, lane=-1, reset=False):
+        out = (C.c_long * 6)()
+        self.ctx._chk(self.L.svo_pipeline_group_lk_cache_stats(self.h, int(lane), out, int(bool(reset))), "svo_pipeline_group_lk_cache_stats")
+        return dict(zip(self.LK_CACHE_STATS, list(out)))
+
     def last_stats(self):
         a, b = (C.c_long * 6)(), (C.c_long * 6)()
         self.ctx._chk(self.L.svo_pipeline_group_last_stats(self.h, a, b), "svo_pipeline_group_last_stats")
diff --git a/stereo_vo_amd/csrc/ba.hip b/stereo_vo_amd/csrc/ba.hip
--- a/stereo_vo_amd/csrc/ba.hip
+++ b/stereo_vo_amd/csrc/ba.hip
@@ -20,6 +20,7 @@
 #include "lm_lds.h"
 #include "lm_turns.h"
 #include "ref_constants.h"
+#include "wide_coherent.h"
 #include "reproj_device.h"
 
 int svo_rccl_allreduce_f64(void* buf, size_t count, void* comm, hipStream_t stream, const char** err);
@@ -87,7 +88,7 @@
 __device__ __forceinline__ void slot_store2(double* p, double x, double y) {
   if constexpr (WT) {
     const svo_d2 v = {x, y};
-    asm volatile("global_store_dwordx4 %0, %1, off sc1\n\ts_nop 1" : : "v"(p), "v"(v) : "memory");
+    svo_wt_store16(p, v);
   } else {
     p[0] = x; p[1] = y;
   }
@@ -102,13 +103,7 @@
   const double* p2 = base + 2 * (idx[2] < 0 ? 0 : idx[2]); const double* p3 = base + 2 * (idx[3] < 0 ? 0 : idx[3]);
   const double* p4 = base + 2 * (idx[4] < 0 ? 0 : idx[4]); const double* p5 = base + 2 * (idx[5] < 0 ? 0 : idx[5]);
   const double* p6 = base + 2 * (idx[6] < 0 ? 0 : idx[6]); const double* p7 = base + 2 * (idx[7] < 0 ? 0 : idx[7]);
-  asm volatile(
-      "global_load_dwordx4 %0, %8, off sc1\n\tglobal_load_dwordx4 %1, %9, off sc1\n\tglobal_load_dwordx4 %2, %10, off sc1\n\t"
-      "global_load_dwordx4 %3, %11, off sc1\n\tglobal_load_dwordx4 %4, %12, off sc1\n\tglobal_load_dwordx4 %5, %13, off sc1\n\t"
-      "global_load_dwordx4 %6, %14, off sc1\n\tglobal_load_dwordx4 %7, %15, off sc1\n\ts_waitcnt vmcnt(0)"
-      : "=&v"(v0), "=&v"(v1), "=&v"(v2), "=&v"(v3), "=&v"(v4), "=&v"(v5), "=&v"(v6), "=&v"(v7)
-      : "v"(p0), "v"(p1), "v"(p2), "v"(p3), "v"(p4), "v"(p5), "v"(p6), "v"(p7)
-      : "memory");
+  svo_coherent_load16x8(p0, p1, p2, p3, p4, p5, p6, p7, v0, v1, v2, v3, v4, v5, v6, v7);
   const svo_d2 v[8] = {v0, v1, v2, v3, v4, v5, v6, v7};
   unsigned ok = 0;
 #pragma unroll
@@ -140,8 +135,7 @@
     const double* p = base + 2 * ((size_t)first + (size_t)i * stride);
     long long t0 = 0;
     for (unsigned spins = 0;; ++spins) {
-      svo_d2 v;
-      asm volatile("global_load_dwordx4 %0, %1, off sc1\n\ts_waitcnt vmcnt(0)" : "=&v"(v) : "v"(p) : "memory");
+      const svo_d2 v = svo_coherent_load16<svo_d2>(p);
       if ((unsigned long long)__double_as_longlong(v.y) == tag) break;
       __builtin_amdgcn_s_sleep(4);
       if ((spins & 255u) == 255u) {
diff --git a/stereo_vo_amd/csrc/group_kernels.h b/stereo_vo_amd/csrc/group_kernels.h
--- a/stereo_vo_amd/csrc/group_kernels.h
+++ b/stereo_vo_amd/csrc/group_kernels.h
@@ -15,6 +15,11 @@
   float* host_xy; long long* host_ids; int* host_n; float* host_av;
   unsigned* arrive; unsigned arrive_target;
   int* word; int seq;
+  char* cache_wr; char* cache_rd; int cache_slots;
+  unsigned cache_tag;
+  const int* src;
+  int* src_dst; int* host_src;
+  unsigned long long* cache_cnt;
 };
 struct SvoLkLanes { int w, h; SvoXcdMap map; SvoLkLane lane[SVO_MAX_LANES]; };
 int svo_kg_track(svo_ctx* ctx, hipStream_t st, const SvoLkLanes& lanes, int n_lanes, int grid_x);
diff --git a/stereo_vo_amd/csrc/lk.hip b/stereo_vo_amd/csrc/lk.hip
--- a/stereo_vo_amd/csrc/lk.hip
+++ b/stereo_vo_amd/csrc/lk.hip
@@ -1,6 +1,8 @@
 #include "kernels.h"
 #include "group_kernels.h"
 #include "tail_device.h"
+#include "wide_coherent.h"
+#include "lk_cache_map.h"
 
 namespace {
 #include "ref_constants.h"
@@ -125,10 +127,18 @@
   phase ^= 1;
 }
 
-__device__ uint8_t lk_point_wave(const Pyr& A, const Pyr& B, float px0, float py0, float* ox, float* oy, LkShared& S);
+enum { LKC_NONE = 0, LKC_READ, LKC_WRITE };
+struct LkCacheIo {
+  char* entry;
+  int mode;
+  unsigned tag;
+};
+
+template <bool CACHE>
+__device__ uint8_t lk_point_wave(const Pyr& A, const Pyr& B, float px0, float py0, float* ox, float* oy, LkShared& S, LkCacheIo& io);
 
 __device__ uint8_t lk_point(const Pyr& A, const Pyr& B, float px0, float py0, float* ox, float* oy, LkShared& S) {
-  if (NW == 1) return lk_point_wave(A, B, px0, py0, ox, oy, S);
+  if (NW == 1) { LkCacheIo none{nullptr, LKC_NONE, 0u}; return lk_point_wave<false>(A, B, px0, py0, ox, oy, S, none); }
   const int lane = threadIdx.x % LKT;
   int phase = 0;
   uint8_t status = 1;
@@ -308,6 +318,7 @@
   } else {
     constexpr int NB = N * N, PERB = (NB + 63) / 64;
     uint8_t v[PERB];
+    asm volatile("" : "+v"(lane));
 #pragma unroll
     for (int k = 0; k < PERB; ++k) {
       const int i = lane + 64 * k;
@@ -322,7 +333,8 @@
   }
 }
 
-__device__ uint8_t lk_point_wave(const Pyr& A, const Pyr& B, float px0, float py0, float* ox, float* oy, LkShared& S) {
+template <bool CACHE>
+__device__ uint8_t lk_point_wave(const Pyr& A, const Pyr& B, float px0, float py0, float* ox, float* oy, LkShared& S, LkCacheIo& io) {
   const int lane = threadIdx.x & 63;
   const bool act = lane < 63;
   const int r = act ? lane / 3 : 0, c0 = act ? 7 * (lane - 3 * (lane / 3)) : 0;
@@ -348,53 +360,87 @@
     int iw01 = __float2int_rn(a * (1.f - b) * (float)(1 << 14));
     int iw10 = __float2int_rn((1.f - a) * b * (float)(1 << 14));
     int iw11 = (1 << 14) - iw00 - iw01 - iw10;
-    lk_sync();
-    stage_tile<RP, sizeof(S.raw)>(S.raw, Ip, Iw_, Ih_, ipx - 1, ipy - 1, lane);
-    lk_sync();
-    int tI[7], tX[7], tY[7];
-    int pA[3] = {0, 0, 0};
-    {
-      int t[4][10];
-#pragma unroll
-      for (int j = 0; j < 4; ++j)
-#pragma unroll
-        for (int i = 0; i < 10; ++i) t[j][i] = S.raw[(r + j) * RP + c0 + i];
-      int gx[2][8], gy[2][8];
-#pragma unroll
-      for (int j = 0; j < 2; ++j)
-#pragma unroll
-        for (int i = 0; i < 8; ++i) {
-          const int X = ipx + c0 + i, Y = ipy + r + j;
-          const int s0 = (t[j][i] + t[j + 2][i]) * 3 + t[j + 1][i] * 10, s2 = (t[j][i + 2] + t[j + 2][i + 2]) * 3 + t[j + 1][i + 2] * 10;
-          const int d0 = t[j + 2][i] - t[j][i], d1 = t[j + 2][i + 1] - t[j][i + 1], d2 = t[j + 2][i + 2] - t[j][i + 2];
-          const bool in = X >= 0 && X < Iw_ && Y >= 0 && Y < Ih_;
-          gx[j][i] = in ? (int)(short)(s2 - s0) : 0;
-          gy[j][i] = in ? (int)(short)((d2 + d0) * 3 + d1 * 10) : 0;
+    int tI[7];
+    lk_s2 tXp[4], tYp[4];
+    float A11 = 0.f, A12 = 0.f, A22 = 0.f;
+    bool hit = false;
+    if (CACHE && io.mode == LKC_READ) {
+      svo_u4 u0, u1, u2, u3, ra;
+      svo_coherent_load16x5_at(io.entry + level * SVO_LK_CACHE_LEVEL_BYTES, svo_unit_lane_off(lane), io.entry + SVO_LK_CACHE_REC_OFF + 16 * level, svo_unit_zero_off(), u0, u1, u2, u3, ra);
+      const unsigned want = io.tag - 1u;
+      hit = __ballot(u0.w == want && u1.w == want && u2.w == want && u3.w == want && ra.w == want) == ~0ull;
+      if (hit) {
+        const unsigned w[12] = {u0.x, u0.y, u0.z, u1.x, u1.y, u1.z, u2.x, u2.y, u2.z, u3.x, u3.y, u3.z};
+#pragma unroll
+        for (int q = 0; q < 4; ++q) { tXp[q] = __builtin_bit_cast(lk_s2, w[q]); tYp[q] = __builtin_bit_cast(lk_s2, w[4 + q]); }
+#pragma unroll
+        for (int p = 0; p < 7; ++p) tI[p] = (1 << 8) - ((p & 1 ? (int)w[8 + (p >> 1)] >> 16 : (int)(short)(w[8 + (p >> 1)] & 0xFFFFu)) << 9);
+        const unsigned a11 = ra.x, a12 = ra.y, a22 = ra.z;
+        A11 = __uint_as_float(a11); A12 = __uint_as_float(a12); A22 = __uint_as_float(a22);
+      } else {
+        io.mode = LKC_NONE;
+      }
+    }
+    if (!hit) {
+      lk_sync();
+      stage_tile<RP, sizeof(S.raw)>(S.raw, Ip, Iw_, Ih_, ipx - 1, ipy - 1, lane);
+      lk_sync();
+      int tX[7], tY[7];
+      int pA[3] = {0, 0, 0};
+      {
+        int t[4][10];
+#pragma unroll
+        for (int j = 0; j < 4; ++j)
+#pragma unroll
+          for (int i = 0; i < 10; ++i) t[j][i] = S.raw[(r + j) * RP + c0 + i];
+        int gx[2][8], gy[2][8];
+#pragma unroll
+        for (int j = 0; j < 2; ++j)
+#pragma unroll
+          for (int i = 0; i < 8; ++i) {
+            const int X = ipx + c0 + i, Y = ipy + r + j;
+            const int s0 = (t[j][i] + t[j + 2][i]) * 3 + t[j + 1][i] * 10, s2 = (t[j][i + 2] + t[j + 2][i + 2]) * 3 + t[j + 1][i + 2] * 10;
+            const int d0 = t[j + 2][i] - t[j][i], d1 = t[j + 2][i + 1] - t[j][i + 1], d2 = t[j + 2][i + 2] - t[j][i + 2];
+            const bool in = X >= 0 && X < Iw_ && Y >= 0 && Y < Ih_;
+            gx[j][i] = in ? (int)(short)(s2 - s0) : 0;
+            gy[j][i] = in ? (int)(short)((d2 + d0) * 3 + d1 * 10) : 0;
+          }
+#pragma unroll
+        for (int p = 0; p < 7; ++p) {
+          const int ival = descale(__mul24(t[1][p + 1], iw00) + __mul24(t[1][p + 2], iw01) + __mul24(t[2][p + 1], iw10) + __mul24(t[2][p + 2], iw11), 9);
+          const int ixv = descale(__mul24(gx[0][p], iw00) + __mul24(gx[0][p + 1], iw01) + __mul24(gx[1][p], iw10) + __mul24(gx[1][p + 1], iw11), 14);
+          const int iyv = descale(__mul24(gy[0][p], iw00) + __mul24(gy[0][p + 1], iw01) + __mul24(gy[1][p], iw10) + __mul24(gy[1][p + 1], iw11), 14);
+          tI[p] = (1 << 8) - ((int)(short)ival << 9); tX[p] = (int)(short)ixv; tY[p] = (int)(short)iyv;
+          if (act) {
+            pA[0] += __mul24(tX[p], tX[p]);
+            pA[1] += __mul24(tX[p], tY[p]);
+            pA[2] += __mul24(tY[p], tY[p]);
+          }
         }
-#pragma unroll
-      for (int p = 0; p < 7; ++p) {
-        const int ival = descale(__mul24(t[1][p + 1], iw00) + __mul24(t[1][p + 2], iw01) + __mul24(t[2][p + 1], iw10) + __mul24(t[2][p + 2], iw11), 9);
-        const int ixv = descale(__mul24(gx[0][p], iw00) + __mul24(gx[0][p + 1], iw01) + __mul24(gx[1][p], iw10) + __mul24(gx[1][p + 1], iw11), 14);
-        const int iyv = descale(__mul24(gy[0][p], iw00) + __mul24(gy[0][p + 1], iw01) + __mul24(gy[1][p], iw10) + __mul24(gy[1][p + 1], iw11), 14);
-        tI[p] = (1 << 8) - ((int)(short)ival << 9); tX[p] = (int)(short)ixv; tY[p] = (int)(short)iyv;
-        if (act) {
-          pA[0] += __mul24(tX[p], tX[p]);
-          pA[1] += __mul24(tX[p], tY[p]);
-          pA[2] += __mul24(tY[p], tY[p]);
-        }
-      }
-    }
-    lk_s2 tXp[4], tYp[4];
-#pragma unroll
-    for (int q = 0; q < 4; ++q) {
-      tXp[q] = pack_s2(act ? tX[2 * q] : 0, act && 2 * q + 1 < 7 ? tX[2 * q + 1] : 0);
-      tYp[q] = pack_s2(act ? tY[2 * q] : 0, act && 2 * q + 1 < 7 ? tY[2 * q + 1] : 0);
-    }
-    long long sA[3];
-    block_sum_split<3>(pA, sA, S, phase);
-    const float A11 = (float)(double)sA[0] * FLT_SCALE;
-    const float A12 = (float)(double)sA[1] * FLT_SCALE;
-    const float A22 = (float)(double)sA[2] * FLT_SCALE;
+      }
+#pragma unroll
+      for (int q = 0; q < 4; ++q) {
+        tXp[q] = pack_s2(act ? tX[2 * q] : 0, act && 2 * q + 1 < 7 ? tX[2 * q + 1] : 0);
+        tYp[q] = pack_s2(act ? tY[2 * q] : 0, act && 2 * q + 1 < 7 ? tY[2 * q + 1] : 0);
+      }
+      long long sA[3];
+      block_sum_split<3>(pA, sA, S, phase);
+      A11 = (float)(double)sA[0] * FLT_SCALE;
+      A12 = (float)(double)sA[1] * FLT_SCALE;
+      A22 = (float)(double)sA[2] * FLT_SCALE;
+    }
+    if (CACHE && io.mode == LKC_WRITE) {
+      const char* e = io.entry + level * SVO_LK_CACHE_LEVEL_BYTES;
+      const unsigned lo = svo_unit_lane_off(lane);
+      unsigned iv[4];
+#pragma unroll
+      for (int q = 0; q < 4; ++q) iv[q] = __builtin_bit_cast(unsigned, pack_s2(((1 << 8) - tI[2 * q]) >> 9, 2 * q + 1 < 7 ? ((1 << 8) - tI[2 * q + 1]) >> 9 : 0));
+      svo_wt_store16_at<0>(e, lo, svo_u4{__builtin_bit_cast(unsigned, tXp[0]), __builtin_bit_cast(unsigned, tXp[1]), __builtin_bit_cast(unsigned, tXp[2]), io.tag});
+      svo_wt_store16_at<1024>(e, lo, svo_u4{__builtin_bit_cast(unsigned, tXp[3]), __builtin_bit_cast(unsigned, tYp[0]), __builtin_bit_cast(unsigned, tYp[1]), io.tag});
+      svo_wt_store16_at<2048>(e, lo, svo_u4{__builtin_bit_cast(unsigned, tYp[2]), __builtin_bit_cast(unsigned, tYp[3]), iv[0], io.tag});
+      svo_wt_store16_at<3072>(e, lo, svo_u4{iv[1], iv[2], iv[3], io.tag});
+      if (lane == 0) svo_wt_store16_at<0>(io.entry + SVO_LK_CACHE_REC_OFF + 16 * level, svo_unit_zero_off(), svo_u4{__float_as_uint(A11), __float_as_uint(A12), __float_as_uint(A22), io.tag});
+    }
     float D = A11 * A22 - A12 * A12;
     const float dif = A11 - A22;
     const float minEig = (A22 + A11 - sqrtf(dif * dif + 4.f * A12 * A12)) / (float)(2 * WIN * WIN);
@@ -652,13 +698,29 @@
     const float x0 = a.xy[2 * f], y0 = a.xy[2 * f + 1];
     float fx = 0.f, fy = 0.f, bx = 0.f, by = 0.f, px = x0, py = y0;
     uint8_t s1 = 0, s2 = 0;
+    char* rd = nullptr;
+    if (a.cache_wr && a.cache_tag > 1u) {
+      const int s = __builtin_amdgcn_readfirstlane(a.src[f]);
+      if (s >= 0 && s < a.cache_slots) {
+        char* e = a.cache_rd + (size_t)s * SVO_LK_CACHE_SLOT_BYTES;
+        const svo_u4 fr = svo_coherent_load16<svo_u4>(e + SVO_LK_CACHE_FEAT_OFF);
+        const bool ok = fr.x == __float_as_uint(x0) && fr.y == __float_as_uint(y0) && fr.z == (unsigned)a.ids[f] && fr.w == a.cache_tag - 1u;
+        if (__builtin_amdgcn_readfirstlane((int)ok)) rd = e;
+      }
+    }
+    bool all_hit = false;
 #pragma nounroll
     for (int dir = 0; dir < 2; ++dir) {
       const Pyr P0 = dir ? B : A, P1 = dir ? A : B;
       float ox, oy;
-      const uint8_t st = lk_point(P0, P1, px, py, &ox, &oy, S);
-      if (dir == 0) { s1 = st; fx = ox; fy = oy; px = ox; py = oy; if (!st) break; }
+      LkCacheIo io{dir ? a.cache_wr + (size_t)f * SVO_LK_CACHE_SLOT_BYTES : rd, dir ? (a.cache_wr ? LKC_WRITE : LKC_NONE) : (rd ? LKC_READ : LKC_NONE), a.cache_tag};
+      const uint8_t st = (uint8_t)__builtin_amdgcn_readfirstlane((int)lk_point_wave<true>(P0, P1, px, py, &ox, &oy, S, io));
+      if (dir == 0) { s1 = st; fx = ox; fy = oy; px = ox; py = oy; all_hit = io.mode == LKC_READ; if (!st) break; }
       else { s2 = st; bx = ox; by = oy; }
+    }
+    if (a.cache_wr && lane == 0) {
+      if (s1) svo_wt_store16(a.cache_wr + (size_t)f * SVO_LK_CACHE_SLOT_BYTES + SVO_LK_CACHE_FEAT_OFF, svo_u4{__float_as_uint(fx), __float_as_uint(fy), (unsigned)a.ids[f], a.cache_tag});
+      __hip_atomic_fetch_add(&a.cache_cnt[all_hit ? 0 : 1], 1ull, __ATOMIC_RELAXED, __HIP_MEMORY_SCOPE_AGENT);
     }
     if (lane == 0) {
       uint8_t k = 0;
@@ -693,6 +755,7 @@
       a.ids_dst[slot] = id;
       a.host_xy[2 * slot] = fx; a.host_xy[2 * slot + 1] = fy;
       a.host_ids[slot] = id;
+      if (a.src_dst) { a.src_dst[slot] = i; a.host_src[slot] = i; }
     }
     base += __popcll(mask);
 #pragma unroll
diff --git a/stereo_vo_amd/csrc/wide_coherent.h b/stereo_vo_amd/csrc/wide_coherent.h
--- /dev/null
+++ b/stereo_vo_amd/csrc/wide_coherent.h
@@ -0,0 +1,60 @@
+#ifndef SVO_WIDE_COHERENT_H_
+#define SVO_WIDE_COHERENT_H_
+
+#if defined(__HIPCC__)
+typedef unsigned svo_u4 __attribute__((ext_vector_type(4)));
+
+template <typename V>
+__device__ __forceinline__ void svo_wt_store16(void* p, V v) {
+  static_assert(sizeof(V) == 16, "one 16-byte unit");
+  asm volatile("global_store_dwordx4 %0, %1, off sc1\n\ts_nop 1" : : "v"(p), "v"(v) : "memory");
+}
+
+template <typename V>
+__device__ __forceinline__ V svo_coherent_load16(const void* p) {
+  static_assert(sizeof(V) == 16, "one 16-byte unit");
+  V v;
+  asm volatile("global_load_dwordx4 %0, %1, off sc1\n\ts_waitcnt vmcnt(0)" : "=&v"(v) : "v"(p) : "memory");
+  return v;
+}
+
+template <int OFF, typename V>
+__device__ __forceinline__ void svo_wt_store16_at(const void* base, unsigned lane_off, V v) {
+  static_assert(sizeof(V) == 16 && OFF >= 0 && OFF < 4096, "one 16-byte unit, 12-bit immediate");
+  asm volatile("global_store_dwordx4 %0, %1, %2 offset:%3 sc1\n\ts_nop 1" : : "v"(lane_off), "v"(v), "s"(base), "n"(OFF) : "memory");
+}
+__device__ __forceinline__ unsigned svo_unit_lane_off(unsigned lane) {
+  asm volatile("v_lshlrev_b32 %0, 4, %0" : "+v"(lane));
+  return lane;
+}
+__device__ __forceinline__ unsigned svo_unit_zero_off() {
+  unsigned z;
+  asm volatile("v_mov_b32 %0, 0" : "=v"(z));
+  return z;
+}
+template <typename V>
+__device__ __forceinline__ void svo_coherent_load16x5_at(const void* base, unsigned lane_off, const void* base4, unsigned off4, V& v0, V& v1, V& v2,
+                                                         V& v3, V& v4) {
+  static_assert(sizeof(V) == 16, "16-byte units");
+  asm volatile(
+      "global_load_dwordx4 %0, %5, %6 sc1\n\tglobal_load_dwordx4 %1, %5, %6 offset:1024 sc1\n\tglobal_load_dwordx4 %2, %5, %6 offset:2048 sc1\n\t"
+      "global_load_dwordx4 %3, %5, %6 offset:3072 sc1\n\tglobal_load_dwordx4 %4, %7, %8 sc1\n\ts_waitcnt vmcnt(0)"
+      : "=&v"(v0), "=&v"(v1), "=&v"(v2), "=&v"(v3), "=&v"(v4)
+      : "v"(lane_off), "s"(base), "v"(off4), "s"(base4)
+      : "memory");
+}
+
+template <typename V>
+__device__ __forceinline__ void svo_coherent_load16x8(const void* p0, const void* p1, const void* p2, const void* p3, const void* p4, const void* p5,
+                                                      const void* p6, const void* p7, V& v0, V& v1, V& v2, V& v3, V& v4, V& v5, V& v6, V& v7) {
+  static_assert(sizeof(V) == 16, "16-byte units");
+  asm volatile(
+      "global_load_dwordx4 %0, %8, off sc1\n\tglobal_load_dwordx4 %1, %9, off sc1\n\tglobal_load_dwordx4 %2, %10, off sc1\n\t"
+      "global_load_dwordx4 %3, %11, off sc1\n\tglobal_load_dwordx4 %4, %12, off sc1\n\tglobal_load_dwordx4 %5, %13, off sc1\n\t"
+      "global_load_dwordx4 %6, %14, off sc1\n\tglobal_load_dwordx4 %7, %15, off sc1\n\ts_waitcnt vmcnt(0)"
+      : "=&v"(v0), "=&v"(v1), "=&v"(v2), "=&v"(v3), "=&v"(v4), "=&v"(v5), "=&v"(v6), "=&v"(v7)
+      : "v"(p0), "v"(p1), "v"(p2), "v"(p3), "v"(p4), "v"(p5), "v"(p6), "v"(p7)
+      : "memory");
+}
+#endif
+#endif
diff --git a/stereo_vo_amd/host/group.cpp b/stereo_vo_amd/host/group.cpp
--- a/stereo_vo_amd/host/group.cpp
+++ b/stereo_vo_amd/host/group.cpp
@@ -19,6 +19,7 @@
 #include "det_trig.h"
 #include "group_kernels.h"
 #include "group_lines.h"
+#include "lk_cache_map.h"
 #include "ref_constants.h"
 #include "svo.h"
 
@@ -47,6 +48,13 @@
   bool from_host = false;
   const uint8_t* last_pyr = nullptr;
   const uint8_t* last_l0 = nullptr;
+  char* d_cache[2] = {nullptr, nullptr};
+  int* d_src[2] = {nullptr, nullptr}; int* h_src[2] = {nullptr, nullptr};
+  int* h_kf_src = nullptr;
+  unsigned long long* d_cache_cnt = nullptr;
+  unsigned lk_tag = 0;
+  int kf_mapped = 0;
+  long cache_stat[6] = {0, 0, 0, 0, 0, 0};
   uint8_t* d_own_pyr = nullptr;
   float4* d_store = nullptr; unsigned store_mask = 0;
   double* d_hyp_pose = nullptr; int* d_hyp_count = nullptr; unsigned long long* d_hyp_mask = nullptr;
@@ -136,6 +144,7 @@
   float K[9];
   std::vector<Lane*> lanes;
   std::vector<void*> dev_allocs, pin_allocs;
+  int lk_cache = 1;
   static constexpr int MAX_LINES = 8;
   int n_lk = 1, n_chain = 1, n_ba = 2;
   int n_cmp = 0;
@@ -251,6 +260,12 @@
   if (g->timing && g->n_kf)
     fprintf(stderr, "[svo group] %d lanes, %ld keyframes; group thread per keyframe (us): get_world_points %.1f, add_keyframe %.1f, join + write-back of the solve %.1f\n",
             g->n_lanes, g->n_kf, 1e-3 * g->t_get_points / g->n_kf, 1e-3 * g->t_add_keyframe / g->n_kf, 1e-3 * g->t_finish / g->n_kf);
+  if (g->timing && g->lk_cache) {
+    long c[6];
+    if (svo_pipeline_group_lk_cache_stats(g, -1, c, 0) == SVO_OK)
+      fprintf(stderr, "[svo group] tracker template cache: %ld features in %ld launches, %ld mapped, %ld hits, %ld misses (hit share %.3f)\n", c[0], c[4], c[1], c[2],
+              c[3], c[0] > 0 ? (double)c[2] / (double)c[0] : 0.0);
+  }
   (void)hipStreamSynchronize(g->ctx->stream);
   for (Lane* l : g->lanes) { if (l->ba) { svo_ba_destroy(l->ba); l->ba = nullptr; } }
   for (int i = 0; i < svo_pipeline_group::MAX_LINES; ++i) {
@@ -312,6 +327,7 @@
     { const char* e = getenv("SVO_GROUP_TRI_XCD"); g->xcd_map_tri = !(e && *e && atoi(e) == 0); }
     { const char* e = getenv("SVO_GROUP_XCD_CHUNKS"); if (e && *e) g->xcd_chunks = std::max(8, std::min(64, atoi(e) / 8 * 8)); }
     g->n_ba = knob("SVO_GROUP_BA_LINES", 4, svo_pipeline_group::MAX_LINES);
+    { const char* e = getenv("SVO_GROUP_LK_TEMPLATE_CACHE"); g->lk_cache = !e || !*e ? 1 : (!strcmp(e, "stale") ? 2 : (atoi(e) != 0 ? 1 : 0)); }
     { const char* e = getenv("SVO_GROUP_COMPACT_LINES"); g->n_cmp = e && *e ? std::max(0, std::min(atoi(e), svo_pipeline_group::MAX_LINES - g->n_ba)) : 0; }
     g->st_lk[0] = ctx->stream;
     for (int i = 1; i < g->n_lk; ++i) chk(hipStreamCreateWithFlags(&g->st_lk[i], hipStreamNonBlocking), "stream");
@@ -371,6 +387,23 @@
     if (!rc) rc = dev_alloc(g, &l->d_chain, 1);
     if (!rc) rc = dev_alloc(g, &l->d_disp, mc);
     if (!rc) rc = dev_alloc(g, &l->d_own_pyr, g->pyr_stride);
+    if (!rc && g->lk_cache) {
+      const size_t half = (size_t)(svo_lk_cache_lane_bytes((int)mf) / 2);
+      for (int b = 0; b < 2 && !rc; ++b) {
+        if (hipMalloc((void**)&l->d_cache[b], half) != hipSuccess) {
+          (void)hipGetLastError();
+          l->d_cache[b] = nullptr;
+          ctx->err = "pipeline_group_create: the tracker's template cache does not fit in device memory (16.5 KB x max_features x 2 per lane; SVO_GROUP_LK_TEMPLATE_CACHE=0 runs without it)";
+          rc = SVO_ERR_CAPACITY;
+          break;
+        }
+        g->dev_allocs.push_back(l->d_cache[b]);
+        chk(hipMemset(l->d_cache[b], 0, half), "hipMemset");
+        if (!rc) rc = dev_alloc(g, &l->d_src[b], mf);
+      }
+      if (!rc) rc = dev_alloc(g, &l->d_cache_cnt, 2);
+      if (!rc) chk(hipMemset(l->d_cache_cnt, 0, sizeof(unsigned long long) * 2), "hipMemset");
+    }
     if (!rc) rc = dev_alloc(g, &l->d_arrive, 16 * C_COUNT);
     if (!rc) chk(hipMemset(l->d_arrive, 0, sizeof(unsigned) * 16 * C_COUNT), "hipMemset");
     if (rc) break;
@@ -380,7 +413,7 @@
     const size_t o_xy0 = take(f2), o_xy1 = take(f2), o_id0 = take(i8), o_id1 = take(i8), o_kxy = take(f2), o_kid = take(i8), o_n = take(64),
                  o_cnt = take(64), o_out = take(64), o_nin = take(64),
                  o_inl = take(sizeof(int) * mf), o_tc = take(64), o_txy = take(sizeof(float) * 2 * mc), o_txyz = take(sizeof(float) * 3 * mc),
-                 o_words = take(64 * W_COUNT);
+                 o_words = take(64 * W_COUNT), o_src0 = take(sizeof(int) * mf), o_src1 = take(sizeof(int) * mf), o_ksrc = take(sizeof(int) * mf);
     void* hp = nullptr;
     chk(hipHostMalloc(&hp, off, hipHostMallocDefault), "hipHostMalloc");
     if (rc) break;
@@ -393,6 +426,7 @@
     l->h_best = (int*)(h + o_cnt); l->h_bad = (int*)(h + o_cnt) + 1; l->h_out = (double*)(h + o_out); l->h_nin = (int*)(h + o_nin);
     l->h_inl = (int*)(h + o_inl); l->h_tri_cnt = (int*)(h + o_tc); l->h_tri_xy = (float*)(h + o_txy); l->h_tri_xyz = (float*)(h + o_txyz);
     l->words = (int*)(h + o_words);
+    l->h_src[0] = (int*)(h + o_src0); l->h_src[1] = (int*)(h + o_src1); l->h_kf_src = (int*)(h + o_ksrc);
     svo_ba_options opt;
     svo_ba_default_options(&opt);
     opt.max_features = p->max_features;
@@ -486,6 +520,26 @@
     for (int i = 0; i < n; ++i) counts[i] += c[(size_t)i];
     if (gave_up) *gave_up += gu;
   }
+  return SVO_OK;
+}
+
+extern "C" int svo_pipeline_group_lk_cache_stats(svo_pipeline_group* g, int lane, long* out6, int reset) {
+  if (!g || !out6 || lane < -1 || lane >= g->n_lanes) return SVO_ERR_INVALID;
+  (void)hipSetDevice(g->ctx->device);
+  for (int i = 0; i < 6; ++i) out6[i] = 0;
+  if (!g->lk_cache) return SVO_OK;
+  if (hipDeviceSynchronize() != hipSuccess) return SVO_ERR_HIP;
+  for (int li = 0; li < g->n_lanes; ++li) {
+    if (lane >= 0 && li != lane) continue;
+    Lane* l = g->lanes[(size_t)li];
+    unsigned long long cnt[2] = {0, 0};
+    if (hipMemcpy(cnt, l->d_cache_cnt, sizeof(cnt), hipMemcpyDeviceToHost) != hipSuccess) return SVO_ERR_HIP;
+    l->cache_stat[2] += (long)cnt[0]; l->cache_stat[3] += (long)cnt[1];
+    if (hipMemset(l->d_cache_cnt, 0, sizeof(cnt)) != hipSuccess) return SVO_ERR_HIP;
+    for (int i = 0; i < 6; ++i) out6[i] += l->cache_stat[i];
+    if (reset) for (int i = 0; i < 6; ++i) l->cache_stat[i] = 0;
+  }
+  if (hipDeviceSynchronize() != hipSuccess) return SVO_ERR_HIP;
   return SVO_OK;
 }
 
@@ -586,6 +640,7 @@
     if (n > ctx->lim.max_features) n = ctx->lim.max_features;
     for (int k = 0; k < nt && k < n; ++k) { l->h_kf_xy[2 * k] = l->kf_tracked_xy[2 * k]; l->h_kf_xy[2 * k + 1] = l->kf_tracked_xy[2 * k + 1]; l->h_kf_ids[k] = l->kf_tracked_ids[k]; }
     for (int k = nt; k < n; ++k) { l->h_kf_xy[2 * k] = l->h_tri_xy[2 * (k - nt)]; l->h_kf_xy[2 * k + 1] = l->h_tri_xy[2 * (k - nt) + 1]; l->h_kf_ids[k] = (long long)l->new_ids[k - nt]; }
+    l->kf_mapped = svo_lk_cache_map_keyframe(l->d_cache[0] ? l->h_src[l->cur] : nullptr, l->m_tracked, l->h_inl, nt, n, l->h_kf_src);
     l->n = l->n_initial = n;
     l->from_host = true;
     l->last_pyr = PYR(li, i);
@@ -812,6 +867,15 @@
     x.fwd = l->d_fwd; x.keep = l->d_keep; x.parallax = l->d_par;
     x.kept_xy = l->d_xy[nxt]; x.init_dst = l->d_init[nxt]; x.ids_dst = l->d_ids[nxt];
     x.host_xy = l->h_xy[nxt]; x.host_ids = l->h_ids[nxt]; x.host_n = l->h_n; x.host_av = l->h_av;
+    x.cache_wr = nullptr; x.cache_rd = nullptr; x.cache_slots = 0; x.cache_tag = 0; x.src = nullptr; x.src_dst = nullptr; x.host_src = nullptr; x.cache_cnt = nullptr;
+    if (l->d_cache[0]) {
+      x.cache_wr = l->d_cache[nxt]; x.cache_rd = l->d_cache[g->lk_cache == 2 ? nxt : l->cur]; x.cache_slots = ctx->lim.max_features;
+      x.cache_tag = ++l->lk_tag;
+      x.src = l->from_host ? l->h_kf_src : l->d_src[l->cur];
+      x.src_dst = l->d_src[nxt]; x.host_src = l->h_src[nxt]; x.cache_cnt = l->d_cache_cnt;
+      const int mapped = x.cache_tag > 1u ? (l->from_host ? l->kf_mapped : l->n) : 0;
+      l->cache_stat[0] += l->n; l->cache_stat[1] += mapped; l->cache_stat[4] += 1; l->cache_stat[5] += mapped == l->n;
+    }
     l->arrive_total[C_LK] += (unsigned)workgroups;
     x.arrive = l->d_arrive + 16 * C_LK; x.arrive_target = l->arrive_total[C_LK];
     x.word = &l->words[16 * W_TRACK]; x.seq = ++l->seq[W_TRACK];
diff --git a/stereo_vo_amd/host/lk_cache_map.h b/stereo_vo_amd/host/lk_cache_map.h
--- /dev/null
+++ b/stereo_vo_amd/host/lk_cache_map.h
@@ -0,0 +1,27 @@
+#ifndef SVO_LK_CACHE_MAP_H_
+#define SVO_LK_CACHE_MAP_H_
+
+constexpr int SVO_LK_CACHE_LEVELS = 4;
+constexpr int SVO_LK_CACHE_UNITS = 4;
+constexpr int SVO_LK_CACHE_LEVEL_BYTES = SVO_LK_CACHE_UNITS * 64 * 16;
+constexpr int SVO_LK_CACHE_REC_OFF = SVO_LK_CACHE_LEVELS * SVO_LK_CACHE_LEVEL_BYTES;
+constexpr int SVO_LK_CACHE_FEAT_OFF = SVO_LK_CACHE_REC_OFF + 16 * SVO_LK_CACHE_LEVELS;
+constexpr int SVO_LK_CACHE_SLOT_BYTES = SVO_LK_CACHE_FEAT_OFF + 64;
+inline unsigned long long svo_lk_cache_lane_bytes(int max_features) { return 2ull * (unsigned long long)max_features * SVO_LK_CACHE_SLOT_BYTES; }
+
+inline int svo_lk_cache_map_keyframe(const int* kept_src, int n_kept, const int* inl, int n_tracked, int n, int* out) {
+  int mapped = 0;
+  for (int k = 0; k < n; ++k) {
+    int s = -1;
+    if (k < n_tracked && kept_src && inl) {
+      const int idx = inl[k];
+      if (idx >= 0 && idx < n_kept) s = kept_src[idx];
+      if (s < 0) s = -1;
+    }
+    out[k] = s;
+    mapped += s >= 0;
+  }
+  return mapped;
+}
+
+#endif
```

Result: slower. 14960 frames/s (-1.2%).
